# gabeur/mmt

Hardware: AMD Instinct MI355X
Metric: video-text pairs/sec (fwd+bwd+Adam), MSRVTT 7-expert d512 L4 (higher is better)
Workload: dtype bf16; 1 GPU; configs[1]: MSRVTT jsfusion shape, 7 experts x 30 tokens, d512, L4, H4, I3072, batch 32/GPU, dropout 0.1, train mode, Adam; text tower replaced by synthetic (B,768) vectors; global_batch=32, seq_len=218, parallelism=dp1, hip_graphs=True, inputs=resident in HBM, input_slots=8, input_format=dense fp32 dict, text_tower=synthetic, grad_sync=single, grad_wire_dtype=fp32, grad_algo=allreduce, comm_log=False, collectives_captured=False, dense_rows=6976, full=False

## Files before the change

### include/mmt_hip.h

```cpp
#ifndef MMT_HIP_H_
#define MMT_HIP_H_
#include <stdint.h>

#ifdef __cplusplus
extern "C" {
#endif

#define MMT_ABI_VERSION 6
#define MMT_ROW_ALIGN 256

#define MMT_ERR_ARG (-1)
#define MMT_ERR_ALIGN (-2)

int mmt_abi_version(void);
const char* mmt_build_info(void);

enum {
  MMT_EPI_BF16 = 0,
  MMT_EPI_BIAS_BF16 = 1,
  MMT_EPI_BIAS_GELU = 2,
  MMT_EPI_BIAS_DROP_RES = 3,
  MMT_EPI_DGELU = 4,
  MMT_EPI_ADD_F32 = 5,
  MMT_EPI_F32 = 6,
// ... 20 lines not shown
  float* dot_out;
  int32_t live_rows_hint;
} MmtEpilogue;

int mmt_gemm_nt_bf16(const void* A, int64_t lda, const void* B, int64_t ldb, void* C, int64_t ldc,
                     int M, int N, int K, int epilogue, const MmtEpilogue* epi,
                     const int32_t* n_rows_dev, void* stream);

int mmt_gemm_select_tile(int epilogue, int M, int N, int K, int packed, int live_rows_hint, int has_colsum, int has_dot_out,
                         int reserved);

int64_t mmt_gemm_nt_splitk_workspace_floats(int M, int N, int K);
int mmt_gemm_nt_splitk(const void* A, int64_t lda, const void* B, int64_t ldb, void* C, int64_t ldc, int M, int N, int K,
                       int epilogue, const MmtEpilogue* epi, float* ws, void* stream);
int mmt_gemm_nt_splitk_ex(const void* A, int64_t lda, const void* B, int64_t ldb, void* C, int64_t ldc, int M, int N, int K,
                          int epilogue, const MmtEpilogue* epi, float* ws, int splits, int wide, const int32_t* n_rows_dev,
                          int no_epilogue, void* stream);
int mmt_gemm_nn_bf16(const void* A, int64_t lda, const void* B, int64_t ldb, void* C, int64_t ldc, int M, int N, int K,
                     int epilogue, const MmtEpilogue* epi, const int32_t* n_rows_dev, void* stream);
int mmt_gemm_nn_splitk_ex(const void* A, int64_t lda, const void* B, int64_t ldb, void* C, int64_t ldc, int M, int N, int K,
                          int epilogue, const MmtEpilogue* epi, float* ws, int splits, int wide, const int32_t* n_rows_dev,
                          int no_epilogue, void* stream);

#define MMT_GEMM_GROUP_MAX 16
typedef struct MmtGemmItem {
  const void* A; const void* B; void* C; const float* bias;
  int64_t lda, ldb, ldc;
  int32_t M, N, K, tile_begin;
  const int32_t* n_rows_dev;
} MmtGemmItem;
int mmt_gemm_nt_grouped(const MmtGemmItem* items, int n, int epilogue, void* stream);

int mmt_gemm_tn_bf16(const void* A, int64_t lda, const void* B, int64_t ldb, float* ws,
                     int rows, int N, int K2, int splits, const int32_t* n_rows_dev, void* stream);
int mmt_reduce_slabs(const float* ws, int splits, int64_t count, float* out, int accumulate,
                     void* stream);
int mmt_reduce_slabs_pair(const float* ws_a, int64_t count_a, float* out_a, const float* ws_b, int64_t count_b,
                          float* out_b, int splits, void* stream);

#define MMT_WGRAD_MAX 16
typedef struct MmtWgradItem {
  const void* A;
  const void* B;
  float* out;
  float* bias_out;
  int64_t lda, ldb, ldo;
  int32_t N, K2, N_out, K2_out, tile_begin;
  int32_t reserved;
  float* slab;
  float* bias_slab;
  int32_t splits, reserved2;
  const int32_t* n_rows_dev;
} MmtWgradItem;
typedef struct MmtWgradGroup {
  MmtWgradItem item[MMT_WGRAD_MAX];
  const int32_t* n_rows_dev;
  int32_t count, rows;
} MmtWgradGroup;
int mmt_wgrad_grouped(const MmtWgradGroup* g, void* stream);

int mmt_reduce_slabs_2d(const float* ws, int splits, int rows, int cols_ws, int cols_out, float* out,
                        int accumulate, void* stream);

int mmt_ln_fwd(const float* z, const float* gamma, const float* beta, float eps, float* h32, void* h16,
               float* mean, float* rstd, int rows, int d, const int32_t* n_rows_dev, void* stream);
int mmt_embed_ln_fwd(const float* features, const int32_t* type_ids, const int32_t* pos_ids,
                     const float* type_emb, const float* pos_emb, float* z_save, const float* gamma,
                     const float* beta, float eps, float* h32, void* h16, float* mean, float* rstd,
                     int rows, int d, const int32_t* n_rows_dev, const int32_t* row_index,
                     uint32_t drop_key, uint32_t thr16, float drop_scale, const uint32_t* seed_dev,
                     void* stream);
int mmt_embed_ln_fwd_sched(const float* features, const int32_t* type_ids, const int32_t* pos_ids,
                           const float* type_emb, const float* pos_emb, float* z_save, const float* gamma,
                           const float* beta, float eps, float* h32, void* h16, float* mean, float* rstd,
                           int rows, int d, const int32_t* n_rows_dev, const int32_t* row_index,
                           uint32_t drop_key, uint32_t thr16, float drop_scale, const uint32_t* seed_dev,
                           const int32_t* sched_cu, int sched_B, int sched_H, int sched_tiles, int32_t* sched_work,
                           void* stream);
int mmt_ln_fwd_scatter(const float* z, const float* gamma, const float* beta, float eps, float* h32,
                       const int32_t* dst_rows, void* h16, float* mean, float* rstd, int rows, int d, void* stream);
int mmt_rows_gather(const float* src, const int32_t* rows, int n, int d, float* dst, const int32_t* idx_in,
                    int32_t* idx_out, void* stream);
int mmt_rows_scatter(const float* src, const int32_t* rows, int n, int d, float* dst, int accumulate, void* stream);
int mmt_table_grad_direct(const float* g, const int32_t* ids, int rows, int d, int vocab, const int32_t* n_rows_dev,
                          float* dtable, void* stream);
int mmt_embedding_grad(const float* g, const int32_t* ids, int n, int d, int vocab, int padding_idx,
                       const int32_t* n_rows_dev, float* dtable, void* stream);
int mmt_text_plan(const int64_t* input_ids, const int64_t* token_type_ids, const int64_t* position_ids,
                  const int64_t* attention_mask, int B, int W, int32_t* counts, int32_t* cu_seqlens, int32_t* n_rows_dev,
                  int32_t* ids, int32_t* types, int32_t* pos, int32_t* row_index, int32_t* cls_rows, void* stream);
int mmt_gemm_splitk_geometry(int M, int N, int K, int splits_requested, int* splits, int64_t* slab_stride);
int mmt_splitk_ln_fwd(const float* slabs, int splits, int64_t slab_stride, const float* bias, const float* res,
                      const int32_t* res_rows, const int32_t* rowidx, const int32_t* row_index, int32_t* rowidx_out,
                      uint32_t drop_key, uint32_t thr16, float drop_scale, const uint32_t* seed_dev, float* z_out,
                      const float* gamma, const float* beta, float eps, float* h32, void* h16, float* mean, float* rstd,
                      int rows, int d, void* stream);
int mmt_ln_bwd_slabs(const float* slabs, int splits, int64_t slab_stride, const float* res, const float* z,
                     const float* mean, const float* rstd, const float* gamma, float* dz, void* dy, float* partials,
                     int rows, int d, int drop_mode, const int32_t* row_index, uint32_t drop_key, uint32_t thr16,
                     float drop_scale, const uint32_t* seed_dev, void* stream);
int mmt_splitk_ln_fwd_ex(const float* slabs, int splits, int64_t slab_stride, const float* bias, const float* res,
                         const int32_t* res_rows, const int32_t* rowidx, const int32_t* row_index, int32_t* rowidx_out,
                         uint32_t drop_key, uint32_t thr16, float drop_scale, const uint32_t* seed_dev, float* z_out,
                         const float* gamma, const float* beta, float eps, float* h32, void* h16, float* mean, float* rstd,
                         int rows, int d, const int32_t* n_rows_dev, void* stream);
int mmt_ln_bwd_slabs_ex(const float* slabs, int splits, int64_t slab_stride, const float* res, const float* z,
                        const float* mean, const float* rstd, const float* gamma, float* dz, void* dy, float* partials,
                        int rows, int d, int drop_mode, const int32_t* n_rows_dev, const int32_t* row_index,
                        uint32_t drop_key, uint32_t thr16, float drop_scale, const uint32_t* seed_dev, void* stream);

int mmt_ln_bwd_rows_per_block(int rows);
int mmt_ln_bwd(const float* dout, const float* z, const float* mean, const float* rstd, const float* gamma,
               float* dz, void* dy, float* partials, int rows, int d, int drop_mode,
               const int32_t* n_rows_dev, const int32_t* row_index, uint32_t drop_key, uint32_t thr16,
               float drop_scale, const uint32_t* seed_dev, void* stream);
int mmt_col_reduce(const float* partials, int nblocks, int nvec, int d, float* out0, float* out1,
                   float* out2, float* out3, int accumulate, void* stream);
#define MMT_COLRED_MAX 32
typedef struct MmtColReduceJob {
  const float* partials;
  float* out[4];
  int32_t nblocks, nvec, nout, d;
} MmtColReduceJob;
int mmt_col_reduce_multi(const MmtColReduceJob* jobs, int n, void* stream);
int64_t mmt_table_grad_scratch_floats(int vocab, int d);
int mmt_table_grad(const float* g, const int32_t* ids, int rows, int d, int vocab,
                   const int32_t* n_rows_dev, float* scratch, float* dtable, int accumulate, void* stream);
int mmt_table_grad_partials(const float* g, const int32_t* ids, int rows, int d, int vocab,
                            const int32_t* n_rows_dev, float* scratch, void* stream);
int mmt_table_grad_partials_pair(const float* g, const int32_t* ids0, int vocab0, float* scratch0, const int32_t* ids1,
                                 int vocab1, float* scratch1, int rows, int d, const int32_t* n_rows_dev, void* stream);
int mmt_table_grad_chunks(void);
int mmt_colsum_bf16(const void* x, int64_t ld, int rows, int cols, const int32_t* n_rows_dev,
                    float* partials, void* stream);

int mmt_attn_fwd(const void* qkv, const int32_t* cu_seqlens, const float* mask_bias, void* ctx, float* lse,
                 int B, int S, int H, int d, float scale, uint32_t drop_key, uint32_t thr16,
                 float drop_scale, const uint32_t* seed_dev,
                 const int32_t* row_index, void* stream);
int mmt_attn_bwd_ex(const void* qkv, const int32_t* cu_seqlens, const float* mask_bias, const void* ctx,
                    const float* lse, const void* dctx, void* dqkv, float* delta, int delta_ready, int B, int S, int H,
                    int d, float scale, uint32_t drop_key, uint32_t thr16, float drop_scale,
                    const uint32_t* seed_dev, const int32_t* row_index, const int32_t* work, void* stream);
int64_t mmt_attn_schedule_words(int B, int S, int H);
int mmt_attn_schedule(const int32_t* cu_seqlens, int B, int S, int H, int32_t* work, void* stream);
int mmt_attn_bwd(const void* qkv, const int32_t* cu_seqlens, const float* mask_bias, const void* ctx,
                 const float* lse, const void* dctx, void* dqkv, float* delta, int B, int S, int H, int d,
                 float scale, uint32_t drop_key, uint32_t thr16, float drop_scale,
                 const uint32_t* seed_dev,
                 const int32_t* row_index, void* stream);
int mmt_attn_fwd_rows(const void* qkv, const int32_t* cu_seqlens, const float* mask_bias, const int32_t* qsel, int nq,
                      void* ctx, float* lse, int B, int S, int H, int d, float scale, uint32_t drop_key, uint32_t thr16,
                      float drop_scale, const uint32_t* seed_dev,
                 const int32_t* row_index, void* stream);
int mmt_attn_bwd_rows_ex(const void* qkv, const int32_t* cu_seqlens, const float* mask_bias, const int32_t* qsel, int nq,
                         const void* ctx, const float* lse, const void* dctx, void* dqkv, float* delta, int delta_ready,
                         int B, int S, int H, int d, float scale, uint32_t drop_key, uint32_t thr16, float drop_scale,
                         const uint32_t* seed_dev, const int32_t* row_index, void* stream);
int mmt_attn_bwd_rows(const void* qkv, const int32_t* cu_seqlens, const float* mask_bias, const int32_t* qsel, int nq,
                      const void* ctx, const float* lse, const void* dctx, void* dqkv, float* delta, int B, int S, int H,
                      int d, float scale, uint32_t drop_key, uint32_t thr16, float drop_scale,
                      const uint32_t* seed_dev,
                 const int32_t* row_index, void* stream);
int mmt_attn_dropout_mask(uint8_t* out, int B, int H, int S, uint32_t drop_key, uint32_t thr16,
                          const uint32_t* seed_dev, void* stream);

#define MMT_PACK_MAX 24
typedef struct MmtPackItem {
  const float* src;
  void* dst;
  void* dst_t;
  int32_t rows, cols, dst_ld, dst_t_ld, dst_t_rows, reserved;
} MmtPackItem;
int mmt_pack_weights(const MmtPackItem* items, int n, void* stream);
int mmt_adam_step(float* params, const float* grads, float* exp_avg, float* exp_avg_sq, int64_t count,
                  float lr, float beta1, float beta2, float eps, float weight_decay,
                  const int32_t* step_dev, const float* lr_dev, void* stream);

#define MMT_ADAM_SEG_MAX 160
typedef struct MmtAdamSeg {
  int64_t offset, count;
  void* dst;
  void* dst_t;
  int32_t rows, cols, dst_ld, dst_t_ld;
} MmtAdamSeg;
int mmt_adam_fused_blocks(const MmtAdamSeg* seg);
int mmt_adam_step_fused(float* params, const float* grads, float* exp_avg, float* exp_avg_sq,
                        const MmtAdamSeg* segs_host, const MmtAdamSeg* segs_dev, int n_segs, float lr, float beta1,
                        float beta2, float eps, float weight_decay, int32_t* step_dev, const float* lr_dev,
                        int bump_step, void* stream);

#define MMT_MAX_EXPERTS 16
typedef struct MmtExpertIO {
  const float* feat;
  const float* maxpool;
  const float* ind;
  const float* t;
  void* x;
  float* y;
  void* dy;
  int32_t D, Dpad, type_idx, rows_pad;
  const float* y_part[2];
  int32_t n_part, reserved;
} MmtExpertIO;
typedef struct MmtVideoSrc {
  int32_t* src_row;
  int32_t* src_cnt;
  int32_t* xsrc;
} MmtVideoSrc;
int mmt_video_plan(const MmtExpertIO* experts, int M, int B, int T, int pack, int max_pos, int32_t* counts,
                   int32_t* cu_seqlens, int32_t* n_rows_dev, int32_t* slot, int32_t* row_index, int32_t* type_ids,
                   int32_t* pos_ids, float* mask_bias, int32_t* agg_row, uint32_t* seed_bump, const MmtVideoSrc* src,
                   void* stream);
int mmt_video_cast(const MmtExpertIO* experts, int M, int B, int T, const MmtVideoSrc* src, void* stream);
int mmt_video_scatter(const MmtExpertIO* experts, int M, int B, int T, int d, const int32_t* n_rows_dev,
                      const int32_t* row_index, const MmtVideoSrc* src, float* features, void* stream);
int mmt_video_scatter_bwd(const MmtExpertIO* experts, int M, int B, int T, int d, const int32_t* n_rows_dev,
                          const int32_t* row_index, const MmtVideoSrc* src, const float* dfeatures, void* stream);

int mmt_readout_fwd(const float* last_hidden, const int32_t* agg_row, int BM, int d, float* vid_embds,
                    float* inv_norm, void* stream);
int mmt_readout_bwd(const float* vid_embds, const float* inv_norm, const float* dvid_embds,
                    const int32_t* agg_row, int BM, int d, float* dlast_hidden, void* stream);
int mmt_sims_fwd(const float* txt, const float* vid, const float* tw, const float* vw, int NT, int NV, int M,
                 int d, float* sims, float* dots, void* stream);
int mmt_sims_bwd(const float* txt, const float* vid, const float* tw, const float* vw, float* dots,
                 const float* dsims, int NT, int NV, int M, int d, float* dtxt, float* dvid, float* dtw,
                 float* dvw, void* stream);
int mmt_simloss_small_max_n(void);
int mmt_simloss_bwd_small(const float* txt, const float* vid, const float* tw, const float* vw, const float* sims,
                          const float* dots, int n, int M, int d, int kind, float margin, int fix_norm, float* loss,
                          float* dtxt, float* dvid, float* dtw, float* dvw, const float* inv_norm,
                          const int32_t* out_rows, float* dlast, void* stream);

int mmt_maxmargin(const float* sims, int n, float margin, int fix_norm, float* partial, float* loss,
                  float* grad, void* stream);
int mmt_infonce(const float* sims, int n, float* scratch, float* loss, float* grad, void* stream);

int64_t mmt_sims_eval_workspace_floats(int NT, int NV, int M, int d);
int mmt_sims_eval(const float* txt, const float* vid, const float* tw, const float* vw, int NT, int NV, int M, int d,
                  float* ws, float* sims, void* stream);
int mmt_retrieval_ranks(const float* sims, const uint8_t* qmask, int NQ, int NV, float* t2v_rank, float* v2t_rank,
                        float* scratch, void* stream);

int mmt_search_fold(const float* x, const float* w, int N, int M, int d, float* out, void* stream);
int mmt_search_fold_bf16(const float* x, const float* w, int N, int M, int d, uint16_t* out, void* stream);
int mmt_search_fold_split_bf16(const float* x, const float* w, int N, int M, int d, uint16_t* hi, uint16_t* lo,
                               void* stream);
int mmt_search_fold_fp8(const float* x, const float* w, int N, int M, int d, uint8_t* out, float* scale, void* stream);
int mmt_rows_topk(const float* sims, int64_t ld, const int32_t* rows, int NR, int NV, int k, uint64_t* ws, float* scores,
                  int64_t* index, void* stream);

#define MMT_SEARCH_FP32 0
#define MMT_SEARCH_BF16 1
#define MMT_SEARCH_FP8 2
#define MMT_SEARCH_SETS_NONE 0
#define MMT_SEARCH_SETS_QUERY 1
#define MMT_SEARCH_SETS_ITEM 2
typedef struct MmtSearchScan {
  const void* q;
  const void* q_lo;
  const float* qw;
  const void* g;
  const float* gw;
  const float* gscale;
  const uint32_t* subset;
  const int64_t* exclude;
  const uint64_t* after;
  const float* lse;
  const float* set_weights;
  int32_t storage;
  int32_t NQ;
  int32_t NV;
  int32_t M;
  int32_t d;
  int32_t E;
  float beta;
  int32_t sets;
  int32_t set_size;
  int32_t mode;
} MmtSearchScan;
#ifdef __cplusplus
static_assert(sizeof(MmtSearchScan) == 128, "MmtSearchScan: 11 pointers, then 10 four-byte fields");
#else
_Static_assert(sizeof(MmtSearchScan) == 128, "MmtSearchScan: 11 pointers, then 10 four-byte fields");
#endif

int64_t mmt_topk_workspace_keys(int NQ, int NV, int k);
int64_t mmt_rank_workspace_ints(int NQ, int NV, int T);
int64_t mmt_count_workspace_ints(int NQ, int NV, int T);
int64_t mmt_range_workspace_ints(int NQ, int NV);
int64_t mmt_col_lse_workspace_floats(int NB, int NV);
int64_t mmt_rescore_workspace_keys(int NQ, int C);
int64_t mmt_topk_pooled_workspace_keys(int NS, int C, int NV, int k);
int64_t mmt_count_pooled_workspace_ints(int NS, int C, int NV, int T);
int64_t mmt_topk_itemsets_workspace_keys(int NQ, int NT, int C, int k);
int64_t mmt_count_itemsets_workspace_ints(int NQ, int NT, int C, int T);
int mmt_search_topk(const MmtSearchScan* scan, int k, uint64_t* ws, float* scores, int64_t* index, void* stream);
int mmt_search_topk_groups(const MmtSearchScan* scan, int k, const int32_t* group_ids, uint64_t* ws, float* scores,
                           int64_t* groups, int64_t* items, void* stream);
int mmt_search_rank(const MmtSearchScan* scan, const int64_t* targets, int T, int32_t* ws, int32_t* greater,
// ... 93 lines not shown
  float *running_mean[MMT_MAX_EXPERTS], *running_var[MMT_MAX_EXPERTS];
  const float *moe_w[MMT_MAX_EXPERTS], *moe_b[MMT_MAX_EXPERTS];
  float *g_w1[MMT_MAX_EXPERTS], *g_b1[MMT_MAX_EXPERTS], *g_w2[MMT_MAX_EXPERTS], *g_b2[MMT_MAX_EXPERTS];
  float *g_bn_gamma[MMT_MAX_EXPERTS], *g_bn_beta[MMT_MAX_EXPERTS], *g_moe_w[MMT_MAX_EXPERTS], *g_moe_b[MMT_MAX_EXPERTS];
} MmtTextHeads;
int64_t mmt_text_heads_workspace_floats(int N, int M, int d);
typedef struct MmtVideoFront {
  const MmtExpertIO* experts;
  int32_t M, B, T, pack, max_pos, do_cast;
  int32_t *counts, *cu_seqlens, *n_rows_dev, *slot, *row_index, *type_ids, *pos_ids;
  float* mask_bias;
  int32_t* agg_row;
  uint32_t* seed_bump;
  const MmtVideoSrc* src;
} MmtVideoFront;
typedef struct MmtTextHeadsOpts {
  uint32_t moe_drop_key, moe_drop_thr16;
  float moe_drop_scale;
  int32_t reserved;
  const uint32_t* seed_dev;
  uint32_t* key_dev;
  int64_t* num_batches_tracked;
  const MmtVideoFront* video_front;
} MmtTextHeadsOpts;
int mmt_text_heads_fast(int N, int M, int d, int K);
int mmt_text_heads_fwd(const MmtTextHeads* h, const float* text, const float* text_moe, int N, int C, int M, int d,
                       int K, int use_bn, int training, float* ws, float* text_embds, float* text_weights,
                       const MmtTextHeadsOpts* opts, void* stream);
int mmt_text_heads_bwd(const MmtTextHeads* h, const float* text, const float* text_moe, const float* w1_all, int N,
                       int C, int M, int d, int K, int use_bn, int training, float* ws, const float* dtext_embds,
                       const float* text_weights, const float* dtext_weights, float* dtext, float* dtext_moe,
                       const MmtTextHeadsOpts* opts, void* stream);

typedef struct MmtBertLayer {
  const void *wqkv, *wqkv_t, *wo, *wo_t, *w1, *w1_t, *w2, *w2_t;
  const float *bqkv, *bo, *ln1_g, *ln1_b, *b1, *b2, *ln2_g, *ln2_b;
  float *g_wqkv, *g_bqkv, *g_wo, *g_bo, *g_ln1_g, *g_ln1_b, *g_w1, *g_b1, *g_w2, *g_b2, *g_ln2_g, *g_ln2_b;
} MmtBertLayer;

typedef struct MmtBertModel {
  int32_t hidden, layers, heads, inter, max_pos, type_vocab;
  float ln_eps, p_hidden, p_attn;
  int32_t reserved;
  const float *pos_emb, *type_emb, *emb_ln_g, *emb_ln_b;
  float *g_pos_emb, *g_type_emb, *g_emb_ln_g, *g_emb_ln_b;
  const MmtBertLayer* layer;
} MmtBertModel;

typedef struct MmtBertBatch {
  const float* features;
  const int32_t* type_ids;
  const int32_t* pos_ids;
  const float* mask_bias;
  const int32_t* cu_seqlens;
  const int32_t* row_index;
  const int32_t* n_rows_dev;
  const uint32_t* seed_dev;
  int32_t rows, rows_alloc, batch, seq;
  const int32_t* out_rows;
  int32_t n_out_per_sample;
  int32_t fork;
  void* side_stream;
  int32_t live_rows_hint;
} MmtBertBatch;

enum {
  MMT_FORK_WGRAD = 1,
  MMT_FORK_EARLY = 2,
  MMT_FORK_REDUCE = 4,
  MMT_FORK_JOIN = 8,
  MMT_RANGE_LAYERS_ONLY = 16
};

int mmt_stream_fork(void* from, void* to);

int64_t mmt_bert_workspace_bytes(const MmtBertModel* m, int rows_alloc);
int mmt_bert_tail_capacity(int rows_alloc);
int mmt_bert_forward(const MmtBertModel* m, const MmtBertBatch* b, void* ws, float* out_last, int training,
                     void* stream);
int mmt_bert_backward(const MmtBertModel* m, const MmtBertBatch* b, void* ws, float* dlast, float* dfeatures,
                      int training, void* stream);
int mmt_bert_backward_range(const MmtBertModel* m, const MmtBertBatch* b, void* ws, float* dlast, float* dfeatures,
                            int training, int l_hi, int l_lo, void* stream);

int mmt_probe_arm(void** start_events, void** stop_events, int n);
int mmt_probe_arm_site(int site, void** start_events, void** stop_events, int n);
int mmt_probe_count_site(int site);
int mmt_dropout_f32(const float* x, float* y, int64_t n, uint32_t drop_key, uint32_t thr16, float scale,
                    const uint32_t* seed_dev, uint32_t* key_save, const uint32_t* key_load, void* stream);
int mmt_debug_dispatch_probe(int blocks, int threads, int lds_bytes, int spin, float* sink, void* stream);
int mmt_probe_count(void);

#ifdef __cplusplus
}
#endif
#endif
```

### mmt_amd/_lib.py

```python
import ctypes
import os

_HERE = os.path.dirname(os.path.abspath(__file__))
LIB_PATH = os.environ.get('MMT_HIP_LIB') or os.path.join(_HERE, 'lib', 'libmmt_hip.so')

c_int, c_i64, c_u32, c_f32, c_vp = ctypes.c_int, ctypes.c_int64, ctypes.c_uint32, ctypes.c_float, ctypes.c_void_p


class MmtEpilogue(ctypes.Structure):
  _fields_ = [('bias', c_vp), ('res', c_vp), ('ldres', c_i64), ('out2', c_vp), ('ldout2', c_i64),
              ('aux', c_vp), ('ldaux', c_i64), ('colsum', c_vp), ('row_index', c_vp), ('seed_dev', c_vp),
              ('drop_key', c_u32), ('drop_thr16', c_u32), ('drop_scale', c_f32), ('reserved', ctypes.c_int32),
              ('dot_src', c_vp), ('lddot', c_i64), ('dot_out', c_vp), ('live_rows_hint', ctypes.c_int32)]


class MmtPackItem(ctypes.Structure):
  _fields_ = [('src', c_vp), ('dst', c_vp), ('dst_t', c_vp), ('rows', ctypes.c_int32), ('cols', ctypes.c_int32),
              ('dst_ld', ctypes.c_int32), ('dst_t_ld', ctypes.c_int32), ('dst_t_rows', ctypes.c_int32),
              ('reserved', ctypes.c_int32)]


class MmtAdamSeg(ctypes.Structure):
  _fields_ = [('offset', c_i64), ('count', c_i64), ('dst', c_vp), ('dst_t', c_vp), ('rows', ctypes.c_int32),
              ('cols', ctypes.c_int32), ('dst_ld', ctypes.c_int32), ('dst_t_ld', ctypes.c_int32)]


class MmtGemmItem(ctypes.Structure):
  _fields_ = [('A', c_vp), ('B', c_vp), ('C', c_vp), ('bias', c_vp), ('lda', c_i64), ('ldb', c_i64), ('ldc', c_i64),
              ('M', ctypes.c_int32), ('N', ctypes.c_int32), ('K', ctypes.c_int32), ('tile_begin', ctypes.c_int32),
              ('n_rows_dev', c_vp)]


class MmtWgradItem(ctypes.Structure):
  _fields_ = [('A', c_vp), ('B', c_vp), ('out', c_vp), ('bias_out', c_vp), ('lda', c_i64), ('ldb', c_i64), ('ldo', c_i64),
              ('N', ctypes.c_int32), ('K2', ctypes.c_int32), ('N_out', ctypes.c_int32), ('K2_out', ctypes.c_int32),
              ('tile_begin', ctypes.c_int32), ('reserved', ctypes.c_int32), ('slab', c_vp), ('bias_slab', c_vp),
              ('splits', ctypes.c_int32), ('reserved2', ctypes.c_int32), ('n_rows_dev', c_vp)]


class MmtWgradGroup(ctypes.Structure):
  _fields_ = [('item', MmtWgradItem * 16), ('n_rows_dev', c_vp), ('count', ctypes.c_int32), ('rows', ctypes.c_int32)]


class MmtColReduceJob(ctypes.Structure):
  _fields_ = [('partials', c_vp), ('out', c_vp * 4), ('nblocks', ctypes.c_int32), ('nvec', ctypes.c_int32),
              ('nout', ctypes.c_int32), ('d', ctypes.c_int32)]


class MmtVideoSrc(ctypes.Structure):
  _fields_ = [('src_row', c_vp), ('src_cnt', c_vp), ('xsrc', c_vp)]


class MmtExpertIO(ctypes.Structure):
  _fields_ = [('feat', c_vp), ('maxpool', c_vp), ('ind', c_vp), ('t', c_vp), ('x', c_vp), ('y', c_vp), ('dy', c_vp),
              ('D', ctypes.c_int32), ('Dpad', ctypes.c_int32), ('type_idx', ctypes.c_int32),
              ('rows_pad', ctypes.c_int32), ('y_part', c_vp * 2), ('n_part', ctypes.c_int32),
              ('reserved', ctypes.c_int32)]


_LAYER_PTRS = ['wqkv', 'wqkv_t', 'wo', 'wo_t', 'w1', 'w1_t', 'w2', 'w2_t',
               'bqkv', 'bo', 'ln1_g', 'ln1_b', 'b1', 'b2', 'ln2_g', 'ln2_b',
               'g_wqkv', 'g_bqkv', 'g_wo', 'g_bo', 'g_ln1_g', 'g_ln1_b', 'g_w1', 'g_b1', 'g_w2', 'g_b2',
               'g_ln2_g', 'g_ln2_b']


class MmtBertLayer(ctypes.Structure):
  _fields_ = [(n, c_vp) for n in _LAYER_PTRS]


class MmtBertModel(ctypes.Structure):
  _fields_ = ([(n, ctypes.c_int32) for n in ('hidden', 'layers', 'heads', 'inter', 'max_pos', 'type_vocab')] +
              [(n, c_f32) for n in ('ln_eps', 'p_hidden', 'p_attn')] + [('reserved', ctypes.c_int32)] +
              [(n, c_vp) for n in ('pos_emb', 'type_emb', 'emb_ln_g', 'emb_ln_b', 'g_pos_emb', 'g_type_emb',
                                   'g_emb_ln_g', 'g_emb_ln_b')] +
              [('layer', ctypes.POINTER(MmtBertLayer))])


class MmtBertBatch(ctypes.Structure):
  _fields_ = ([(n, c_vp) for n in ('features', 'type_ids', 'pos_ids', 'mask_bias', 'cu_seqlens', 'row_index',
                                   'n_rows_dev', 'seed_dev')] +
              [(n, ctypes.c_int32) for n in ('rows', 'rows_alloc', 'batch', 'seq')] +
              [('out_rows', c_vp), ('n_out_per_sample', ctypes.c_int32), ('fork', ctypes.c_int32),
               ('side_stream', c_vp), ('live_rows_hint', ctypes.c_int32)])


FORK_WGRAD, FORK_EARLY, FORK_REDUCE, FORK_JOIN, RANGE_LAYERS_ONLY = 1, 2, 4, 8, 16


_PTR16 = c_vp * 16


class MmtSgemm(ctypes.Structure):
  _fields_ = [('A', _PTR16), ('B', _PTR16), ('C', _PTR16), ('bias', _PTR16),
              ('sai', c_i64), ('sak', c_i64), ('sbj', c_i64), ('sbk', c_i64), ('ldc', c_i64),
              ('batch', ctypes.c_int32), ('M', ctypes.c_int32), ('N', ctypes.c_int32), ('K', ctypes.c_int32),
              ('beta', c_f32), ('reserved', ctypes.c_int32)]


_TEXT_HEAD_FIELDS = ['w1', 'b1', 'w2', 'b2', 'bn_gamma', 'bn_beta', 'running_mean', 'running_var', 'moe_w', 'moe_b',
                     'g_w1', 'g_b1', 'g_w2', 'g_b2', 'g_bn_gamma', 'g_bn_beta', 'g_moe_w', 'g_moe_b']


class MmtTextHeads(ctypes.Structure):
  _fields_ = [(n, _PTR16) for n in _TEXT_HEAD_FIELDS]


class MmtVideoFront(ctypes.Structure):
  _fields_ = [('experts', c_vp), ('M', ctypes.c_int32), ('B', ctypes.c_int32), ('T', ctypes.c_int32), ('pack', ctypes.c_int32),
              ('max_pos', ctypes.c_int32), ('do_cast', ctypes.c_int32), ('counts', c_vp), ('cu_seqlens', c_vp),
              ('n_rows_dev', c_vp), ('slot', c_vp), ('row_index', c_vp), ('type_ids', c_vp), ('pos_ids', c_vp),
              ('mask_bias', c_vp), ('agg_row', c_vp), ('seed_bump', c_vp), ('src', c_vp)]


class MmtTextHeadsOpts(ctypes.Structure):
  _fields_ = [('moe_drop_key', c_u32), ('moe_drop_thr16', c_u32), ('moe_drop_scale', c_f32), ('reserved', ctypes.c_int32),
              ('seed_dev', c_vp), ('key_dev', c_vp), ('num_batches_tracked', c_vp), ('video_front', c_vp)]


class MmtSearchScan(ctypes.Structure):
  _fields_ = ([(n, c_vp) for n in ('q', 'q_lo', 'qw', 'g', 'gw', 'gscale', 'subset', 'exclude', 'after', 'lse',
                                   'set_weights')] +
              [(n, ctypes.c_int32) for n in ('storage', 'NQ', 'NV', 'M', 'd', 'E')] + [('beta', c_f32)] +
              [(n, ctypes.c_int32) for n in ('sets', 'set_size', 'mode')])


SEARCH_FP32, SEARCH_BF16, SEARCH_FP8 = 0, 1, 2
SEARCH_SETS_NONE, SEARCH_SETS_QUERY, SEARCH_SETS_ITEM = 0, 1, 2
_SCAN = ctypes.POINTER(MmtSearchScan)

EPI = dict(BF16=0, BIAS_BF16=1, BIAS_GELU=2, BIAS_DROP_RES=3, DGELU=4, ADD_F32=5, F32=6, BIAS_F32=7)

SIGNATURES = {
    'mmt_abi_version': (c_int, []),
    'mmt_build_info': (ctypes.c_char_p, []),
    'mmt_gemm_nt_bf16': (c_int, [c_vp, c_i64, c_vp, c_i64, c_vp, c_i64, c_int, c_int, c_int, c_int,
                                 ctypes.POINTER(MmtEpilogue), c_vp, c_vp]),
    'mmt_gemm_select_tile': (c_int, [c_int] * 9),
    'mmt_gemm_tn_bf16': (c_int, [c_vp, c_i64, c_vp, c_i64, c_vp, c_int, c_int, c_int, c_int, c_vp, c_vp]),
    'mmt_gemm_nt_splitk_workspace_floats': (c_i64, [c_int, c_int, c_int]),
    'mmt_gemm_nt_splitk': (c_int, [c_vp, c_i64, c_vp, c_i64, c_vp, c_i64, c_int, c_int, c_int, c_int,
                                   ctypes.POINTER(MmtEpilogue), c_vp, c_vp]),
    'mmt_gemm_nn_bf16': (c_int, [c_vp, c_i64, c_vp, c_i64, c_vp, c_i64, c_int, c_int, c_int, c_int,
                                 ctypes.POINTER(MmtEpilogue), c_vp, c_vp]),
    'mmt_gemm_nn_splitk_ex': (c_int, [c_vp, c_i64, c_vp, c_i64, c_vp, c_i64, c_int, c_int, c_int, c_int,
                                      ctypes.POINTER(MmtEpilogue), c_vp, c_int, c_int, c_vp, c_int, c_vp]),
    'mmt_gemm_nt_splitk_ex': (c_int, [c_vp, c_i64, c_vp, c_i64, c_vp, c_i64, c_int, c_int, c_int, c_int,
                                      ctypes.POINTER(MmtEpilogue), c_vp, c_int, c_int, c_vp, c_int, c_vp]),
    'mmt_gemm_nt_grouped': (c_int, [ctypes.POINTER(MmtGemmItem), c_int, c_int, c_vp]),
    'mmt_wgrad_grouped': (c_int, [ctypes.POINTER(MmtWgradGroup), c_vp]),
    'mmt_reduce_slabs': (c_int, [c_vp, c_int, c_i64, c_vp, c_int, c_vp]),
    'mmt_reduce_slabs_pair': (c_int, [c_vp, c_i64, c_vp, c_vp, c_i64, c_vp, c_int, c_vp]),
    'mmt_ln_fwd': (c_int, [c_vp, c_vp, c_vp, c_f32, c_vp, c_vp, c_vp, c_vp, c_int, c_int, c_vp, c_vp]),
    'mmt_embed_ln_fwd': (c_int, [c_vp, c_vp, c_vp, c_vp, c_vp, c_vp, c_vp, c_vp, c_f32, c_vp, c_vp, c_vp, c_vp,
                                 c_int, c_int, c_vp, c_vp, c_u32, c_u32, c_f32, c_vp, c_vp]),
    'mmt_embed_ln_fwd_sched': (c_int, [c_vp, c_vp, c_vp, c_vp, c_vp, c_vp, c_vp, c_vp, c_f32, c_vp, c_vp, c_vp, c_vp,
                                 c_int, c_int, c_vp, c_vp, c_u32, c_u32, c_f32, c_vp, c_vp, c_int, c_int, c_int, c_vp, c_vp]),
    'mmt_ln_bwd_rows_per_block': (c_int, [c_int]),
    'mmt_gemm_splitk_geometry': (c_int, [c_int, c_int, c_int, c_int, c_vp, c_vp]),
    'mmt_splitk_ln_fwd': (c_int, [c_vp, c_int, c_i64, c_vp, c_vp, c_vp, c_vp, c_vp, c_vp, c_u32, c_u32, c_f32, c_vp, c_vp, c_vp,
                                  c_vp, c_f32, c_vp, c_vp, c_vp, c_vp, c_int, c_int, c_vp]),
    'mmt_ln_bwd_slabs': (c_int, [c_vp, c_int, c_i64, c_vp, c_vp, c_vp, c_vp, c_vp, c_vp, c_vp, c_vp, c_int, c_int, c_int, c_vp,
                                 c_u32, c_u32, c_f32, c_vp, c_vp]),
    'mmt_splitk_ln_fwd_ex': (c_int, [c_vp, c_int, c_i64, c_vp, c_vp, c_vp, c_vp, c_vp, c_vp, c_u32, c_u32, c_f32, c_vp, c_vp, c_vp,
                                     c_vp, c_f32, c_vp, c_vp, c_vp, c_vp, c_int, c_int, c_vp, c_vp]),
    'mmt_ln_bwd_slabs_ex': (c_int, [c_vp, c_int, c_i64, c_vp, c_vp, c_vp, c_vp, c_vp, c_vp, c_vp, c_vp, c_int, c_int, c_int, c_vp,
                                    c_vp, c_u32, c_u32, c_f32, c_vp, c_vp]),
    'mmt_ln_bwd': (c_int, [c_vp, c_vp, c_vp, c_vp, c_vp, c_vp, c_vp, c_vp, c_int, c_int, c_int, c_vp, c_vp,
                           c_u32, c_u32, c_f32, c_vp, c_vp]),
    'mmt_col_reduce': (c_int, [c_vp, c_int, c_int, c_int, c_vp, c_vp, c_vp, c_vp, c_int, c_vp]),
    'mmt_col_reduce_multi': (c_int, [ctypes.POINTER(MmtColReduceJob), c_int, c_vp]),
    'mmt_table_grad_partials': (c_int, [c_vp, c_vp, c_int, c_int, c_int, c_vp, c_vp, c_vp]),
    'mmt_table_grad_chunks': (c_int, []),
    'mmt_table_grad_partials_pair': (c_int, [c_vp, c_vp, c_int, c_vp, c_vp, c_int, c_vp, c_int, c_int, c_vp, c_vp]),
    'mmt_table_grad_scratch_floats': (c_i64, [c_int, c_int]),
    'mmt_table_grad': (c_int, [c_vp, c_vp, c_int, c_int, c_int, c_vp, c_vp, c_vp, c_int, c_vp]),
    'mmt_attn_fwd': (c_int, [c_vp, c_vp, c_vp, c_vp, c_vp, c_int, c_int, c_int, c_int, c_f32, c_u32, c_u32,
                             c_f32, c_vp, c_vp, c_vp]),
    'mmt_attn_bwd': (c_int, [c_vp, c_vp, c_vp, c_vp, c_vp, c_vp, c_vp, c_vp, c_int, c_int, c_int, c_int, c_f32,
                             c_u32, c_u32, c_f32, c_vp, c_vp, c_vp]),
    'mmt_attn_bwd_ex': (c_int, [c_vp, c_vp, c_vp, c_vp, c_vp, c_vp, c_vp, c_vp, c_int, c_int, c_int, c_int, c_int, c_f32,
                                c_u32, c_u32, c_f32, c_vp, c_vp, c_vp, c_vp]),
    'mmt_attn_schedule_words': (c_i64, [c_int, c_int, c_int]),
    'mmt_attn_schedule': (c_int, [c_vp, c_int, c_int, c_int, c_vp, c_vp]),
    'mmt_attn_bwd_rows_ex': (c_int, [c_vp, c_vp, c_vp, c_vp, c_int, c_vp, c_vp, c_vp, c_vp, c_vp, c_int, c_int, c_int, c_int,
                                     c_int, c_f32, c_u32, c_u32, c_f32, c_vp, c_vp, c_vp]),
    'mmt_attn_fwd_rows': (c_int, [c_vp, c_vp, c_vp, c_vp, c_int, c_vp, c_vp, c_int, c_int, c_int, c_int, c_f32, c_u32, c_u32,
                                  c_f32, c_vp, c_vp, c_vp]),
    'mmt_attn_bwd_rows': (c_int, [c_vp, c_vp, c_vp, c_vp, c_int, c_vp, c_vp, c_vp, c_vp, c_vp, c_int, c_int, c_int, c_int,
                                  c_f32, c_u32, c_u32, c_f32, c_vp, c_vp, c_vp]),
    'mmt_ln_fwd_scatter': (c_int, [c_vp, c_vp, c_vp, c_f32, c_vp, c_vp, c_vp, c_vp, c_vp, c_int, c_int, c_vp]),
    'mmt_rows_gather': (c_int, [c_vp, c_vp, c_int, c_int, c_vp, c_vp, c_vp, c_vp]),
    'mmt_rows_scatter': (c_int, [c_vp, c_vp, c_int, c_int, c_vp, c_int, c_vp]),
    'mmt_embedding_grad': (c_int, [c_vp, c_vp, c_int, c_int, c_int, c_int, c_vp, c_vp, c_vp]),
    'mmt_text_plan': (c_int, [c_vp, c_vp, c_vp, c_vp, c_int, c_int, c_vp, c_vp, c_vp, c_vp, c_vp, c_vp, c_vp, c_vp, c_vp]),
    'mmt_table_grad_direct': (c_int, [c_vp, c_vp, c_int, c_int, c_int, c_vp, c_vp, c_vp]),
    'mmt_attn_dropout_mask': (c_int, [c_vp, c_int, c_int, c_int, c_u32, c_u32, c_vp, c_vp]),
    'mmt_reduce_slabs_2d': (c_int, [c_vp, c_int, c_int, c_int, c_int, c_vp, c_int, c_vp]),
    'mmt_colsum_bf16': (c_int, [c_vp, c_i64, c_int, c_int, c_vp, c_vp, c_vp]),
    'mmt_pack_weights': (c_int, [ctypes.POINTER(MmtPackItem), c_int, c_vp]),
    'mmt_dropout_f32': (c_int, [c_vp, c_vp, c_i64, c_u32, c_u32, c_f32, c_vp, c_vp, c_vp, c_vp]),
    'mmt_debug_dispatch_probe': (c_int, [c_int, c_int, c_int, c_int, c_vp, c_vp]),
    'mmt_adam_step': (c_int, [c_vp, c_vp, c_vp, c_vp, c_i64, c_f32, c_f32, c_f32, c_f32, c_f32, c_vp, c_vp, c_vp]),
    'mmt_adam_fused_blocks': (c_int, [ctypes.POINTER(MmtAdamSeg)]),
    'mmt_adam_step_fused': (c_int, [c_vp, c_vp, c_vp, c_vp, ctypes.POINTER(MmtAdamSeg), c_vp, c_int, c_f32, c_f32, c_f32,
                                    c_f32, c_f32, c_vp, c_vp, c_int, c_vp]),
    'mmt_video_plan': (c_int, [ctypes.POINTER(MmtExpertIO), c_int, c_int, c_int, c_int, c_int, c_vp, c_vp, c_vp, c_vp,
                               c_vp, c_vp, c_vp, c_vp, c_vp, c_vp, ctypes.POINTER(MmtVideoSrc), c_vp]),
    'mmt_video_cast': (c_int, [ctypes.POINTER(MmtExpertIO), c_int, c_int, c_int, ctypes.POINTER(MmtVideoSrc), c_vp]),
    'mmt_video_scatter': (c_int, [ctypes.POINTER(MmtExpertIO), c_int, c_int, c_int, c_int, c_vp, c_vp,
                                  ctypes.POINTER(MmtVideoSrc), c_vp, c_vp]),
    'mmt_video_scatter_bwd': (c_int, [ctypes.POINTER(MmtExpertIO), c_int, c_int, c_int, c_int, c_vp, c_vp,
                                      ctypes.POINTER(MmtVideoSrc), c_vp, c_vp]),
    'mmt_readout_fwd': (c_int, [c_vp, c_vp, c_int, c_int, c_vp, c_vp, c_vp]),
    'mmt_readout_bwd': (c_int, [c_vp, c_vp, c_vp, c_vp, c_int, c_int, c_vp, c_vp]),
    'mmt_sims_fwd': (c_int, [c_vp, c_vp, c_vp, c_vp, c_int, c_int, c_int, c_int, c_vp, c_vp, c_vp]),
    'mmt_sims_bwd': (c_int, [c_vp, c_vp, c_vp, c_vp, c_vp, c_vp, c_int, c_int, c_int, c_int, c_vp, c_vp, c_vp, c_vp,
                             c_vp]),
    'mmt_sims_eval_workspace_floats': (c_i64, [c_int, c_int, c_int, c_int]),
    'mmt_sims_eval': (c_int, [c_vp, c_vp, c_vp, c_vp, c_int, c_int, c_int, c_int, c_vp, c_vp, c_vp]),
    'mmt_retrieval_ranks': (c_int, [c_vp, c_vp, c_int, c_int, c_vp, c_vp, c_vp, c_vp]),
    'mmt_search_fold': (c_int, [c_vp, c_vp, c_int, c_int, c_int, c_vp, c_vp]),
    'mmt_topk_workspace_keys': (c_i64, [c_int, c_int, c_int]),
    'mmt_rows_topk': (c_int, [c_vp, c_i64, c_vp, c_int, c_int, c_int, c_vp, c_vp, c_vp, c_vp]),
    'mmt_search_fold_bf16': (c_int, [c_vp, c_vp, c_int, c_int, c_int, c_vp, c_vp]),
    'mmt_search_fold_split_bf16': (c_int, [c_vp, c_vp, c_int, c_int, c_int, c_vp, c_vp, c_vp]),
    'mmt_rank_workspace_ints': (c_i64, [c_int, c_int, c_int]),
    'mmt_search_subset_pack': (c_int, [c_vp, c_int, c_vp, c_vp]),
    'mmt_count_workspace_ints': (c_i64, [c_int, c_int, c_int]),
    'mmt_search_merge_lists': (c_int, [c_vp, c_vp, c_vp, c_int, c_int, c_int, c_int, c_vp, c_vp, c_vp]),
    'mmt_col_lse_workspace_floats': (c_i64, [c_int, c_int]),
    'mmt_range_workspace_ints': (c_i64, [c_int, c_int]),
    'mmt_search_fold_fp8': (c_int, [c_vp, c_vp, c_int, c_int, c_int, c_vp, c_vp, c_vp]),
    'mmt_search_merge_group_lists': (c_int, [c_vp, c_vp, c_vp, c_vp, c_int, c_int, c_int, c_int, c_vp, c_vp, c_vp, c_vp]),
    'mmt_topk_pooled_workspace_keys': (c_i64, [c_int, c_int, c_int, c_int]),
    'mmt_count_pooled_workspace_ints': (c_i64, [c_int, c_int, c_int, c_int]),
    'mmt_topk_itemsets_workspace_keys': (c_i64, [c_int, c_int, c_int, c_int]),
    'mmt_count_itemsets_workspace_ints': (c_i64, [c_int, c_int, c_int, c_int]),
    'mmt_rescore_workspace_keys': (c_i64, [c_int, c_int]),
    'mmt_search_after_keys': (c_int, [c_vp, c_vp, c_int, c_vp, c_vp]),
    'mmt_search_topk': (c_int, [_SCAN, c_int, c_vp, c_vp, c_vp, c_vp]),
    'mmt_search_topk_groups': (c_int, [_SCAN, c_int, c_vp, c_vp, c_vp, c_vp, c_vp, c_vp]),
    'mmt_search_rank': (c_int, [_SCAN, c_vp, c_int, c_vp, c_vp, c_vp, c_vp]),
    'mmt_search_thresholds': (c_int, [_SCAN, c_vp, c_int, c_vp, c_vp]),
    'mmt_search_count': (c_int, [_SCAN, c_vp, c_int, c_vp, c_vp, c_vp, c_vp]),
    'mmt_search_range_count': (c_int, [_SCAN, c_vp, c_vp, c_vp, c_vp]),
    'mmt_search_range_fill': (c_int, [_SCAN, c_vp, c_vp, c_vp, c_vp, c_vp, c_vp]),
    'mmt_search_rescore': (c_int, [_SCAN, c_vp, c_int, c_int, c_vp, c_vp, c_vp, c_vp]),
    'mmt_search_col_lse': (c_int, [_SCAN, c_f32, c_vp, c_vp, c_int, c_vp, c_vp]),
    'mmt_col_topk_workspace_keys': (c_i64, [c_int, c_int, c_int]),
    'mmt_search_col_topk': (c_int, [_SCAN, c_int, c_int, c_vp, c_vp, c_int, c_vp, c_vp, c_vp, c_f32, c_vp]),
    'mmt_search_pair_scores': (c_int, [c_vp, c_vp, c_vp, c_int, c_int, c_int, c_int, c_vp, c_int, c_int, c_vp, c_vp]),
    'mmt_search_mmr': (c_int, [c_vp, c_vp, c_vp, c_int, c_int, c_int, c_f32, c_f32, c_vp, c_vp, c_vp, c_vp]),
    'mmt_self_topk_workspace_keys': (c_i64, [c_int, c_int, c_int]),
    'mmt_self_range_workspace_ints': (c_i64, [c_int, c_int]),
    'mmt_search_self_topk': (c_int, [c_vp, c_vp, c_vp, c_int, c_vp, c_vp, c_int, c_vp, c_vp, c_vp, c_int, c_vp, c_int, c_int,
                                     c_int, c_int, c_vp, c_vp, c_vp, c_vp]),
    'mmt_search_self_range_count': (c_int, [c_vp, c_vp, c_vp, c_int, c_vp, c_vp, c_int, c_vp, c_vp, c_vp, c_int, c_vp, c_int,
                                            c_int, c_int, c_vp, c_vp, c_vp, c_vp]),
    'mmt_search_self_range_fill': (c_int, [c_vp, c_vp, c_vp, c_int, c_vp, c_vp, c_int, c_vp, c_vp, c_vp, c_int, c_vp, c_int,
                                           c_int, c_int, c_vp, c_vp, c_vp, c_vp, c_vp, c_vp]),
    'mmt_row_expsum_workspace_ints64': (c_i64, [c_int, c_int]),
    'mmt_search_row_expsum': (c_int, [_SCAN, c_f32, c_vp, c_int, c_vp, c_vp]),
    'mmt_ls_fold_bf16': (c_int, [c_vp, c_vp, c_int, c_int, c_int, c_int, c_vp, c_vp]),
    'mmt_transpose_bf16': (c_int, [c_vp, c_i64, c_int, c_int, c_vp, c_i64, c_vp]),
    'mmt_ls_finish': (c_int, [c_vp, c_i64, c_vp, c_vp, c_int, c_int, c_int, c_vp]),
    'mmt_ls_col_blocks': (c_int, [c_int]),
    'mmt_ls_diag': (c_int, [c_vp, c_i64, c_vp, c_vp, c_int, c_int, c_int, c_int, c_vp, c_vp]),
    'mmt_ls_counts_ex': (c_int, [c_vp, c_i64, c_vp, c_vp, c_vp, c_vp, c_int, c_int, c_int, c_int, c_int, c_f32, c_vp, c_vp, c_vp, c_vp]),
    'mmt_ls_counts': (c_int, [c_vp, c_i64, c_vp, c_int, c_int, c_int, c_f32, c_vp, c_vp, c_vp, c_vp]),
    'mmt_ls_grad': (c_int, [c_vp, c_i64, c_vp, c_vp, c_vp, c_vp, c_vp, c_int, c_int, c_int, c_int, c_f32, c_f32, c_vp, c_i64,
                            c_vp, c_vp]),
    'mmt_ls_grad_ex': (c_int, [c_vp, c_i64, c_vp, c_vp, c_vp, c_vp, c_vp, c_vp, c_int, c_int, c_int, c_int, c_f32, c_f32, c_vp, c_i64,
                            c_vp, c_int, c_vp]),
    'mmt_ls_unfold': (c_int, [c_vp, c_i64, c_vp, c_vp, c_vp, c_int, c_int, c_int, c_vp, c_vp, c_vp]),
    'mmt_ls_nce_col_blocks': (c_int, [c_int]),
    'mmt_ls_nce_row_groups': (c_int, [c_int]),
    'mmt_ls_nce_stats': (c_int, [c_vp, c_i64, c_vp, c_vp, c_vp, c_int, c_int, c_int, c_int, c_f32, c_vp, c_vp, c_vp]),
    'mmt_ls_nce_grad': (c_int, [c_vp, c_i64, c_vp, c_vp, c_vp, c_vp, c_vp, c_int, c_int, c_int, c_int, c_f32, c_f32, c_vp, c_i64,
                                c_vp, c_vp]),
    'mmt_simloss_small_max_n': (c_int, []),
    'mmt_simloss_bwd_small': (c_int, [c_vp, c_vp, c_vp, c_vp, c_vp, c_vp, c_int, c_int, c_int, c_int, c_f32, c_int, c_vp, c_vp,
                                      c_vp, c_vp, c_vp, c_vp, c_vp, c_vp, c_vp]),
    'mmt_maxmargin': (c_int, [c_vp, c_int, c_f32, c_int, c_vp, c_vp, c_vp, c_vp]),
    'mmt_infonce': (c_int, [c_vp, c_int, c_vp, c_vp, c_vp, c_vp]),
    'mmt_bert_tail_capacity': (c_int, [c_int]),
    'mmt_bert_workspace_bytes': (c_i64, [ctypes.POINTER(MmtBertModel), c_int]),
    'mmt_bert_forward': (c_int, [ctypes.POINTER(MmtBertModel), ctypes.POINTER(MmtBertBatch), c_vp, c_vp, c_int, c_vp]),
    'mmt_bert_backward': (c_int, [ctypes.POINTER(MmtBertModel), ctypes.POINTER(MmtBertBatch), c_vp, c_vp, c_vp, c_int,
                                  c_vp]),
    'mmt_bert_backward_range': (c_int, [ctypes.POINTER(MmtBertModel), ctypes.POINTER(MmtBertBatch), c_vp, c_vp, c_vp,
                                        c_int, c_int, c_int, c_vp]),
    'mmt_stream_fork': (c_int, [c_vp, c_vp]),
    'mmt_sgemm_batched': (c_int, [ctypes.POINTER(MmtSgemm), c_vp]),
    'mmt_text_heads_workspace_floats': (c_i64, [c_int, c_int, c_int]),
    'mmt_text_heads_fast': (c_int, [c_int, c_int, c_int, c_int]),
    'mmt_text_heads_fwd': (c_int, [ctypes.POINTER(MmtTextHeads), c_vp, c_vp, c_int, c_int, c_int, c_int, c_int, c_int,
                                   c_int, c_vp, c_vp, c_vp, ctypes.POINTER(MmtTextHeadsOpts), c_vp]),
    'mmt_text_heads_bwd': (c_int, [ctypes.POINTER(MmtTextHeads), c_vp, c_vp, c_vp, c_int, c_int, c_int, c_int, c_int,
                                   c_int, c_int, c_vp, c_vp, c_vp, c_vp, c_vp, c_vp, ctypes.POINTER(MmtTextHeadsOpts),
                                   c_vp]),
    'mmt_probe_arm': (c_int, [c_vp, c_vp, c_int]),
    'mmt_probe_count': (c_int, []),
    'mmt_probe_arm_site': (c_int, [c_int, c_vp, c_vp, c_int]),
    'mmt_probe_count_site': (c_int, [c_int]),
}

_lib = None


def lib():
  global _lib
  if _lib is None:
    if not os.path.exists(LIB_PATH):
      raise RuntimeError(
          'libmmt_hip.so is missing (%s): run `python -m mmt_amd.build` (hipcc, gfx950). '
          'There is no CPU fallback for the MMT hot path.' % LIB_PATH)
    handle = ctypes.CDLL(LIB_PATH)
    for name, (res, args) in SIGNATURES.items():
      fn = getattr(handle, name)
      fn.restype = res
      fn.argtypes = args
    if handle.mmt_abi_version() != 6:
      raise RuntimeError('libmmt_hip.so ABI mismatch')
    _lib = handle
  return _lib


def check(rc, what):
  if rc != 0:
    raise RuntimeError('%s failed with code %d' % (what, rc))
```

### mmt_amd/bert.py

```python
import ctypes
import math

import torch
from torch import nn

from . import _lib, ops
from ._lib import MmtBertBatch, MmtBertLayer, MmtBertModel, check
from .flat import FlatParams


class BertEmbeddings(nn.Module):

  def __init__(self, config):
    super().__init__()
    self.position_embeddings = nn.Embedding(config.max_position_embeddings, config.hidden_size)
    self.token_type_embeddings = nn.Embedding(config.type_vocab_size, config.hidden_size)
    self.layer_norm = nn.LayerNorm(config.hidden_size, eps=config.layer_norm_eps)
    self.dropout = nn.Dropout(config.hidden_dropout_prob)


class BertSelfAttention(nn.Module):

  def __init__(self, config):
    super().__init__()
    if config.hidden_size % config.num_attention_heads != 0:
      raise ValueError('The hidden size (%d) is not a multiple of the number of attention heads (%d)' %
                       (config.hidden_size, config.num_attention_heads))
    self.num_attention_heads = config.num_attention_heads
    self.attention_head_size = config.hidden_size // config.num_attention_heads
    self.query = nn.Linear(config.hidden_size, config.hidden_size)
    self.key = nn.Linear(config.hidden_size, config.hidden_size)
    self.value = nn.Linear(config.hidden_size, config.hidden_size)
    self.dropout = nn.Dropout(config.attention_probs_dropout_prob)


class BertSelfOutput(nn.Module):

  def __init__(self, config):
    super().__init__()
    self.dense = nn.Linear(config.hidden_size, config.hidden_size)
    self.layer_norm = nn.LayerNorm(config.hidden_size, eps=config.layer_norm_eps)
    self.dropout = nn.Dropout(config.hidden_dropout_prob)


class BertAttention(nn.Module):

  def __init__(self, config):
    super().__init__()
    self.self = BertSelfAttention(config)
    self.output = BertSelfOutput(config)


class BertIntermediate(nn.Module):

  def __init__(self, config):
    super().__init__()
    if config.hidden_act != 'gelu':
      raise NotImplementedError('native video-BERT implements hidden_act="gelu" (erf form) only')
    self.dense = nn.Linear(config.hidden_size, config.intermediate_size)


class BertOutput(nn.Module):

  def __init__(self, config):
    super().__init__()
    self.dense = nn.Linear(config.intermediate_size, config.hidden_size)
    self.layer_norm = nn.LayerNorm(config.hidden_size, eps=config.layer_norm_eps)
    self.dropout = nn.Dropout(config.hidden_dropout_prob)


class BertLayer(nn.Module):

  def __init__(self, config):
    super().__init__()
    self.attention = BertAttention(config)
    self.intermediate = BertIntermediate(config)
    self.output = BertOutput(config)


class BertEncoder(nn.Module):

  def __init__(self, config):
    super().__init__()
    self.layer = nn.ModuleList([BertLayer(config) for _ in range(config.num_hidden_layers)])


class BertPooler(nn.Module):

  def __init__(self, config):
    super().__init__()
    self.dense = nn.Linear(config.hidden_size, config.hidden_size)
    self.activation = nn.Tanh()

  def forward(self, hidden_states):
    return self.activation(self.dense(hidden_states[:, 0]))


class EngineBatch:

  def __init__(self, features, type_ids, pos_ids, mask_bias, rows, batch, seq, cu_seqlens=None,
               row_index=None, n_rows_dev=None, out_rows=None, n_out_per_sample=0):
    self.features, self.type_ids, self.pos_ids, self.mask_bias = features, type_ids, pos_ids, mask_bias
    self.rows, self.batch, self.seq = rows, batch, seq
    self.cu_seqlens, self.row_index, self.n_rows_dev = cu_seqlens, row_index, n_rows_dev
    self.out_rows, self.n_out_per_sample = out_rows, n_out_per_sample
    self.save = False
    self.side_stream, self.fork = None, 0


class _BertFn(torch.autograd.Function):

  @staticmethod
  def forward(ctx, model, batch, features, *params):
    out = model._engine_forward(batch, features, save=batch.save)
    ctx.model, ctx.batch, ctx.generation = model, batch, model._generation
    ctx.training = model.training
    return out

  @staticmethod
  def backward(ctx, dout):
    model = ctx.model
    if model._generation != ctx.generation:
      raise RuntimeError('mmt_amd.BertModel: saved activations were overwritten by a later forward '
                         '(one pending backward per module)')
    dfeat, grads = model._engine_backward(ctx.batch, dout, ctx.training)
    return (None, None, dfeat) + tuple(grads)


class BertModel(nn.Module):

  def __init__(self, config):
    super().__init__()
    self.config = config
    self.embeddings = BertEmbeddings(config)
    self.encoder = BertEncoder(config)
    self.pooler = BertPooler(config)
    self.apply(self._init_weights)
    self.compute_pooler = True
    self._flat = None
    self._owns_flat = True
    self._ws = {}
    self._generation = 0
    self._seed_dev = None
    self._structs = {}

  def _init_weights(self, module):
    if isinstance(module, (nn.Linear, nn.Embedding)):
      module.weight.data.normal_(mean=0.0, std=self.config.initializer_range)
    elif isinstance(module, nn.LayerNorm):
      module.bias.data.zero_()
      module.weight.data.fill_(1.0)
    if isinstance(module, nn.Linear) and module.bias is not None:
      module.bias.data.zero_()

  def engine_named_params(self, prefix=''):
    e = self.embeddings
    out = [('embeddings.position_embeddings.weight', e.position_embeddings.weight),
           ('embeddings.token_type_embeddings.weight', e.token_type_embeddings.weight),
           ('embeddings.layer_norm.weight', e.layer_norm.weight), ('embeddings.layer_norm.bias', e.layer_norm.bias)]
    for i, L in enumerate(self.encoder.layer):
      a, p = L.attention, 'encoder.layer.%d.' % i
      out += [(p + 'attention.self.query.weight', a.self.query.weight),
              (p + 'attention.self.key.weight', a.self.key.weight),
              (p + 'attention.self.value.weight', a.self.value.weight),
              (p + 'attention.self.query.bias', a.self.query.bias),
              (p + 'attention.self.key.bias', a.self.key.bias),
              (p + 'attention.self.value.bias', a.self.value.bias),
              (p + 'attention.output.dense.weight', a.output.dense.weight),
              (p + 'attention.output.dense.bias', a.output.dense.bias),
              (p + 'attention.output.layer_norm.weight', a.output.layer_norm.weight),
              (p + 'attention.output.layer_norm.bias', a.output.layer_norm.bias),
              (p + 'intermediate.dense.weight', L.intermediate.dense.weight),
              (p + 'intermediate.dense.bias', L.intermediate.dense.bias),
              (p + 'output.dense.weight', L.output.dense.weight), (p + 'output.dense.bias', L.output.dense.bias),
              (p + 'output.layer_norm.weight', L.output.layer_norm.weight),
              (p + 'output.layer_norm.bias', L.output.layer_norm.bias)]
    return [(prefix + n, q) for n, q in out]

  def trainable_engine_params(self):
    return [p for _, p in self.engine_named_params()]

  def flat_named_params(self):
    return self.engine_named_params()

  def register_shadows(self, flat):
    d, i = self.config.hidden_size, self.config.intermediate_size
    for l, L in enumerate(self.encoder.layer):
      a = L.attention
      flat.add_shadow(('bert', id(self), l, 'wqkv'), [a.self.query.weight, a.self.key.weight, a.self.value.weight],
                      3 * d, d, transpose=True)
# ... 58 lines not shown
                        emb_ln_g=e.layer_norm.weight, emb_ln_b=e.layer_norm.bias).items():
      setattr(m, name, f.ptr(p))
      setattr(m, 'g_' + name, f.ptr(p, grad_buf))
    m.layer = layers
    self._structs[key] = (m, layers)
    return m, layers

  def _batch_struct(self, batch, rows_alloc):
    b = MmtBertBatch()
    b.features = batch.features.data_ptr()
    b.type_ids = batch.type_ids.data_ptr()
    b.pos_ids = batch.pos_ids.data_ptr() if batch.pos_ids is not None else None
    b.mask_bias = batch.mask_bias.data_ptr()
    b.cu_seqlens = batch.cu_seqlens.data_ptr() if batch.cu_seqlens is not None else None
    b.row_index = batch.row_index.data_ptr() if batch.row_index is not None else None
    b.n_rows_dev = batch.n_rows_dev.data_ptr() if batch.n_rows_dev is not None else None
    b.seed_dev = self._seed_dev.data_ptr()
    b.rows, b.rows_alloc, b.batch, b.seq = batch.rows, rows_alloc, batch.batch, batch.seq
    if batch.out_rows is not None and batch.n_out_per_sample > 0:
      b.out_rows, b.n_out_per_sample = batch.out_rows.data_ptr(), batch.n_out_per_sample
    if batch.side_stream is not None and batch.fork:
      b.side_stream, b.fork = batch.side_stream.cuda_stream, int(batch.fork)
    b.live_rows_hint = int(getattr(batch, 'live_rows_hint', 0) or 0)
    return b

  def _workspace(self, rows_alloc, save, model_struct):
    key = (rows_alloc, bool(save))
    ws = self._ws.get(key)
    if ws is None:
      nbytes = _lib.lib().mmt_bert_workspace_bytes(ctypes.byref(model_struct), rows_alloc)
      if nbytes <= 0:
        raise RuntimeError('mmt_bert_workspace_bytes failed (%d)' % nbytes)
      ws = torch.zeros(nbytes, dtype=torch.uint8, device=self._flat.master.device)
      self._ws[key] = ws
    return ws

  def compact_output(self, batch, rows_alloc):
    if batch.out_rows is None or batch.n_out_per_sample <= 0:
      return False
    return batch.batch * batch.n_out_per_sample <= _lib.lib().mmt_bert_tail_capacity(rows_alloc)

  def _engine_forward(self, batch, features, save):
    rows_alloc = features.shape[0]
    if features.dtype != torch.float32 or not features.is_contiguous() or rows_alloc % ops.ROW_ALIGN:
      raise RuntimeError('engine features must be contiguous fp32 [rows padded to %d, hidden]' % ops.ROW_ALIGN)
    batch.features = features
    grad_buf = self._flat.current_grad()
    m, _ = self._struct(grad_buf)
    if save:
      self._generation += 1
      if self.training and not getattr(self, '_seed_bumped', False):
        self._seed_dev.add_(1)
    self._seed_bumped = False
    ws = self._workspace(rows_alloc, save, m)
    out = torch.empty(rows_alloc, self.config.hidden_size, device=features.device, dtype=torch.float32)
    b = self._batch_struct(batch, rows_alloc)
    check(_lib.lib().mmt_bert_forward(ctypes.byref(m), ctypes.byref(b), ws.data_ptr(), out.data_ptr(),
                                      int(self.training), ops._stream()), 'mmt_bert_forward')
    return out

  def _engine_backward(self, batch, dout, training):
    run = self.backward_ranges(batch, dout, training)
    run(self.config.num_hidden_layers - 1, 0)
    grad_buf = self._flat.current_grad()
    grads = [self._flat.view(p, grad_buf) if p.requires_grad else None for p in self.trainable_engine_params()]
    return run.dfeat, grads

  def backward_ranges(self, batch, dout, training):
    rows_alloc = batch.features.shape[0]
    grad_buf = self._flat.current_grad()
    m, _ = self._struct(grad_buf)
    ws = self._workspace(rows_alloc, True, m)
    if self.compact_output(batch, rows_alloc):
      dlast = dout.contiguous()
    else:
      dlast = dout.contiguous().clone()
    dfeat = torch.empty_like(dlast)
    L = _lib.lib()

    def run(l_hi, l_lo, embed=True):
      b = self._batch_struct(batch, rows_alloc)
      if not embed:
        b.fork |= _lib.RANGE_LAYERS_ONLY
      check(L.mmt_bert_backward_range(ctypes.byref(m), ctypes.byref(b), ws.data_ptr(), dlast.data_ptr(),
                                      dfeat.data_ptr(), int(training), int(l_hi), int(l_lo), ops._stream()),
            'mmt_bert_backward_range')

    run.dfeat, run.keep = dfeat, (dlast, ws, m)
    return run

  def run_engine(self, batch, features):
    self._ensure_ready(features.device)
    params = self.trainable_engine_params()
    batch.save = torch.is_grad_enabled() and (features.requires_grad or any(p.requires_grad for p in params))
    return _BertFn.apply(self, batch, features, *params)

  def forward(self, input_ids, attention_mask=None, token_type_ids=None, position_ids=None, features=None):
    if features is None:
      raise ValueError('features are required (the video BERT has no word embeddings)')
    if not features.is_cuda:
      raise RuntimeError('mmt_amd.BertModel runs on the GPU only (no CPU fallback)')
    bsz, seq, d = features.shape
    dev = features.device
    rows = bsz * seq
    R = ops.pad_rows(rows)
    if attention_mask is None:
      attention_mask = torch.ones(bsz, seq, device=dev)
    if token_type_ids is None:
      token_type_ids = torch.zeros(bsz, seq, dtype=torch.long, device=dev)

    for name, ids, size in (('token_type_ids', token_type_ids, self.config.type_vocab_size),
                            ('position_ids', position_ids, self.config.max_position_embeddings)):
      if ids is not None and ids.numel() and not (0 <= int(ids.min()) and int(ids.max()) < size):
        raise IndexError('%s out of range [0, %d)' % (name, size))

    def rows_i32(x):
      buf = torch.zeros(R, dtype=torch.int32, device=dev)
      buf[:rows] = x.reshape(-1).to(device=dev, dtype=torch.int32)
      return buf

    feat = torch.zeros(R, d, device=dev, dtype=torch.float32)
    feat[:rows] = features.reshape(rows, d).float()
    if features.requires_grad:
      feat = _PadRows.apply(features.reshape(rows, d).float(), R)
    mask_bias = torch.zeros(R, device=dev, dtype=torch.float32)
    mask_bias[:rows] = (1.0 - attention_mask.reshape(-1).to(device=dev, dtype=torch.float32)) * -10000.0
    batch = EngineBatch(None, rows_i32(token_type_ids), rows_i32(position_ids) if position_ids is not None else None,
                        mask_bias, rows, bsz, seq)
    seq_out = self.run_engine(batch, feat)[:rows].view(bsz, seq, d)
    if not self.compute_pooler:
      return (seq_out, None)
    return (seq_out, self.pooler(seq_out))


class _PadRows(torch.autograd.Function):

  @staticmethod
  def forward(ctx, x, R):
    ctx.rows = x.shape[0]
    out = torch.zeros(R, x.shape[1], device=x.device, dtype=x.dtype)
    out[:ctx.rows] = x
    return out

  @staticmethod
  def backward(ctx, g):
    return g[:ctx.rows], None
```

### mmt_amd/csrc/assemble.hip

```cpp
#include "mmt_common.h"
#include "../../include/mmt_hip.h"
#include "video_front.h"

__global__ __launch_bounds__(256) void video_plan_kernel(VideoPlanArgs p) {
  extern __shared__ float plan_ind_s[];
  video_plan_block(p, (int)blockIdx.x, (int)threadIdx.x, plan_ind_s);
}

__global__ void scan_counts_kernel(const int32_t* __restrict__ counts, int B, int32_t* __restrict__ cu,
                                   int32_t* __restrict__ n_rows) {
  if (threadIdx.x == 0 && blockIdx.x == 0) {
    int acc = 0;
    for (int b = 0; b < B; ++b) { cu[b] = acc; acc += counts[b]; }
    cu[B] = acc;
    *n_rows = acc;
  }
}

__global__ __launch_bounds__(256) void cast_kernel(VideoCastArgs c) {
  video_cast_block(c, (int)blockIdx.y, (int)blockIdx.x, (int)gridDim.x, (int)threadIdx.x, 256);
}

template <bool BWD>
__global__ __launch_bounds__(256) void scatter_kernel(ExpertTable tab, int M, int T, int S, int d, int rows,
                                                      const int32_t* __restrict__ n_rows_dev,
                                                      const int32_t* __restrict__ row_index, MmtVideoSrc src,
                                                      float* __restrict__ feat, const float* __restrict__ dfeat) {
  const int lane = threadIdx.x & 63, wave = threadIdx.x >> 6;
  const int nrows = n_rows_dev ? min(*n_rows_dev, rows) : rows;
  const int nch = d >> 8;
  for (int row = blockIdx.x * 4 + wave; row < nrows; row += gridDim.x * 4) {
    const int s = row_index[row] % S;
    if (s == 0) {
      if constexpr (!BWD)
        for (int c = lane * 4; c < d; c += 256) *(f32x4*)(feat + (int64_t)row * d + c) = (f32x4){0.f, 0.f, 0.f, 0.f};
      continue;
    }
    const MmtExpertIO e = tab.e[(s - 1) / (T + 1)];
    const int64_t r = src.src_row[row];
    f32x4 y[4];
    float ss = 0.f;
#pragma unroll
    for (int c = 0; c < 4; ++c)
      if (c < nch) {
        y[c] = *(const f32x4*)(e.y + r * d + c * 256 + lane * 4);
        if (e.n_part > 0) y[c] += *(const f32x4*)(e.y_part[0] + r * d + c * 256 + lane * 4);
        if (e.n_part > 1) y[c] += *(const f32x4*)(e.y_part[1] + r * d + c * 256 + lane * 4);
        ss += y[c][0] * y[c][0] + y[c][1] * y[c][1] + y[c][2] * y[c][2] + y[c][3] * y[c][3];
      }
    const float nrm = sqrtf(wave_sum(ss));
    const float inv = 1.0f / fmaxf(nrm, 1e-12f);
    if constexpr (!BWD) {
#pragma unroll
      for (int c = 0; c < 4; ++c)
        if (c < nch) *(f32x4*)(feat + (int64_t)row * d + c * 256 + lane * 4) = y[c] * inv;
    } else {
      f32x4 g[4];
      float dot = 0.f;
#pragma unroll
      for (int c = 0; c < 4; ++c)
        if (c < nch) {
          g[c] = *(const f32x4*)(dfeat + (int64_t)row * d + c * 256 + lane * 4);
          dot += g[c][0] * y[c][0] + g[c][1] * y[c][1] + g[c][2] * y[c][2] + g[c][3] * y[c][3];
        }
      const float proj = nrm > 1e-12f ? wave_sum(dot) * inv * inv : 0.f;
#pragma unroll
      for (int c = 0; c < 4; ++c)
        if (c < nch) {
          f32x4 dyv = (g[c] - y[c] * proj) * inv;
          u32x2 o = {pack_bf2(dyv[0], dyv[1]), pack_bf2(dyv[2], dyv[3])};
          *(u32x2*)((bf16_t*)e.dy + r * d + c * 256 + lane * 4) = o;
        }
    }
  }
}

__global__ __launch_bounds__(256) void text_count_kernel(const int64_t* __restrict__ mask, int W, int32_t* __restrict__ counts) {
  __shared__ int red[4];
  const int b = blockIdx.x;
  int c = 0;
  for (int t = threadIdx.x; t < W; t += 256) c += (mask[(int64_t)b * W + t] != 0) || t == 0;
#pragma unroll
  for (int o = 32; o > 0; o >>= 1) c += __shfl_xor(c, o, 64);
  if ((threadIdx.x & 63) == 0) red[threadIdx.x >> 6] = c;
  __syncthreads();
  if (threadIdx.x == 0) counts[b] = red[0] + red[1] + red[2] + red[3];
}

__global__ __launch_bounds__(256) void text_pack_kernel(const int64_t* __restrict__ ids_in, const int64_t* __restrict__ types_in,
                                                        const int64_t* __restrict__ pos_in, const int64_t* __restrict__ mask,
                                                        int W, const int32_t* __restrict__ cu, int32_t* __restrict__ ids,
                                                        int32_t* __restrict__ types, int32_t* __restrict__ pos,
                                                        int32_t* __restrict__ row_index, int32_t* __restrict__ cls_rows) {
  __shared__ int wave_cnt[4];
  const int b = blockIdx.x, lane = threadIdx.x & 63, wave = threadIdx.x >> 6;
  const int base = cu[b];
  int carry = 0;
  for (int t0 = 0; t0 < W; t0 += 256) {
    const int t = t0 + threadIdx.x;
    const int64_t src = (int64_t)b * W + t;
    const bool keep = t < W && (mask[src] != 0 || t == 0);
    const unsigned long long bal = __ballot(keep);
    const int before = __popcll(bal & ((1ull << lane) - 1ull));
    if (lane == 0) wave_cnt[wave] = __popcll(bal);
    __syncthreads();
    int woff = 0, total = 0;
#pragma unroll
    for (int i = 0; i < 4; ++i) { if (i < wave) woff += wave_cnt[i]; total += wave_cnt[i]; }
    if (keep) {
      const int r = base + carry + woff + before;
      ids[r] = (int32_t)ids_in[src];
      types[r] = types_in ? (int32_t)types_in[src] : 0;
      pos[r] = pos_in ? (int32_t)pos_in[src] : t;
      row_index[r] = (int32_t)src;
    }
    carry += total;
    __syncthreads();
  }
  if (threadIdx.x == 0) cls_rows[b] = base;
}

extern "C" int mmt_text_plan(const int64_t* input_ids, const int64_t* token_type_ids, const int64_t* position_ids,
                             const int64_t* attention_mask, int B, int W, int32_t* counts, int32_t* cu_seqlens,
                             int32_t* n_rows_dev, int32_t* ids, int32_t* types, int32_t* pos, int32_t* row_index,
                             int32_t* cls_rows, void* stream) {
  if (!input_ids || !attention_mask || !counts || !cu_seqlens || !n_rows_dev || !ids || !types || !pos || !row_index ||
      !cls_rows || B <= 0 || W <= 0)
    return MMT_ERR_ARG;
  hipStream_t s = (hipStream_t)stream;
  hipLaunchKernelGGL(text_count_kernel, dim3(B), dim3(256), 0, s, attention_mask, W, counts);
  hipLaunchKernelGGL(scan_counts_kernel, dim3(1), dim3(64), 0, s, counts, B, cu_seqlens, n_rows_dev);
  hipLaunchKernelGGL(text_pack_kernel, dim3(B), dim3(256), 0, s, input_ids, token_type_ids, position_ids, attention_mask, W,
                     cu_seqlens, ids, types, pos, row_index, cls_rows);
  return (int)hipGetLastError();
}

extern "C" int mmt_video_plan(const MmtExpertIO* experts, int M, int B, int T, int pack, int max_pos,
                              int32_t* counts, int32_t* cu_seqlens, int32_t* n_rows_dev, int32_t* slot,
                              int32_t* row_index, int32_t* type_ids, int32_t* pos_ids, float* mask_bias,
                              int32_t* agg_row, uint32_t* seed_bump, const MmtVideoSrc* src, void* stream) {
  VideoPlanArgs p;
  if (int e = video_plan_args(p, experts, M, B, T, pack, max_pos, counts, cu_seqlens, n_rows_dev, slot, row_index, type_ids,
                              pos_ids, mask_bias, agg_row, seed_bump, src))
    return e;
  hipLaunchKernelGGL(video_plan_kernel, dim3(B), dim3(256), (size_t)M * T * sizeof(float), (hipStream_t)stream, p);
  return (int)hipGetLastError();
}

extern "C" int mmt_video_cast(const MmtExpertIO* experts, int M, int B, int T, const MmtVideoSrc* src, void* stream) {
  VideoCastArgs c;
  if (int e = video_cast_args(c, experts, M, B, T, src)) return e;
  hipLaunchKernelGGL(cast_kernel, dim3(256, M), dim3(256), 0, (hipStream_t)stream, c);
  return (int)hipGetLastError();
}

extern "C" int mmt_video_scatter(const MmtExpertIO* experts, int M, int B, int T, int d, const int32_t* n_rows_dev,
                                 const int32_t* row_index, const MmtVideoSrc* src, float* features, void* stream) {
  ExpertTable tab;
  if (int e = make_table(experts, M, tab)) return e;
  if (int e = check_src(src)) return e;
  if (!row_index || !features || d % 256 || d > 1024) return MMT_ERR_ARG;
  const int S = 1 + M * (T + 1), rows = B * S;
  hipLaunchKernelGGL(scatter_kernel<false>, dim3((rows + 3) / 4), dim3(256), 0, (hipStream_t)stream, tab, M, T, S, d, rows,
                     n_rows_dev, row_index, *src, features, nullptr);
  return (int)hipGetLastError();
}

extern "C" int mmt_video_scatter_bwd(const MmtExpertIO* experts, int M, int B, int T, int d, const int32_t* n_rows_dev,
                                     const int32_t* row_index, const MmtVideoSrc* src, const float* dfeatures,
                                     void* stream) {
  ExpertTable tab;
  if (int e = make_table(experts, M, tab)) return e;
  if (int e = check_src(src)) return e;
  if (!row_index || !dfeatures || d % 256 || d > 1024) return MMT_ERR_ARG;
  for (int i = 0; i < M; ++i)
    if (!experts[i].dy) return MMT_ERR_ARG;
  const int S = 1 + M * (T + 1), rows = B * S;
  hipLaunchKernelGGL(scatter_kernel<true>, dim3((rows + 3) / 4), dim3(256), 0, (hipStream_t)stream, tab, M, T, S, d, rows,
                     n_rows_dev, row_index, *src, nullptr, dfeatures);
  return (int)hipGetLastError();
}
```

### mmt_amd/csrc/bert_engine.hip

```cpp
#include <hip/hip_runtime.h>
#include <stdint.h>
#include <mutex>
#include "../../include/mmt_hip.h"

namespace {

enum { SITE_EMB = 0, SITE_PROBS = 1, SITE_ATTN_OUT = 2, SITE_FFN_OUT = 3 };
inline uint32_t site_key(int layer, int site) { return 0x5eed0000u + (uint32_t)layer * 16u + (uint32_t)site; }
inline uint32_t thr16_of(float p) { int t = (int)(p * 65536.0f + 0.5f); return t < 0 ? 0u : (uint32_t)t; }
inline float scale_of(uint32_t thr) { return thr ? 1.0f / (1.0f - (float)thr / 65536.0f) : 1.0f; }

struct LayerWs {
  char *qkv, *ctx, *a16, *hpre, *g, *h16;
  float *lse, *z1, *mean1, *rstd1, *a32, *z2, *mean2, *rstd2, *h32;
};
constexpr int TAIL_WSPLIT = 4;
struct TailWs {
  char *ctx, *a16, *hpre, *g, *dy2, *dy, *dhpre, *dctx;
  float *lse, *res32, *z1, *mean1, *rstd1, *a32, *z2, *mean2, *rstd2, *dcur, *dz, *dA, *delta;
  int32_t* rowidx;
  float* slabs;
  float *wslab, *bslab;
  int cap;
};
// ... 177 lines not shown
  const float qk_scale = m->hidden == m->heads * 128 ? 0.08838834764831845f : 0.125f;

  TRY(mmt_embed_ln_fwd_sched(b->features, b->type_ids, b->pos_ids, m->type_emb, m->pos_emb, w.z0, m->emb_ln_g,
                       m->emb_ln_b, m->ln_eps, w.h32_in, w.h16_in, w.mean0, w.rstd0, rows, d, b->n_rows_dev,
                       b->row_index, site_key(0, SITE_EMB), th, sh, b->seed_dev, b->cu_seqlens, b->batch, m->heads, (b->seq + 63) / 64,
                             const_cast<int32_t*>(attn_work_of(m, b, w)), stream));
  const float* hin32 = w.h32_in;
  const char* hin16 = w.h16_in;
  const int nc = tail_rows(b, w);
  for (int l = 0; l < m->layers; ++l) {
    const MmtBertLayer& P = m->layer[l];
    LayerWs& L = w.layer[l];
    MmtEpilogue e = {}; e.live_rows_hint = lh;
    e.bias = P.bqkv;
    TRY(mmt_gemm_nt_bf16(hin16, d, P.wqkv, d, L.qkv, 3 * d, rows, 3 * d, d, MMT_EPI_BIAS_BF16, &e, b->n_rows_dev, stream));
    if (nc && l == m->layers - 1) {
      TailWs& t = w.t;
      TRY(mmt_attn_fwd_rows(L.qkv, b->cu_seqlens, b->mask_bias, b->out_rows, b->n_out_per_sample, t.ctx, t.lse, b->batch,
                            b->seq, m->heads, d, qk_scale, site_key(l, SITE_PROBS), ta, sa, b->seed_dev, b->row_index, stream));
      int sp = 0;
      int64_t sstride = 0;
      TRY(mmt_gemm_splitk_geometry(nc, d, d, 0, &sp, &sstride));
      TRY(mmt_gemm_nt_splitk_ex(t.ctx, d, P.wo, d, nullptr, d, nc, d, d, MMT_EPI_F32, nullptr, t.slabs, 0, 0, nullptr, 1, stream));
      TRY(mmt_splitk_ln_fwd(t.slabs, sp, sstride, P.bo, hin32, b->out_rows, nullptr, b->row_index, t.rowidx,
                            site_key(l, SITE_ATTN_OUT), th, sh, b->seed_dev, t.z1, P.ln1_g, P.ln1_b, m->ln_eps, t.a32, t.a16,
                            t.mean1, t.rstd1, nc, d, stream));
      e = {}; e.live_rows_hint = lh;
      e.bias = P.b1; e.out2 = t.g; e.ldout2 = I;
      TRY(mmt_gemm_nt_bf16(t.a16, d, P.w1, d, t.hpre, I, nc, I, d, MMT_EPI_BIAS_GELU, &e, nullptr, stream));
      TRY(mmt_gemm_splitk_geometry(nc, d, I, 0, &sp, &sstride));
      TRY(mmt_gemm_nt_splitk_ex(t.g, I, P.w2, I, nullptr, d, nc, d, I, MMT_EPI_F32, nullptr, t.slabs, 0, 0, nullptr, 1, stream));
      TRY(mmt_splitk_ln_fwd(t.slabs, sp, sstride, P.b2, t.a32, nullptr, t.rowidx, nullptr, nullptr, site_key(l, SITE_FFN_OUT), th,
                            sh, b->seed_dev, t.z2, P.ln2_g, P.ln2_b, m->ln_eps, out_last, nullptr, t.mean2, t.rstd2, nc, d,
                            stream));
      break;
    }
    {
      ProbeScope probe(3, l == 0, stream);
      TRY(mmt_attn_fwd(L.qkv, b->cu_seqlens, b->mask_bias, L.ctx, L.lse, b->batch, b->seq, m->heads, d, qk_scale,
                       site_key(l, SITE_PROBS), ta, sa, b->seed_dev, b->row_index, stream));
    }
    e = {}; e.live_rows_hint = lh;
    e.bias = P.bo; e.res = hin32; e.ldres = d; e.row_index = b->row_index; e.seed_dev = b->seed_dev;
    e.drop_key = site_key(l, SITE_ATTN_OUT); e.drop_thr16 = th; e.drop_scale = sh;
    TRY(mmt_gemm_nt_bf16(L.ctx, d, P.wo, d, L.z1, d, rows, d, d, MMT_EPI_BIAS_DROP_RES, &e, b->n_rows_dev, stream));
    TRY(mmt_ln_fwd(L.z1, P.ln1_g, P.ln1_b, m->ln_eps, L.a32, L.a16, L.mean1, L.rstd1, rows, d, b->n_rows_dev, stream));
    e = {}; e.live_rows_hint = lh;
    e.bias = P.b1; e.out2 = L.g; e.ldout2 = I;
    {
      ProbeScope probe(0, l == 0, stream);
      TRY(mmt_gemm_nt_bf16(L.a16, d, P.w1, d, L.hpre, I, rows, I, d, MMT_EPI_BIAS_GELU, &e, b->n_rows_dev, stream));
    }
    float* hout32 = (l == m->layers - 1) ? out_last : L.h32;
    if (const int splits = short_batch_splits(w, rows, d, I)) {
      int sp = 0;
      int64_t sstride = 0;
      TRY(mmt_gemm_splitk_geometry(rows, d, I, splits, &sp, &sstride));
      {
        ProbeScope probe(1, l == 0, stream);
        TRY(mmt_gemm_nt_splitk_ex(L.g, I, P.w2, I, nullptr, d, rows, d, I, MMT_EPI_F32, nullptr, w.t.slabs, splits, 0,
                                  b->n_rows_dev, 1, stream));
      }
      TRY(mmt_splitk_ln_fwd_ex(w.t.slabs, sp, sstride, P.b2, L.a32, nullptr, nullptr, b->row_index, nullptr,
                               site_key(l, SITE_FFN_OUT), th, sh, b->seed_dev, L.z2, P.ln2_g, P.ln2_b, m->ln_eps, hout32, L.h16,
                               L.mean2, L.rstd2, rows, d, b->n_rows_dev, stream));
    } else {
      e = {}; e.live_rows_hint = lh;
      e.bias = P.b2; e.res = L.a32; e.ldres = d; e.row_index = b->row_index; e.seed_dev = b->seed_dev;
      e.drop_key = site_key(l, SITE_FFN_OUT); e.drop_thr16 = th; e.drop_scale = sh;
      {
        ProbeScope probe(1, l == 0, stream);
        TRY(gemm_hidden(w, rows, d, L.g, I, P.w2, I, L.z2, d, I, MMT_EPI_BIAS_DROP_RES, &e, b->n_rows_dev, stream));
      }
      TRY(mmt_ln_fwd(L.z2, P.ln2_g, P.ln2_b, m->ln_eps, hout32, L.h16, L.mean2, L.rstd2, rows, d, b->n_rows_dev, stream));
    }
    hin32 = hout32;
    hin16 = L.h16;
  }
  return 0;
}

extern "C" int mmt_bert_backward_range(const MmtBertModel* m, const MmtBertBatch* b, void* ws, float* dlast,
                                       float* dfeatures, int training, int l_hi, int l_lo, void* stream) {
  TRY(check_model(m, b));
  const bool embed_only = l_hi == -1 && l_lo == -1;
  if (!ws || !dlast || !dfeatures || l_hi >= m->layers || (!embed_only && (l_lo < 0 || l_lo > l_hi))) return MMT_ERR_ARG;
  Ws w;
  layout(m, b->rows_alloc, (char*)ws, &w);
  const int d = m->hidden, I = m->inter, rows = b->rows;
  const uint32_t th = training ? thr16_of(m->p_hidden) : 0u, ta = training ? thr16_of(m->p_attn) : 0u;
  const float sh = scale_of(th), sa = scale_of(ta);
  const int lh = b->n_rows_dev ? b->live_rows_hint : 0;
  const float qk_scale = m->hidden == m->heads * 128 ? 0.08838834764831845f : 0.125f;
  const int rpb = mmt_ln_bwd_rows_per_block(rows);
  const int ln_blocks = (rows + rpb - 1) / rpb;
  const int32_t* nr = b->n_rows_dev;

  void* side = (b->side_stream && b->side_stream != stream) ? b->side_stream : nullptr;
  const int fork = side ? b->fork : 0;
  const bool fork_w = fork & MMT_FORK_WGRAD, fork_early = fork_w && (fork & MMT_FORK_EARLY);
  const bool fork_r = fork & MMT_FORK_REDUCE, join = fork & MMT_FORK_JOIN;
  void* wstream = fork_w ? side : stream;
  void* rstream = fork_r ? side : stream;
  DoneEvents* done_e = fork_w ? done_entry(ws) : nullptr;
  if (fork_w && !done_e) return MMT_ERR_ARG;
  hipEvent_t* done = done_e ? done_e->ev : nullptr;
  unsigned long long* done_cap = done_e ? done_e->cap : nullptr;

  MmtColReduceJob jobs[2 * 64 + 5];
  int njobs = 0;
  auto add_job = [&](const float* partials, int nblocks, int nvec, int nout, int dd, float* o0, float* o1) {
    MmtColReduceJob& j = jobs[njobs++];
    j = {};
    j.partials = partials; j.nblocks = nblocks; j.nvec = nvec; j.nout = nout; j.d = dd; j.out[0] = o0; j.out[1] = o1;
  };
  auto finish = [&]() -> int {
    if (njobs) {
      if (fork_r) TRY(mmt_stream_fork(stream, side));
      TRY(mmt_col_reduce_multi(jobs, njobs, rstream));
    }
    if (join) TRY(mmt_stream_fork(side, stream));
    return 0;
  };
  const int nc = tail_rows(b, w);
  float* dcur = ((m->layers - 1 - l_hi) & 1) ? w.dA : dlast;
  const float* dc_slabs = nullptr;
  int dc_sp = 0;
  int64_t dc_stride = 0;
  for (int l = l_hi; l >= l_lo && !embed_only; --l) {
    const MmtBertLayer& P = m->layer[l];
    LayerWs& L = w.layer[l];
    const char* hin16 = l ? w.layer[l - 1].h16 : w.h16_in;
    const int par = fork_w ? (l & 1) : 0;
    char *dy = w.dy_[par], *dy2 = w.dy2_[par], *dhpre = w.dhpre_[par], *dqkv = w.dqkv_[par];
    if (fork_w && !join && l + 2 <= m->layers - 1) {
      if (capture_id((hipStream_t)stream) != done_cap[par]) return MMT_ERR_ARG;
      if (hipStreamWaitEvent((hipStream_t)stream, done[par], 0) != hipSuccess) return MMT_ERR_ARG;
    }
    if (nc && l == m->layers - 1) {
      TailWs& t = w.t;
      const int crpb = mmt_ln_bwd_rows_per_block(nc);
      const int cblocks = (nc + crpb - 1) / crpb;
      TRY(mmt_ln_bwd(dlast, t.z2, t.mean2, t.rstd2, P.ln2_g, t.dz, t.dy2, w.ln_partials[2 * l + 2], nc, d, 1, nullptr,
                     t.rowidx, site_key(l, SITE_FFN_OUT), th, sh, b->seed_dev, stream));
      add_job(w.ln_partials[2 * l + 2], cblocks, 3, 2, d, P.g_ln2_g, P.g_ln2_b);
      MmtEpilogue e = {}; e.live_rows_hint = lh;
      e.aux = t.hpre; e.ldaux = I;
      TRY(mmt_gemm_nt_bf16(t.dy2, d, P.w2_t, d, t.dhpre, I, nc, I, d, MMT_EPI_DGELU, &e, nullptr, stream));
      {
        int sp = 0;
        int64_t sstride = 0;
        TRY(mmt_gemm_splitk_geometry(nc, d, I, 0, &sp, &sstride));
        MmtEpilogue er = {}; er.live_rows_hint = lh;
        TRY(mmt_gemm_nt_splitk_ex(t.dhpre, I, P.w1_t, I, nullptr, d, nc, d, I, MMT_EPI_F32, &er, t.slabs, 0, 0, nullptr, 1,
                                  stream));
        TRY(mmt_ln_bwd_slabs(t.slabs, sp, sstride, t.dz, t.z1, t.mean1, t.rstd1, P.ln1_g, t.dz, t.dy, w.ln_partials[2 * l + 1],
                             nc, d, 1, t.rowidx, site_key(l, SITE_ATTN_OUT), th, sh, b->seed_dev, stream));
      }
      add_job(w.ln_partials[2 * l + 1], cblocks, 3, 2, d, P.g_ln1_g, P.g_ln1_b);
      e = {}; e.live_rows_hint = lh;
      e.dot_src = t.ctx; e.lddot = d; e.dot_out = t.delta;
      if (d <= 512) TRY(mmt_gemm_nt_bf16(t.dy, d, P.wo_t, d, t.dctx, d, nc, d, d, MMT_EPI_BF16, &e, nullptr, stream));
      else TRY(mmt_gemm_nt_splitk(t.dy, d, P.wo_t, d, t.dctx, d, nc, d, d, MMT_EPI_BF16, &e, t.slabs, stream));
      TRY(mmt_attn_bwd_rows_ex(L.qkv, b->cu_seqlens, b->mask_bias, b->out_rows, b->n_out_per_sample, t.ctx, t.lse, t.dctx,
                               dqkv, t.delta, 1, b->batch, b->seq, m->heads, d, qk_scale, site_key(l, SITE_PROBS), ta, sa,
                               b->seed_dev, b->row_index, stream));
      if (fork_w) TRY(mmt_stream_fork(stream, side));
      {
        MmtWgradGroup g = {};
        g.count = 4; g.rows = rows; g.n_rows_dev = nr;
        g.item[0].A = dqkv;    g.item[0].lda = 3 * d; g.item[0].B = hin16; g.item[0].ldb = d; g.item[0].N = 3 * d; g.item[0].K2 = d;
        g.item[0].out = P.g_wqkv; g.item[0].bias_out = P.g_bqkv;
        g.item[0].splits = TAIL_WSPLIT; g.item[0].slab = t.wslab; g.item[0].bias_slab = t.bslab;
        g.item[1].A = t.dhpre; g.item[1].lda = I;     g.item[1].B = t.a16; g.item[1].ldb = d; g.item[1].N = I;     g.item[1].K2 = d;
        g.item[1].out = P.g_w1;   g.item[1].bias_out = P.g_b1; g.item[1].reserved = nc;
        g.item[2].A = t.dy2;   g.item[2].lda = d;     g.item[2].B = t.g;   g.item[2].ldb = I; g.item[2].N = d;     g.item[2].K2 = I;
        g.item[2].out = P.g_w2;   g.item[2].bias_out = P.g_b2; g.item[2].reserved = nc;
        g.item[3].A = t.dy;    g.item[3].lda = d;     g.item[3].B = t.ctx; g.item[3].ldb = d; g.item[3].N = d;     g.item[3].K2 = d;
        g.item[3].out = P.g_wo;   g.item[3].bias_out = P.g_bo; g.item[3].reserved = nc;
        TRY(mmt_wgrad_grouped(&g, wstream));
        TRY(mmt_reduce_slabs_pair(t.wslab, (int64_t)3 * d * d, P.g_wqkv, t.bslab, (int64_t)3 * d, P.g_bqkv, TAIL_WSPLIT, wstream));
        if (fork_w) { if (hipEventRecord(done[par], (hipStream_t)side) != hipSuccess) return MMT_ERR_ARG; done_cap[par] = capture_id((hipStream_t)side); }
      }
      e = {}; e.live_rows_hint = lh;
      float* dnext = w.dA;
      TRY(gemm_hidden(w, rows, d, dqkv, 3 * d, P.wqkv_t, 3 * d, dnext, d, 3 * d, MMT_EPI_F32, &e, nr, stream));
      TRY(mmt_rows_scatter(t.dz, b->out_rows, nc, d, dnext, 1, stream));
      dcur = dnext;
      continue;
    }
    MmtWgradGroup gffn = {}, gatt = {};
    gffn.count = 2; gffn.rows = rows; gffn.n_rows_dev = nr;
    gffn.item[0].A = dhpre; gffn.item[0].lda = I;     gffn.item[0].B = L.a16; gffn.item[0].ldb = d; gffn.item[0].N = I;     gffn.item[0].K2 = d;
    gffn.item[0].out = P.g_w1;   gffn.item[0].bias_out = P.g_b1;
    gffn.item[1].A = dy2;   gffn.item[1].lda = d;     gffn.item[1].B = L.g;   gffn.item[1].ldb = I; gffn.item[1].N = d;     gffn.item[1].K2 = I;
    gffn.item[1].out = P.g_w2;   gffn.item[1].bias_out = P.g_b2;
    gatt.count = 2; gatt.rows = rows; gatt.n_rows_dev = nr;
    gatt.item[0].A = dqkv;  gatt.item[0].lda = 3 * d; gatt.item[0].B = hin16; gatt.item[0].ldb = d; gatt.item[0].N = 3 * d; gatt.item[0].K2 = d;
    gatt.item[0].out = P.g_wqkv; gatt.item[0].bias_out = P.g_bqkv;
    gatt.item[1].A = dy;    gatt.item[1].lda = d;     gatt.item[1].B = L.ctx; gatt.item[1].ldb = d; gatt.item[1].N = d;     gatt.item[1].K2 = d;
    gatt.item[1].out = P.g_wo;   gatt.item[1].bias_out = P.g_bo;
    if (dc_slabs) {
      TRY(mmt_ln_bwd_slabs_ex(dc_slabs, dc_sp, dc_stride, w.dz, L.z2, L.mean2, L.rstd2, P.ln2_g, w.dz, dy2, w.ln_partials[2 * l + 2],
                              rows, d, 1, nr, b->row_index, site_key(l, SITE_FFN_OUT), th, sh, b->seed_dev, stream));
      dc_slabs = nullptr;
    } else {
      TRY(mmt_ln_bwd(dcur, L.z2, L.mean2, L.rstd2, P.ln2_g, w.dz, dy2, w.ln_partials[2 * l + 2], rows, d, 1, nr, b->row_index,
                     site_key(l, SITE_FFN_OUT), th, sh, b->seed_dev, stream));
    }
    add_job(w.ln_partials[2 * l + 2], ln_blocks, 3, 2, d, P.g_ln2_g, P.g_ln2_b);
    MmtEpilogue e = {}; e.live_rows_hint = lh;
    e.aux = L.hpre; e.ldaux = I;
    TRY(mmt_gemm_nt_bf16(dy2, d, P.w2_t, d, dhpre, I, rows, I, d, MMT_EPI_DGELU, &e, nr, stream));
    if (fork_early) {
      TRY(mmt_stream_fork(stream, side));
      TRY(mmt_wgrad_grouped(&gffn, side));
    }
    if (const int splits = short_batch_splits(w, rows, d, I)) {
      int sp = 0;
      int64_t sstride = 0;
      TRY(mmt_gemm_splitk_geometry(rows, d, I, splits, &sp, &sstride));
      MmtEpilogue er = {}; er.live_rows_hint = lh;
      TRY(mmt_gemm_nt_splitk_ex(dhpre, I, P.w1_t, I, nullptr, d, rows, d, I, MMT_EPI_F32, &er, w.t.slabs, splits, 0, nr, 1,
                                stream));
      TRY(mmt_ln_bwd_slabs_ex(w.t.slabs, sp, sstride, w.dz, L.z1, L.mean1, L.rstd1, P.ln1_g, w.dz, dy, w.ln_partials[2 * l + 1],
                              rows, d, 1, nr, b->row_index, site_key(l, SITE_ATTN_OUT), th, sh, b->seed_dev, stream));
    } else {
      e = {}; e.live_rows_hint = lh;
      e.res = w.dz; e.ldres = d;
      TRY(gemm_hidden(w, rows, d, dhpre, I, P.w1_t, I, w.dA, d, I, MMT_EPI_ADD_F32, &e, nr, stream));
      TRY(mmt_ln_bwd(w.dA, L.z1, L.mean1, L.rstd1, P.ln1_g, w.dz, dy, w.ln_partials[2 * l + 1], rows, d, 1, nr, b->row_index,
                     site_key(l, SITE_ATTN_OUT), th, sh, b->seed_dev, stream));
    }
    add_job(w.ln_partials[2 * l + 1], ln_blocks, 3, 2, d, P.g_ln1_g, P.g_ln1_b);
    e = {}; e.live_rows_hint = lh;
    e.dot_src = L.ctx; e.lddot = d; e.dot_out = w.delta;
    TRY(mmt_gemm_nt_bf16(dy, d, P.wo_t, d, w.dctx, d, rows, d, d, MMT_EPI_BF16, &e, nr, stream));
    {
      ProbeScope probe(4, l == 0, stream);
      TRY(mmt_attn_bwd_ex(L.qkv, b->cu_seqlens, b->mask_bias, L.ctx, L.lse, w.dctx, dqkv, w.delta, 1, b->batch, b->seq,
                          m->heads, d, qk_scale, site_key(l, SITE_PROBS), ta, sa, b->seed_dev, b->row_index, attn_work_of(m, b, w),
                          stream));
    }
    if (fork_w) {
      TRY(mmt_stream_fork(stream, side));
      if (fork_early) {
        TRY(mmt_wgrad_grouped(&gatt, side));
      } else {
        MmtWgradGroup g = gffn;
        g.count = 4; g.item[2] = gatt.item[0]; g.item[3] = gatt.item[1];
        ProbeScope probe(2, l == 0, side);
        TRY(mmt_wgrad_grouped(&g, side));
      }
      if (hipEventRecord(done[par], (hipStream_t)side) != hipSuccess) return MMT_ERR_ARG;
      done_cap[par] = capture_id((hipStream_t)side);
    }
    e = {}; e.live_rows_hint = lh;
    e.res = w.dz; e.ldres = d;
    float* dnext = (dcur == dlast) ? w.dA : dlast;
    const int qkv_sp = (l > l_lo && !fork_w) ? short_batch_splits(w, rows, d, 3 * d) : 0;
    if (qkv_sp) {
      TRY(mmt_gemm_splitk_geometry(rows, d, 3 * d, qkv_sp, &dc_sp, &dc_stride));
      TRY(mmt_gemm_nt_splitk_ex(dqkv, 3 * d, P.wqkv_t, 3 * d, nullptr, d, rows, d, 3 * d, MMT_EPI_F32, &e, w.t.slabs, qkv_sp, 0, nr, 1,
                                stream));
      dc_slabs = w.t.slabs;
    } else {
      TRY(gemm_hidden(w, rows, d, dqkv, 3 * d, P.wqkv_t, 3 * d, dnext, d, 3 * d, MMT_EPI_ADD_F32, &e, nr, stream));
    }
    if (!fork_w) {
      MmtWgradGroup g = gffn;
      g.count = 4; g.item[2] = gatt.item[0]; g.item[3] = gatt.item[1];
      ProbeScope probe(2, l == 0, stream);
      TRY(mmt_wgrad_grouped(&g, stream));
    }
    dcur = dnext;
  }
  if (!embed_only && (l_lo > 0 || (b->fork & MMT_RANGE_LAYERS_ONLY))) return finish();
  TRY(mmt_ln_bwd(dcur, w.z0, w.mean0, w.rstd0, m->emb_ln_g, dfeatures, nullptr, w.ln_partials[0], rows, d, 2, nr,
                 b->row_index, site_key(0, SITE_EMB), th, sh, b->seed_dev, stream));
  add_job(w.ln_partials[0], ln_blocks, 3, 2, d, m->g_emb_ln_g, m->g_emb_ln_b);
  if (fork_r) TRY(mmt_stream_fork(stream, side));
  const int chunks = mmt_table_grad_chunks();
  const bool pos_partials = b->pos_ids && m->max_pos <= 128;
  if (m->type_vocab <= 128) {
    TRY(mmt_table_grad_partials_pair(dfeatures, b->type_ids, m->type_vocab, w.table_scratch[0],
                                     pos_partials ? b->pos_ids : nullptr, m->max_pos, w.table_scratch[1], rows, d, nr, rstream));
  } else {
    TRY(mmt_table_grad_partials(dfeatures, b->type_ids, rows, d, m->type_vocab, nr, w.table_scratch[0], rstream));
    if (pos_partials) TRY(mmt_table_grad_partials(dfeatures, b->pos_ids, rows, d, m->max_pos, nr, w.table_scratch[1], rstream));
  }
  add_job(w.table_scratch[0], chunks, 1, 1, m->type_vocab * d, m->g_type_emb, nullptr);
  if (pos_partials) add_job(w.table_scratch[1], chunks, 1, 1, m->max_pos * d, m->g_pos_emb, nullptr);
  else if (b->pos_ids)
    TRY(mmt_table_grad_direct(dfeatures, b->pos_ids, rows, d, m->max_pos, nr, m->g_pos_emb, rstream));
  TRY(mmt_col_reduce_multi(jobs, njobs, rstream));
  if (join) TRY(mmt_stream_fork(side, stream));
  return 0;
}

extern "C" int mmt_bert_backward(const MmtBertModel* m, const MmtBertBatch* b, void* ws, float* dlast,
                                 float* dfeatures, int training, void* stream) {
  if (!m) return MMT_ERR_ARG;
  return mmt_bert_backward_range(m, b, ws, dlast, dfeatures, training, m->layers - 1, 0, stream);
}
```

### mmt_amd/csrc/gemm.hip

```cpp
#include "mmt_common.h"
#include "../../include/mmt_hip.h"

#define BK 64

template <int R>
__device__ __forceinline__ void stage_nt(const bf16_t* __restrict__ G, int64_t ld, int row0, int k0,
                                         bf16_t* lds_tile, int wave, int lane) {
#pragma unroll
  for (int i = 0; i < R / 32; ++i) {
    const int rbase = (wave * (R / 32) + i) * 8;
    const int r = rbase + (lane >> 3);
    const int c = (lane & 7) ^ (r & 7);
    const bf16_t* src = G + (int64_t)(row0 + r) * ld + k0 + c * 8;
    __builtin_amdgcn_global_load_lds(GLB_PTR(src), LDS_PTR(lds_tile + rbase * BK), 16, 0, 0);
  }
}

template <int BM, int BN, int EPI>
__global__ __launch_bounds__(256, 2) void gemm_nt_kernel(
    const bf16_t* __restrict__ A, int64_t lda, const bf16_t* __restrict__ B, int64_t ldb,
    void* __restrict__ Cout, int64_t ldc, int M, int N, int K, MmtEpilogue epi,
    const int32_t* __restrict__ n_rows_dev) {
  constexpr int MI = BM / 32, NI = BN / 32;
  __shared__ __attribute__((aligned(16))) bf16_t smem[2 * (BM + BN) * BK];
  const int tiles_n = N / BN;
  const int nrows = n_rows_dev ? *n_rows_dev : M;
  const int live_tiles = min((int)gridDim.x, ((min(nrows, M) + BM - 1) / BM) * tiles_n);
  if ((int)blockIdx.x >= live_tiles) {
    if constexpr (EPI == MMT_EPI_DGELU) {
      const int dtm = (int)blockIdx.x / tiles_n, dn0 = ((int)blockIdx.x % tiles_n) * BN;
      if (epi.colsum && threadIdx.x < BN) epi.colsum[(int64_t)dtm * N + dn0 + threadIdx.x] = 0.f;
    }
    return;
  }
  const int id = xcd_remap(blockIdx.x, live_tiles);
  const int tm = id / tiles_n, tn = id % tiles_n;
  const int m0 = tm * BM, n0 = tn * BN;

  const int tid = threadIdx.x, lane = tid & 63, wave = tid >> 6;
  const int wm = wave >> 1, wn = wave & 1;
  const int li = lane & 15, lg = lane >> 4;

  f32x4 acc[MI][NI];
#pragma unroll
  for (int i = 0; i < MI; ++i)
#pragma unroll
    for (int j = 0; j < NI; ++j) acc[i][j] = (f32x4){0.f, 0.f, 0.f, 0.f};

  constexpr int STAGE = (BM + BN) * BK;

  const int KT = K / BK;
  stage_nt<BM>(A, lda, m0, 0, smem, wave, lane);
  stage_nt<BN>(B, ldb, n0, 0, smem + BM * BK, wave, lane);
  for (int kt = 0; kt < KT; ++kt) {
    const int cur = kt & 1;
    asm volatile("s_waitcnt vmcnt(0)" ::: "memory");
    __syncthreads();
    if (kt + 1 < KT) {
      stage_nt<BM>(A, lda, m0, (kt + 1) * BK, smem + (cur ^ 1) * STAGE, wave, lane);
      stage_nt<BN>(B, ldb, n0, (kt + 1) * BK, smem + (cur ^ 1) * STAGE + BM * BK, wave, lane);
    }
    const bf16_t* as = smem + cur * STAGE;
    const bf16_t* bs = as + BM * BK;
#pragma unroll
    for (int ks = 0; ks < 2; ++ks) {
      bf16x8_t af[MI], bfr[NI];
      const int c = ks * 4 + lg;
#pragma unroll
      for (int i = 0; i < MI; ++i) {
        const int r = wm * (BM / 2) + i * 16 + li;
        af[i] = *(const bf16x8_t*)(as + r * BK + ((c ^ (r & 7)) << 3));
      }
#pragma unroll
      for (int j = 0; j < NI; ++j) {
        const int r = wn * (BN / 2) + j * 16 + li;
        bfr[j] = *(const bf16x8_t*)(bs + r * BK + ((c ^ (r & 7)) << 3));
      }
#pragma unroll
      for (int i = 0; i < MI; ++i)
#pragma unroll
        for (int j = 0; j < NI; ++j)
          acc[i][j] = __builtin_amdgcn_mfma_f32_16x16x32_bf16(bfr[j], af[i], acc[i][j], 0, 0, 0);
    }
  }
// ... 597 lines not shown
    const long t128 = rt128 * (N / 128);
    const bool plain_epi = EPI != MMT_EPI_BIAS_GELU && EPI != MMT_EPI_DGELU && !dot_out;
    if (N < 1024 && N % 128 == 0 && K >= kNarrowLongK && plain_epi && t128 >= kNarrowLongKTiles) return 24;
    if (N < 1024 && packed && rt128 * (N / 64) <= kRoundBlocks) return 18;
    if (N >= 1024 && N % 128 == 0 && K >= 128 && K <= 1024 && t128 >= kWideLiveTiles) return 24;
  }
  if (reserved == 0 && M <= 1024 && !dgelu_sums) return 13;
  if (reserved == 0 && M >= 512) {
    if (N >= 1024 && N % 128 == 0 && !dgelu_sums) return 14;
    if (packed && N % 64 == 0) return 13;
  }
  if (reserved == 0 && M < 512 && N >= 1024 && !dgelu_sums) return 13;
  if (EPI == MMT_EPI_BF16 && dot_out) return 13;
  return (N % 128 == 0 && reserved == 1) ? 1 : 2;
}

extern "C" int mmt_gemm_select_tile(int epilogue, int M, int N, int K, int packed, int live_rows_hint, int has_colsum,
                                    int has_dot_out, int reserved) {
  if (M <= 0 || N <= 0 || K <= 0 || epilogue < 0 || epilogue > MMT_EPI_BIAS_F32) return MMT_ERR_ARG;
  return select_tile(epilogue, M, N, K, packed != 0, live_rows_hint, has_colsum != 0, has_dot_out != 0, reserved);
}

template <int EPI>
static int dispatch_tile(const void* A, int64_t lda, const void* B, int64_t ldb, void* C, int64_t ldc,
                         int M, int N, int K, const MmtEpilogue& e, const int32_t* nr, hipStream_t s) {
  const int t = select_tile(EPI, M, N, K, nr != nullptr, e.live_rows_hint, e.colsum != nullptr, e.dot_out != nullptr, e.reserved);
  if (t >= 3) return mmt_gemm2_dispatch(t, EPI, A, lda, B, ldb, C, ldc, M, N, K, e, nr, s);
  if (t == 1) return launch_nt<128, 128, EPI>(A, lda, B, ldb, C, ldc, M, N, K, e, nr, s);
  return launch_nt<128, 64, EPI>(A, lda, B, ldb, C, ldc, M, N, K, e, nr, s);
}

extern "C" int mmt_gemm_nt_bf16(const void* A, int64_t lda, const void* B, int64_t ldb, void* C,
                                int64_t ldc, int M, int N, int K, int epilogue, const MmtEpilogue* epi,
                                const int32_t* n_rows_dev, void* stream) {
  if (!A || !B || !C || M <= 0 || N <= 0 || K <= 0) return MMT_ERR_ARG;
  if (K % BK || N % 64) return MMT_ERR_ARG;
  if ((lda % 8) || (ldb % 8) || (ldc % 4) || ((uintptr_t)A & 15) || ((uintptr_t)B & 15) || ((uintptr_t)C & 15))
    return MMT_ERR_ALIGN;
  MmtEpilogue e = {};
  if (epi) e = *epi;
  hipStream_t s = (hipStream_t)stream;
  switch (epilogue) {
    case MMT_EPI_BF16:
      if (e.dot_out && !e.dot_src) return MMT_ERR_ARG;
      return dispatch_tile<MMT_EPI_BF16>(A, lda, B, ldb, C, ldc, M, N, K, e, n_rows_dev, s);
    case MMT_EPI_BIAS_BF16:
      if (!e.bias) return MMT_ERR_ARG;
      return dispatch_tile<MMT_EPI_BIAS_BF16>(A, lda, B, ldb, C, ldc, M, N, K, e, n_rows_dev, s);
    case MMT_EPI_BIAS_GELU:
      if (!e.bias || !e.out2) return MMT_ERR_ARG;
      return dispatch_tile<MMT_EPI_BIAS_GELU>(A, lda, B, ldb, C, ldc, M, N, K, e, n_rows_dev, s);
    case MMT_EPI_BIAS_DROP_RES:
      if (!e.bias || !e.res) return MMT_ERR_ARG;
      return dispatch_tile<MMT_EPI_BIAS_DROP_RES>(A, lda, B, ldb, C, ldc, M, N, K, e, n_rows_dev, s);
    case MMT_EPI_DGELU:
      if (!e.aux) return MMT_ERR_ARG;
      return dispatch_tile<MMT_EPI_DGELU>(A, lda, B, ldb, C, ldc, M, N, K, e, n_rows_dev, s);
    case MMT_EPI_ADD_F32:
      if (!e.res) return MMT_ERR_ARG;
      return dispatch_tile<MMT_EPI_ADD_F32>(A, lda, B, ldb, C, ldc, M, N, K, e, n_rows_dev, s);
    case MMT_EPI_F32: return dispatch_tile<MMT_EPI_F32>(A, lda, B, ldb, C, ldc, M, N, K, e, n_rows_dev, s);
    case MMT_EPI_BIAS_F32:
      if (!e.bias) return MMT_ERR_ARG;
      return dispatch_tile<MMT_EPI_BIAS_F32>(A, lda, B, ldb, C, ldc, M, N, K, e, n_rows_dev, s);
  }
  return MMT_ERR_ARG;
}

extern "C" int mmt_gemm_tn_bf16(const void* A, int64_t lda, const void* B, int64_t ldb, float* ws,
                                int rows, int N, int K2, int splits, const int32_t* n_rows_dev,
                                void* stream) {
  if (!A || !B || !ws || rows <= 0 || N <= 0 || K2 <= 0 || splits <= 0) return MMT_ERR_ARG;
  if (N % 128 || K2 % 128) return MMT_ERR_ARG;
  if ((lda % 8) || (ldb % 8) || ((uintptr_t)A & 15) || ((uintptr_t)B & 15) || ((uintptr_t)ws & 15))
    return MMT_ERR_ALIGN;
  const int grid = (N / 128) * (K2 / 128) * splits;
  hipLaunchKernelGGL(gemm_tn_kernel, dim3(grid), dim3(256), 0, (hipStream_t)stream, (const bf16_t*)A, lda,
                     (const bf16_t*)B, ldb, ws, rows, N, K2, splits, n_rows_dev);
  return (int)hipGetLastError();
}

__global__ void reduce_slabs_pair_kernel(const float* __restrict__ wa, int64_t ca4, float* __restrict__ oa,
                                         const float* __restrict__ wb, int64_t cb4, float* __restrict__ ob, int splits) {
  for (int64_t i = blockIdx.x * (int64_t)blockDim.x + threadIdx.x; i < ca4 + cb4; i += (int64_t)gridDim.x * blockDim.x) {
    const bool first = i < ca4;
    const f32x4* ws = (const f32x4*)(first ? wa : wb);
    const int64_t j = first ? i : i - ca4, c4 = first ? ca4 : cb4;
    f32x4 s = ws[j];
    for (int k = 1; k < splits; ++k) s += ws[k * c4 + j];
    ((f32x4*)(first ? oa : ob))[j] = s;
  }
}

extern "C" int mmt_reduce_slabs_pair(const float* ws_a, int64_t count_a, float* out_a, const float* ws_b, int64_t count_b,
                                     float* out_b, int splits, void* stream) {
  if (!ws_a || !out_a || !ws_b || !out_b || splits <= 0 || count_a <= 0 || count_b <= 0 || ((count_a | count_b) & 3))
    return MMT_ERR_ARG;
  const int64_t c4 = (count_a + count_b) / 4;
  const int grid = (int)((c4 + 255) / 256 < 2048 ? (c4 + 255) / 256 : 2048);
  hipLaunchKernelGGL(reduce_slabs_pair_kernel, dim3(grid), dim3(256), 0, (hipStream_t)stream, ws_a, count_a / 4, out_a, ws_b,
                     count_b / 4, out_b, splits);
  return (int)hipGetLastError();
}

extern "C" int mmt_reduce_slabs(const float* ws, int splits, int64_t count, float* out, int accumulate,
                                void* stream) {
  if (!ws || !out || splits <= 0 || count <= 0 || (count & 3)) return MMT_ERR_ARG;
  const int64_t c4 = count / 4;
  const int grid = (int)((c4 + 255) / 256 < 2048 ? (c4 + 255) / 256 : 2048);
  hipLaunchKernelGGL(reduce_slabs_kernel, dim3(grid), dim3(256), 0, (hipStream_t)stream, ws, splits, c4,
                     out, accumulate);
  return (int)hipGetLastError();
}
```

### mmt_amd/csrc/norm.hip

```cpp
#include "mmt_common.h"
#include "attn_sched.h"
#include "../../include/mmt_hip.h"

#define MAXC 4

template <bool EMBED>
__global__ __launch_bounds__(256) void ln_fwd_kernel(
    const float* __restrict__ z_in, const int32_t* __restrict__ type_ids, const int32_t* __restrict__ pos_ids,
    const float* __restrict__ type_emb, const float* __restrict__ pos_emb, float* __restrict__ z_save,
    const float* __restrict__ gamma, const float* __restrict__ beta, float eps, float* __restrict__ h32,
    bf16_t* __restrict__ h16, float* __restrict__ mean_out, float* __restrict__ rstd_out, int rows, int d,
    const int32_t* __restrict__ n_rows_dev, const int32_t* __restrict__ row_index, uint32_t drop_key_in,
    uint32_t thr16, float drop_scale, const uint32_t* __restrict__ seed_dev, const int32_t* __restrict__ dst_rows,
    int ln_blocks, AttnSched sched) {
  if (EMBED && (int)blockIdx.x >= ln_blocks) {
    if (sched.work) attn_schedule_block(sched);
    return;
  }
  const int lane = threadIdx.x & 63, wave = threadIdx.x >> 6;
  const int nrows = n_rows_dev ? min(*n_rows_dev, rows) : rows;
  const int nch = d >> 8;
  const unsigned drop_key = eff_key(drop_key_in, seed_dev);
  for (int row = blockIdx.x * 4 + wave; row < nrows; row += ln_blocks * 4) {
    const int64_t hrow = dst_rows ? dst_rows[row] : row;
    f32x4 x[MAXC];
    float s = 0.f;
#pragma unroll
    for (int c = 0; c < MAXC; ++c) {
      if (c < nch) {
        const int col = c * 256 + lane * 4;
        x[c] = *(const f32x4*)(z_in + (int64_t)row * d + col);
        if constexpr (EMBED) {
          x[c] += *(const f32x4*)(type_emb + (int64_t)type_ids[row] * d + col);
          if (pos_ids) x[c] += *(const f32x4*)(pos_emb + (int64_t)pos_ids[row] * d + col);
          if (z_save) *(f32x4*)(z_save + (int64_t)row * d + col) = x[c];
        }
        s += x[c][0] + x[c][1] + x[c][2] + x[c][3];
      }
    }
    const float mean = wave_sum(s) / (float)d;
    float v = 0.f;
#pragma unroll
    for (int c = 0; c < MAXC; ++c)
      if (c < nch) {
#pragma unroll
        for (int k = 0; k < 4; ++k) { const float t = x[c][k] - mean; v += t * t; }
      }
    const float rstd = 1.0f / sqrtf(wave_sum(v) / (float)d + eps);
    if (lane == 0) { mean_out[row] = mean; rstd_out[row] = rstd; }
    const int orow = row_index ? row_index[row] : row;
#pragma unroll
    for (int c = 0; c < MAXC; ++c)
      if (c < nch) {
        const int col = c * 256 + lane * 4;
        const f32x4 g = *(const f32x4*)(gamma + col), b = *(const f32x4*)(beta + col);
        f32x4 y;
#pragma unroll
        for (int k = 0; k < 4; ++k) y[k] = (x[c][k] - mean) * rstd * g[k] + b[k];
        if constexpr (EMBED) {
          if (thr16) {
            bool kp[4];
            keep4(drop_key, (unsigned long long)orow * (unsigned)d + (unsigned)col, thr16, kp);
#pragma unroll
            for (int k = 0; k < 4; ++k) y[k] = kp[k] ? y[k] * drop_scale : 0.f;
          }
        }
        if (h32) *(f32x4*)(h32 + hrow * d + col) = y;
        u32x2 o = {pack_bf2(y[0], y[1]), pack_bf2(y[2], y[3])};
        if (h16) *(u32x2*)(h16 + (int64_t)row * d + col) = o;
      }
  }
}

struct SplitkLnArgs {
  const float* slabs; int splits; int64_t slab_stride;
  const float *bias, *res; const int32_t *res_rows, *rowidx, *row_index; int32_t* rowidx_out;
  uint32_t drop_key, thr16; float drop_scale; const uint32_t* seed_dev;
  float* z_out; const float *gamma, *beta; float eps;
  float* h32; bf16_t* h16; float *mean, *rstd;
  int rows, d;
  const int32_t* n_rows_dev;
};
__global__ __launch_bounds__(256) void splitk_ln_fwd_kernel(SplitkLnArgs a) {
  const int lane = threadIdx.x & 63, wave = threadIdx.x >> 6;
  const int row = blockIdx.x * 4 + wave;
// ... 201 lines not shown
          dbias[c][2] += bf2f((bf16_t)(o[1] & 0xffff)); dbias[c][3] += bf2f((bf16_t)(o[1] >> 16));
        }
      }
  }
#pragma unroll
  for (int c = 0; c < NCH; ++c)
    {
      const int col = c * 256 + lane * 4;
      *(f32x4*)(red_raw + (wave * 3 + 0) * d + col) = dg[c];
      *(f32x4*)(red_raw + (wave * 3 + 1) * d + col) = db[c];
      *(f32x4*)(red_raw + (wave * 3 + 2) * d + col) = dbias[c];
    }
  __syncthreads();
  for (int e = threadIdx.x; e < 3 * d / 4; e += 64 * LNB_WAVES) {
    f32x4 acc = *(const f32x4*)(red_raw + e * 4);
#pragma unroll
    for (int w = 1; w < LNB_WAVES; ++w) acc += *(const f32x4*)(red_raw + w * 3 * d + e * 4);
    *(f32x4*)(partials + (int64_t)blockIdx.x * 3 * d + e * 4) = acc;
  }
}

struct ColOuts { float* p[4]; };
#define CR_RG 16
__global__ __launch_bounds__(64 * CR_RG) void col_reduce_kernel(const float* __restrict__ partials, int nblocks, int nvec,
                                                                int d, ColOuts outs, int accumulate) {
  __shared__ float red[CR_RG][64];
  const int chunks = (d + 63) / 64;
  const int j = blockIdx.x / chunks, c = (blockIdx.x % chunks) * 64 + (threadIdx.x & 63);
  const int rg = threadIdx.x >> 6;
  float* out = outs.p[j];
  float s = 0.f;
  if (out && c < d)
    for (int b = rg; b < nblocks; b += CR_RG) s += partials[((int64_t)b * nvec + j) * d + c];
  red[rg][threadIdx.x & 63] = s;
  __syncthreads();
  if (rg == 0 && out && c < d) {
    const int t = threadIdx.x;
    float v = 0.f;
#pragma unroll
    for (int g = 0; g < CR_RG; ++g) v += red[g][t];
    out[c] = accumulate ? out[c] + v : v;
  }
}

struct ColJobs { MmtColReduceJob job[MMT_COLRED_MAX]; int begin[MMT_COLRED_MAX]; int count; };
__global__ __launch_bounds__(64 * CR_RG) void col_reduce_multi_kernel(ColJobs jobs) {
  __shared__ float red[CR_RG][64];
  int p = 0;
#pragma unroll 1
  for (int q = 1; q < jobs.count; ++q)
    if ((int)blockIdx.x >= jobs.begin[q]) p = q;
  const MmtColReduceJob& jb = jobs.job[p];
  const int bid = (int)blockIdx.x - jobs.begin[p];
  const int d = jb.d, nvec = jb.nvec, nblocks = jb.nblocks;
  const int chunks = (d + 63) / 64;
  const int j = bid / chunks, c = (bid % chunks) * 64 + (threadIdx.x & 63);
  const int rg = threadIdx.x >> 6;
  float* out = jb.out[j];
  const float* __restrict__ partials = jb.partials;
  float s = 0.f;
  if (out && c < d) {
    float s1 = 0.f, s2 = 0.f, s3 = 0.f;
    int b = rg;
    for (; b + 3 * CR_RG < nblocks; b += 4 * CR_RG) {
      s += partials[((int64_t)b * nvec + j) * d + c];
      s1 += partials[((int64_t)(b + CR_RG) * nvec + j) * d + c];
      s2 += partials[((int64_t)(b + 2 * CR_RG) * nvec + j) * d + c];
      s3 += partials[((int64_t)(b + 3 * CR_RG) * nvec + j) * d + c];
    }
    for (; b < nblocks; b += CR_RG) s += partials[((int64_t)b * nvec + j) * d + c];
    s = (s + s1) + (s2 + s3);
  }
  red[rg][threadIdx.x & 63] = s;
  __syncthreads();
  if (rg == 0 && out && c < d) {
    const int t = threadIdx.x;
    float v = 0.f;
#pragma unroll
    for (int g = 0; g < CR_RG; ++g) v += red[g][t];
    out[c] = v;
  }
}

#define TABLE_CHUNKS 64
__global__ __launch_bounds__(256) void table_grad_kernel(
    const float* __restrict__ g, const int32_t* __restrict__ ids, int rows, int d, int vocab,
    const int32_t* __restrict__ n_rows_dev, float* __restrict__ partial) {
  const int v = blockIdx.x, col = blockIdx.y * 256 + threadIdx.x, chunk = blockIdx.z;
  const int nrows = n_rows_dev ? min(*n_rows_dev, rows) : rows;
  const int per = (nrows + TABLE_CHUNKS - 1) / TABLE_CHUNKS;
  const int r_begin = chunk * per, r_end = min(nrows, r_begin + per);
  __shared__ int32_t sid[256];
  float s = 0.f;
  for (int r0 = r_begin; r0 < r_end; r0 += 256) {
    const int r = r0 + threadIdx.x;
    sid[threadIdx.x] = r < r_end ? ids[r] : -1;
    __syncthreads();
    const int lim = min(256, r_end - r0);
    for (int k = 0; k < lim; ++k)
      if (sid[k] == v) s += g[(int64_t)(r0 + k) * d + col];
    __syncthreads();
  }
  partial[((int64_t)chunk * vocab + v) * d + col] = s;
}

typedef __attribute__((ext_vector_type(16))) float f32x16_t;
struct TablePair { const int32_t* ids[2]; float* partial[2]; int vocab[2]; };
#define TG_ROWS 64
template <int NU>
__global__ __launch_bounds__(256) void table_grad_mfma_kernel(const float* __restrict__ g, TablePair tp, int rows, int d,
                                                              const int32_t* __restrict__ n_rows_dev) {
  __shared__ __attribute__((aligned(16))) float gt[TG_ROWS][128 + 4];
  __shared__ int32_t idt[2][TG_ROWS];
  const int tid = threadIdx.x, lane = tid & 63, wave = tid >> 6, l31 = lane & 31, h = lane >> 5;
  const int cb = blockIdx.x * 128, chunk = blockIdx.y;
  const int nrows = n_rows_dev ? min(*n_rows_dev, rows) : rows;
  const int per = (nrows + TABLE_CHUNKS - 1) / TABLE_CHUNKS;
  const int r_begin = chunk * per, r_end = min(nrows, r_begin + per);
  const int ntab = tp.ids[1] ? 2 : 1;
  f32x16_t acc[2][NU];
#pragma unroll
  for (int t = 0; t < 2; ++t)
#pragma unroll
    for (int u = 0; u < NU; ++u)
#pragma unroll
      for (int r = 0; r < 16; ++r) acc[t][u][r] = 0.f;
  for (int r0 = r_begin; r0 < r_end; r0 += TG_ROWS) {
#pragma unroll
    for (int i = 0; i < TG_ROWS * 32 / 256; ++i) {
      const int e = i * 256 + tid, rr = e >> 5, c4 = (e & 31) * 4;
      f32x4 v = {0.f, 0.f, 0.f, 0.f};
      if (r0 + rr < r_end) v = *(const f32x4*)(g + (int64_t)(r0 + rr) * d + cb + c4);
      *(f32x4*)(&gt[rr][c4]) = v;
    }
    if (tid < 2 * TG_ROWS) {
      const int t = tid / TG_ROWS, rr = tid % TG_ROWS;
      idt[t][rr] = (t < ntab && r0 + rr < r_end) ? tp.ids[t][r0 + rr] : -1;
    }
    __syncthreads();
#pragma unroll
    for (int t = 0; t < 2; ++t) {
      if (t >= ntab) continue;
#pragma unroll
      for (int u = 0; u < NU; ++u) {
        if (u * 32 >= tp.vocab[t]) continue;
        const int myv = u * 32 + l31;
#pragma unroll 8
        for (int kk = 0; kk < TG_ROWS / 2; ++kk) {
          const int k = 2 * kk + h;
          acc[t][u] = __builtin_amdgcn_mfma_f32_32x32x2f32(idt[t][k] == myv ? 1.0f : 0.0f, gt[k][wave * 32 + l31], acc[t][u], 0, 0, 0);
        }
      }
    }
    __syncthreads();
  }
#pragma unroll
  for (int t = 0; t < 2; ++t) {
    if (t >= ntab) continue;
#pragma unroll
    for (int u = 0; u < NU; ++u)
#pragma unroll
      for (int r = 0; r < 16; ++r) {
        const int v = u * 32 + (r & 3) + 8 * (r >> 2) + 4 * h;
        if (v < tp.vocab[t]) tp.partial[t][((int64_t)chunk * tp.vocab[t] + v) * d + cb + wave * 32 + l31] = acc[t][u][r];
      }
  }
}

static inline int ln_grid(int rows) {
  int g = (rows + 3) / 4;
  return g < 1 ? 1 : (g > 4096 ? 4096 : g);
}

extern "C" int mmt_ln_fwd(const float* z, const float* gamma, const float* beta, float eps, float* h32,
                          void* h16, float* mean, float* rstd, int rows, int d, const int32_t* n_rows_dev,
                          void* stream) {
  if (!z || !gamma || !beta || !h16 || !mean || !rstd || rows <= 0) return MMT_ERR_ARG;
  if (d % 256 || d > MAXC * 256) return MMT_ERR_ARG;
  hipLaunchKernelGGL(ln_fwd_kernel<false>, dim3(ln_grid(rows)), dim3(256), 0, (hipStream_t)stream, z,
                     nullptr, nullptr, nullptr, nullptr, nullptr, gamma, beta, eps, h32, (bf16_t*)h16, mean,
                     rstd, rows, d, n_rows_dev, nullptr, 0u, 0u, 1.0f, nullptr, nullptr, ln_grid(rows), AttnSched{});
  return (int)hipGetLastError();
}

extern "C" int mmt_ln_fwd_scatter(const float* z, const float* gamma, const float* beta, float eps, float* h32,
                                  const int32_t* dst_rows, void* h16, float* mean, float* rstd, int rows, int d,
                                  void* stream) {
  if (!z || !gamma || !beta || !h32 || !dst_rows || !mean || !rstd || rows <= 0) return MMT_ERR_ARG;
  if (d % 256 || d > MAXC * 256) return MMT_ERR_ARG;
  hipLaunchKernelGGL(ln_fwd_kernel<false>, dim3(ln_grid(rows)), dim3(256), 0, (hipStream_t)stream, z,
                     nullptr, nullptr, nullptr, nullptr, nullptr, gamma, beta, eps, h32, (bf16_t*)h16, mean,
                     rstd, rows, d, nullptr, nullptr, 0u, 0u, 1.0f, nullptr, dst_rows, ln_grid(rows), AttnSched{});
  return (int)hipGetLastError();
}

__global__ __launch_bounds__(256) void row_move_kernel(const float* __restrict__ src, float* __restrict__ dst,
                                                       const int32_t* __restrict__ rows, int n, int d, int scatter,
                                                       const int32_t* __restrict__ idx_in, int32_t* __restrict__ idx_out) {
  const int lane = threadIdx.x & 63, wave = threadIdx.x >> 6;
  for (int i = blockIdx.x * 4 + wave; i < n; i += gridDim.x * 4) {
    const int64_t r = rows[i];
    const float* s = scatter ? src + (int64_t)i * d : src + r * d;
    float* t = scatter ? dst + r * d : dst + (int64_t)i * d;
    if (scatter == 2) {
      for (int c = lane * 4; c < d; c += 256) *(f32x4*)(t + c) += *(const f32x4*)(s + c);
    } else {
      for (int c = lane * 4; c < d; c += 256) *(f32x4*)(t + c) = *(const f32x4*)(s + c);
    }
    if (!scatter && idx_out && lane == 0) idx_out[i] = idx_in ? idx_in[r] : (int32_t)r;
  }
}

extern "C" int mmt_rows_gather(const float* src, const int32_t* rows, int n, int d, float* dst, const int32_t* idx_in,
                               int32_t* idx_out, void* stream) {
  if (!src || !rows || !dst || n <= 0 || d <= 0 || (d & 3)) return MMT_ERR_ARG;
  hipLaunchKernelGGL(row_move_kernel, dim3((n + 3) / 4), dim3(256), 0, (hipStream_t)stream, src, dst, rows, n, d, 0, idx_in,
                     idx_out);
  return (int)hipGetLastError();
}
extern "C" int mmt_rows_scatter(const float* src, const int32_t* rows, int n, int d, float* dst, int accumulate,
                                void* stream) {
  if (!src || !rows || !dst || n <= 0 || d <= 0 || (d & 3)) return MMT_ERR_ARG;
  hipLaunchKernelGGL(row_move_kernel, dim3((n + 3) / 4), dim3(256), 0, (hipStream_t)stream, src, dst, rows, n, d,
                     accumulate ? 2 : 1, nullptr, nullptr);
  return (int)hipGetLastError();
}

__global__ __launch_bounds__(256) void table_grad_direct_kernel(const float* __restrict__ g, const int32_t* __restrict__ ids,
                                                                int rows, int d, const int32_t* __restrict__ n_rows_dev,
                                                                float* __restrict__ out) {
  const int v = blockIdx.x, c = threadIdx.x * 4;
  const int n = n_rows_dev ? min(rows, *n_rows_dev) : rows;
  if (c >= d) return;
  f32x4 acc = {0.f, 0.f, 0.f, 0.f};
  for (int r = 0; r < n; ++r)
    if (ids[r] == v) acc += *(const f32x4*)(g + (int64_t)r * d + c);
  *(f32x4*)(out + (int64_t)v * d + c) = acc;
}

extern "C" int mmt_table_grad_direct(const float* g, const int32_t* ids, int rows, int d, int vocab,
                                     const int32_t* n_rows_dev, float* dtable, void* stream) {
  if (!g || !ids || !dtable || rows <= 0 || vocab <= 0 || d <= 0 || (d & 3) || d > 1024) return MMT_ERR_ARG;
  hipLaunchKernelGGL(table_grad_direct_kernel, dim3(vocab), dim3(256), 0, (hipStream_t)stream, g, ids, rows, d, n_rows_dev,
                     dtable);
  return (int)hipGetLastError();
}

__global__ __launch_bounds__(256) void embedding_grad_kernel(const float* __restrict__ g, const int32_t* __restrict__ ids,
                                                             int n, int d, int vocab, int padding_idx,
                                                             const int32_t* __restrict__ n_rows_dev,
                                                             float* __restrict__ dtable) {
  const int i = blockIdx.x;
  if (n_rows_dev) n = min(n, *n_rows_dev);
  if (i >= n) return;
  const int id = ids[i];
  if (id < 0 || id >= vocab || id == padding_idx) return;
  int seen = 0;
  for (int j = threadIdx.x; j < i; j += 256) seen |= (ids[j] == id);
  if (__syncthreads_or(seen)) return;
  for (int c = threadIdx.x * 4; c < d; c += 1024) {
    f32x4 acc = *(const f32x4*)(g + (int64_t)i * d + c);
    for (int j = i + 1; j < n; ++j)
      if (ids[j] == id) acc += *(const f32x4*)(g + (int64_t)j * d + c);
    *(f32x4*)(dtable + (int64_t)id * d + c) = acc;
  }
}

extern "C" int mmt_embedding_grad(const float* g, const int32_t* ids, int n, int d, int vocab, int padding_idx,
                                  const int32_t* n_rows_dev, float* dtable, void* stream) {
  if (!g || !ids || !dtable || n <= 0 || d <= 0 || (d & 3) || vocab <= 0) return MMT_ERR_ARG;
  hipLaunchKernelGGL(embedding_grad_kernel, dim3(n), dim3(256), 0, (hipStream_t)stream, g, ids, n, d, vocab, padding_idx,
                     n_rows_dev, dtable);
  return (int)hipGetLastError();
}

extern "C" int mmt_embed_ln_fwd_sched(const float* features, const int32_t* type_ids, const int32_t* pos_ids,
                                const float* type_emb, const float* pos_emb, float* z_save,
                                const float* gamma, const float* beta, float eps, float* h32, void* h16,
                                float* mean, float* rstd, int rows, int d, const int32_t* n_rows_dev,
                                const int32_t* row_index, uint32_t drop_key, uint32_t thr16, float drop_scale,
                                const uint32_t* seed_dev, const int32_t* sched_cu, int sched_B, int sched_H, int sched_tiles,
                                      int32_t* sched_work, void* stream) {
  if (!features || !type_ids || !type_emb || !gamma || !beta || !h16 || !mean || !rstd || rows <= 0)
    return MMT_ERR_ARG;
  if (pos_ids && !pos_emb) return MMT_ERR_ARG;
  if (d % 256 || d > MAXC * 256) return MMT_ERR_ARG;
  const AttnSched sc = {sched_cu, sched_work, sched_B, sched_H, sched_tiles};
  hipLaunchKernelGGL(ln_fwd_kernel<true>, dim3(ln_grid(rows) + (sched_work ? 1 : 0)), dim3(256), 0, (hipStream_t)stream, features,
                     type_ids, pos_ids, type_emb, pos_emb, z_save, gamma, beta, eps, h32, (bf16_t*)h16, mean,
                     rstd, rows, d, n_rows_dev, row_index, drop_key, thr16, drop_scale, seed_dev, nullptr, ln_grid(rows), sc);
  return (int)hipGetLastError();
}
extern "C" int mmt_embed_ln_fwd(const float* features, const int32_t* type_ids, const int32_t* pos_ids,
// ... 146 lines not shown
```

### mmt_amd/model.py

```python
import collections
import ctypes
import re
import types

import torch
import torch.nn.functional as F
from torch import nn

from . import _lib, ops
from ._lib import MmtExpertIO, MmtTextHeads, MmtTextHeadsOpts, MmtVideoFront, MmtVideoSrc, check
from .bert import BertModel, EngineBatch
from .feature_store import RaggedFeatures
from .flat import FlatParams


def _round_up(x, m):
  return (x + m - 1) // m * m


class ReduceDim(nn.Module):

  def __init__(self, input_dimension, output_dimension):
    super().__init__()
    self.fc = nn.Linear(input_dimension, output_dimension)

  def forward(self, x):
    return F.normalize(self.fc(x), dim=-1)


class ContextGating(nn.Module):

  def __init__(self, dimension, add_batch_norm=True):
    super().__init__()
    self.fc = nn.Linear(dimension, dimension)
    self.add_batch_norm = add_batch_norm
    self.batch_norm = nn.BatchNorm1d(dimension)

  def forward(self, x):
    x1 = self.fc(x)
    if self.add_batch_norm:
      x1 = self.batch_norm(x1)
    return F.glu(torch.cat((x, x1), 1), 1)


class GatedEmbeddingUnit(nn.Module):

  def __init__(self, input_dimension, output_dimension, use_bn, normalize):
    super().__init__()
    self.fc = nn.Linear(input_dimension, output_dimension)
    self.cg = ContextGating(output_dimension, add_batch_norm=use_bn)
    self.normalize = normalize

  def forward(self, x):
    x = self.cg(self.fc(x))
    if self.normalize:
      x = F.normalize(x, dim=-1)
    return x


class _VideoTokensFn(torch.autograd.Function):

  @staticmethod
  def forward(ctx, net, plan, *params):
    ctx.net, ctx.plan, ctx.generation = net, plan, plan.generation
    return net._video_tokens_forward(plan)

  @staticmethod
  def backward(ctx, dfeat):
    if ctx.plan.generation != ctx.generation:
      raise RuntimeError('mmt_amd.CENet: video-token buffers were overwritten by a later forward')
    return (None, None) + tuple(ctx.net._video_tokens_backward(ctx.plan, dfeat.contiguous()))


class _ReadoutFn(torch.autograd.Function):

  @staticmethod
  def forward(ctx, last, agg_row, bm, compact=False, stash=None):
    ctx.compact = compact
    d = last.shape[1]
    out = torch.empty(bm, d, device=last.device, dtype=torch.float32)
    inv = torch.empty(bm, device=last.device, dtype=torch.float32)
    check(_lib.lib().mmt_readout_fwd(ops._p(last), ops._p(agg_row), bm, d, ops._p(out), ops._p(inv), ops._stream()),
          'mmt_readout_fwd')
    ctx.save_for_backward(out, inv, agg_row)
    ctx.shape = last.shape
    if stash is not None:
      stash.update(readout_inv=inv, readout_rows=None if compact else agg_row, readout_compact=compact)
    return out

  @staticmethod
  def backward(ctx, dout):
    out, inv, agg_row = ctx.saved_tensors
    dlast = (torch.empty if ctx.compact else torch.zeros)(ctx.shape, device=out.device, dtype=torch.float32)
# ... 31 lines not shown
class _MoeDropoutFn(torch.autograd.Function):
  SITE_KEY = 0x7e57d0a1

  @staticmethod
  def forward(ctx, x, p, seed_dev):
    x = x.contiguous().float()
    y = torch.empty_like(x)
    ctx.key = torch.empty(1, dtype=torch.int32, device=x.device)
    ctx.thr, ctx.scale = ops.dropout_params(p)
    check(_lib.lib().mmt_dropout_f32(ops._p(x), ops._p(y), x.numel(), _MoeDropoutFn.SITE_KEY, ctx.thr, ctx.scale,
                                     ops._p(seed_dev), ops._p(ctx.key), None, ops._stream()), 'mmt_dropout_f32')
    return y

  @staticmethod
  def backward(ctx, g):
    g = g.contiguous().float()
    gx = torch.empty_like(g)
    check(_lib.lib().mmt_dropout_f32(ops._p(g), ops._p(gx), g.numel(), _MoeDropoutFn.SITE_KEY, ctx.thr, ctx.scale, None,
                                     None, ops._p(ctx.key), ops._stream()), 'mmt_dropout_f32')
    return gx, None, None


class _TextHeadsFn(torch.autograd.Function):

  @staticmethod
  def forward(ctx, net, text, text_moe, caps, moe_drop_p, *params):
    tm = None if text_moe is None else text_moe.detach().contiguous().float()
    out = net._text_heads_forward(text.detach().contiguous().float(), tm, caps, moe_drop_p)
    ctx.net, ctx.caps, ctx.generation, ctx.training = net, caps, net._th_generation, net.training
    ctx.need_dtext = text.requires_grad
    ctx.need_dmoe = text_moe is not None and text_moe.requires_grad
    net._th_needs_input_grad = ctx.need_dtext or ctx.need_dmoe
    return out

  @staticmethod
  def backward(ctx, de, dtw):
    net = ctx.net
    if net._th_generation != ctx.generation:
      raise RuntimeError('mmt_amd.CENet: text-head buffers were overwritten by a later forward')
    dtext, dmoe, grads = net._text_heads_backward(ctx.caps, de, dtw, ctx.need_dtext, ctx.need_dmoe, ctx.training)
    return (None, dtext, dmoe, None, None) + tuple(grads)


def cross_view_similarity(vid_embds, text_embds, vid_weights, text_weights, merge='avg'):
  b, m, d = vid_embds.shape
  c = text_embds.shape[2]
  dev = vid_embds.device
  on_cpu = not vid_embds.is_cuda
  if on_cpu:
    if not torch.cuda.is_available():
      raise RuntimeError('mmt_amd similarity needs a GPU (no CPU fallback)')
    vid_embds, text_embds, vid_weights, text_weights = (x.cuda() for x in (vid_embds, text_embds, vid_weights,
                                                                           text_weights))
  txt = text_embds.permute(0, 2, 1, 3).reshape(b * c, m, d)
  sims = _SimsFn.apply(txt, vid_embds, text_weights.reshape(b * c, m), vid_weights.reshape(b, m))
  if c > 1:
    if merge == 'avg':
      sims = sims.view(b, c, b).mean(1)
    elif merge != 'indep':
      raise ValueError('unrecognised merge mode: {}'.format(merge))
  return sims.to(dev) if on_cpu else sims


def sharded_cross_view_inner_product(vid_embds, text_embds, vid_weights, text_weights, subspaces,
                                     merge_caption_similiarities='avg'):
  vid = torch.stack([vid_embds[mod] for mod in subspaces], 1)
  b = vid.shape[0]
  txt = torch.stack([text_embds[mod].reshape(b, -1, vid.shape[-1]) for mod in subspaces], 1)
  c = txt.shape[2]
  return cross_view_similarity(vid, txt, vid_weights.reshape(b, -1), text_weights.reshape(b, c, -1),
                               merge_caption_similiarities)


class _VideoPlan:
  KSPLIT = 768

  def __init__(self, net, bsz, t, device):
    mods, dims = net.modalities, net.expert_dims
    m = len(mods)
    self.batch, self.tokens, self.seq = bsz, t, 1 + m * (t + 1)
    self.rows = bsz * self.seq
    self.rows_alloc = ops.pad_rows(self.rows)
    self.generation = 0
    self.front_done = -1
    i32 = dict(device=device, dtype=torch.int32)
    self.counts = torch.zeros(bsz, **i32)
    self.cu = torch.zeros(bsz + 1, **i32)
    self.n_rows = torch.zeros(1, **i32)
    self.slot = torch.zeros(self.rows, **i32)
    self.row_index = torch.zeros(self.rows_alloc, **i32)
    self.type_ids = torch.zeros(self.rows_alloc, **i32)
    self.pos_ids = torch.zeros(self.rows_alloc, **i32)
    self.mask_bias = torch.zeros(self.rows_alloc, device=device, dtype=torch.float32)
    self.agg_row = torch.zeros(bsz * m, **i32)
    self.src_row = torch.zeros(self.rows_alloc, **i32)
    self.src_cnt = torch.zeros(m, **i32)
    self.xsrc = torch.zeros(m, bsz * t, **i32)
    self.src = MmtVideoSrc()
    self.src.src_row, self.src.src_cnt, self.src.xsrc = (x.data_ptr() for x in (self.src_row, self.src_cnt, self.xsrc))
    self.compact_rows = None
    self.features = None
    self.src_rows = bsz * (t + 1)
    self.src_rows_pad = _round_up(self.src_rows, 128)
    d = net.same_dim
    self.x, self.y, self.dy, self.y_part = {}, {}, {}, {}
    self.zero_bias = torch.zeros(d, device=device, dtype=torch.float32)
    chunks = {mod: min(3, -(-_round_up(dims[mod]['dim'], 128) // self.KSPLIT)) for mod in mods}
    if sum(chunks.values()) > 16:
      chunks = {mod: 1 for mod in mods}
    self.xin = {}
    self.precast = False
    for mod in mods:
      dpad = _round_up(dims[mod]['dim'], 128)
      self.x[mod] = torch.zeros(self.src_rows_pad, dpad, device=device, dtype=torch.bfloat16)
      self.y[mod] = torch.zeros(self.src_rows_pad, d, device=device, dtype=torch.float32)
      self.dy[mod] = torch.zeros(self.src_rows_pad, d, device=device, dtype=torch.bfloat16)
      self.y_part[mod] = [torch.zeros(self.src_rows_pad, d, device=device, dtype=torch.float32)
                          for _ in range(chunks[mod] - 1)]
    self.io = (MmtExpertIO * m)()
    self.inputs = None


class CENet(nn.Module):

  def __init__(self, l2renorm, expert_dims, tokenizer, keep_missing_modalities, test_caption_mode,
               freeze_weights=False, mimic_ce_dims=False, concat_experts=False, concat_mix_experts=False,
               use_experts='origfeat', txt_inp=None, txt_agg=None, txt_pro=None, txt_wgh=None, vid_inp=None,
               vid_cont=None, vid_wgh=None, pos_enc=None, out_tok=None, use_mask='nomask', same_dim=512,
               vid_bert_params=None, txt_bert_params=None, agg_dims=None, normalize_experts=True,
               txt_bert=None, pack_tokens=True):
    super().__init__()
    self.expert_dims = expert_dims
    self.modalities = list(expert_dims.keys())
    self.test_caption_mode = test_caption_mode
    self.keep_missing_modalities = keep_missing_modalities
    self.l2renorm, self.same_dim = l2renorm, same_dim
    self.txt_inp, self.txt_agg, self.txt_pro, self.txt_wgh = txt_inp, txt_agg, txt_pro, txt_wgh
    self.vid_inp, self.vid_cont, self.vid_wgh = vid_inp, vid_cont, vid_wgh
    self.pos_enc, self.out_tok = pos_enc, out_tok
    self.vid_bert_params = vid_bert_params
    self.normalize_experts = normalize_experts
    self.pack_tokens = pack_tokens
    self.tail_rows_only = True
    self._vid_weights = {}
    self.live_rows_hint = None
    self.text_live_rows_hint = None
    self.overlap_text_heads = False
    self._side_streams = {}
    type_vocab = (vid_bert_params or {}).get('type_vocab_size')
    if type_vocab is not None:
      bad = [m for m, e in expert_dims.items() if not 0 <= e['idx'] < type_vocab]
      if bad:
        raise IndexError('expert type ids of %r do not fit vid_bert_params.type_vocab_size = %d' % (bad, type_vocab))
    unsupported = []
    if vid_cont != 'bert': unsupported.append('vid_cont=%r' % vid_cont)
    if vid_inp != 'both': unsupported.append('vid_inp=%r' % vid_inp)
    if out_tok != 'mxp': unsupported.append('out_tok=%r' % out_tok)
    if pos_enc not in ('tint', 'none'): unsupported.append('pos_enc=%r' % pos_enc)
    if vid_wgh != 'none': unsupported.append('vid_wgh=%r' % vid_wgh)
    if not keep_missing_modalities: unsupported.append('keep_missing_modalities=False')
    if not normalize_experts: unsupported.append('normalize_experts=False')
    if txt_pro not in ('gbn', 'gem', 'lin'): unsupported.append('txt_pro=%r' % txt_pro)
    if txt_wgh not in ('emb', 'none'): unsupported.append('txt_wgh=%r' % txt_wgh)
    if unsupported:
      raise NotImplementedError('mmt_amd.CENet implements the published MMT configuration natively; '
                                'unsupported: ' + ', '.join(unsupported))
# ... 111 lines not shown
    return out

  @staticmethod
  def count_live_rows(features_ind):
    first = next(iter(features_ind.values()))
    total = int(first.shape[0])
    for ind in features_ind.values():
      total += int(ind.shape[0]) + int((torch.as_tensor(ind) != 0).sum())
    return total

  @staticmethod
  def count_live_tokens(token_ids):
    return int((torch.as_tensor(token_ids)[..., 1] != 0).sum())

  def engine_params(self):
    return self._flat.params

  def flats(self):
    out = [self._flat]
    if self._native_text_tower:
      out.append(self.txt_bert.build_flat())
    return out

  def _reduce_params(self):
    out = []
    for mod in self.modalities:
      out += [self.video_dim_reduce[mod].fc.weight, self.video_dim_reduce[mod].fc.bias]
    return out

  def _prepare(self, device):
    if self._flat.ensure(device):
      self.vid_bert._structs = {}
      self._th_ws = {}
    self._flat.pack()
    if torch.is_grad_enabled():
      self._flat.select_grad_buffer()
    self.vid_bert._ensure_ready(device)

  def _video_tokens_forward(self, plan):
    L, m, d = _lib.lib(), len(self.modalities), self.same_dim
    io, stream = plan.io, ops._stream()
    max_pos = self.vid_bert_params['max_position_embeddings'] - 1
    vb = self.vid_bert
    bump = vb._seed_dev if (plan.bump_seed and vb._seed_dev is not None) else None
    vb._seed_bumped = bump is not None
    if plan.front_done != plan.generation:
      check(L.mmt_video_plan(io, m, plan.batch, plan.tokens, int(self.pack_tokens), max_pos, ops._p(plan.counts),
                             ops._p(plan.cu), ops._p(plan.n_rows), ops._p(plan.slot), ops._p(plan.row_index),
                             ops._p(plan.type_ids), ops._p(plan.pos_ids), ops._p(plan.mask_bias), ops._p(plan.agg_row),
                             ops._p(bump), ctypes.byref(plan.src), stream), 'mmt_video_plan')
      if not plan.precast:
        check(L.mmt_video_cast(io, m, plan.batch, plan.tokens, ctypes.byref(plan.src), stream), 'mmt_video_cast')
    items, index = [], []
    for i, mod in enumerate(self.modalities):
      x, w = plan.xin[mod], self._flat.shadow(('reduce', mod))[0]
      outs = [plan.y[mod]] + plan.y_part[mod]
      step = _round_up(-(-x.shape[1] // len(outs)), 64)
      for c, out in enumerate(outs):
        k0 = c * step
        k1 = x.shape[1] if c == len(outs) - 1 else k0 + step
        items.append((x[:, k0:k1], w[:, k0:k1], out, self.video_dim_reduce[mod].fc.bias if c == 0 else plan.zero_bias))
        index.append(i)
    ops.gemm_nt_grouped(items, m=plan.src_rows, n_rows_dev=plan.src_cnt, n_rows_index=index)
    feats = torch.empty(plan.rows_alloc, d, device=plan.slot.device, dtype=torch.float32)
    check(L.mmt_video_scatter(io, m, plan.batch, plan.tokens, d, ops._p(plan.n_rows), ops._p(plan.row_index),
                              ctypes.byref(plan.src), ops._p(feats), stream), 'mmt_video_scatter')
    return feats

  def _video_front(self, plan):
    vb = self.vid_bert
    bump = vb._seed_dev if (plan.bump_seed and vb._seed_dev is not None) else None
    f = MmtVideoFront()
    f.experts = ctypes.addressof(plan.io)
    f.M, f.B, f.T, f.pack = len(self.modalities), plan.batch, plan.tokens, int(self.pack_tokens)
    f.max_pos, f.do_cast = self.vid_bert_params['max_position_embeddings'] - 1, int(not plan.precast)
    for name, t in (('counts', plan.counts), ('cu_seqlens', plan.cu), ('n_rows_dev', plan.n_rows), ('slot', plan.slot),
                    ('row_index', plan.row_index), ('type_ids', plan.type_ids), ('pos_ids', plan.pos_ids),
                    ('mask_bias', plan.mask_bias), ('agg_row', plan.agg_row)):
      setattr(f, name, t.data_ptr())
    f.seed_bump = bump.data_ptr() if bump is not None else None
    f.src = ctypes.addressof(plan.src)
    return f

  def _video_tokens_backward(self, plan, dfeat, side_stream=None):
    L, m, d = _lib.lib(), len(self.modalities), self.same_dim
    stream = ops._stream()
    check(L.mmt_video_scatter_bwd(plan.io, m, plan.batch, plan.tokens, d, ops._p(plan.n_rows), ops._p(plan.row_index),
                                  ctypes.byref(plan.src), ops._p(dfeat), stream), 'mmt_video_scatter_bwd')
    grad_buf = self._flat.current_grad()
    grads, items = [], []
    for mod in self.modalities:
      fc = self.video_dim_reduce[mod].fc
      gw, gb = self._flat.view(fc.weight, grad_buf), self._flat.view(fc.bias, grad_buf)
      items.append((plan.dy[mod], plan.xin[mod], gw, gb))
      grads += [gw if fc.weight.requires_grad else None, gb if fc.bias.requires_grad else None]
    if side_stream is not None:
      side_stream.wait_stream(torch.cuda.current_stream())
      with torch.cuda.stream(side_stream):
        ops.wgrad_grouped(items, plan.src_rows, item_rows_dev=plan.src_cnt)
    else:
      ops.wgrad_grouped(items, plan.src_rows, item_rows_dev=plan.src_cnt)
    return grads

  def video_embeddings(self, features, features_t, features_ind, features_maxpool, plan=None):
    if plan is None:
      plan = self._video_prepare(features, features_t, features_ind, features_maxpool)
    mods, bsz, dev = self.modalities, plan.batch, plan.slot.device
    feats = _VideoTokensFn.apply(self, plan, *self._reduce_params())
    batch = EngineBatch(None, plan.type_ids, plan.pos_ids if self.pos_enc != 'none' else None, plan.mask_bias,
                        plan.rows, bsz, plan.seq, cu_seqlens=plan.cu,
                        row_index=plan.row_index if self.pack_tokens else None,
                        n_rows_dev=plan.n_rows if self.pack_tokens else None,
                        out_rows=plan.agg_row if self.tail_rows_only else None, n_out_per_sample=len(mods))
    hint = self.live_rows_hint
    if hint is None and isinstance(features, RaggedFeatures):
      hint = bsz + sum(int(v) for v in features.live.values())
    batch.live_rows_hint = int(hint or 0) if self.pack_tokens else 0
    last = self.vid_bert.run_engine(batch, feats)
    self._stages = dict(plan=plan, feats=feats, batch=batch, last=last) if last.requires_grad else None
    if self.vid_bert.compact_output(batch, plan.rows_alloc):
      if plan.compact_rows is None:
        plan.compact_rows = torch.arange(bsz * len(mods), device=dev, dtype=torch.int32)
      vid = _ReadoutFn.apply(last, plan.compact_rows, bsz * len(mods), True, self._stages)
    else:
      vid = _ReadoutFn.apply(last, plan.agg_row, bsz * len(mods), False, self._stages)
    vid = vid.view(bsz, len(mods), self.same_dim)
    if self._stages is not None:
      self._stages['vid_embds'] = vid
    return vid

  def _video_prepare(self, features, features_t, features_ind, features_maxpool):
    mods = self.modalities
    ragged = features if isinstance(features, RaggedFeatures) else None
    if ragged is not None:
      if not self.pack_tokens:
        raise NotImplementedError('RaggedFeatures carry no padded rows: they need pack_tokens=True')
      if [n for n, _ in ragged.layout.experts] != mods or any(
          d != self.expert_dims[n]['dim'] for n, d in ragged.layout.experts):
        raise ValueError('RaggedFeatures experts %r do not match the model\'s %r' % (ragged.layout.experts, mods))
      dev, bsz, t = ragged.device, ragged.batch, ragged.tokens
      if dev.type != 'cuda':
        raise RuntimeError('mmt_amd.CENet runs on the GPU only (no CPU fallback)')
      features_ind, features_t = ragged.ind, ragged.t
    else:
      f0 = features[mods[0]]
      if not f0.is_cuda:
        raise RuntimeError('mmt_amd.CENet runs on the GPU only (no CPU fallback)')
      dev = f0.device
      bsz, t = f0.shape[0], f0.shape[1]
      for mod in mods:
        if features[mod].shape[1] != t:
          raise NotImplementedError('all experts must share max_expert_tokens (as in every published config)')
    self._prepare(dev)
    key = (bsz, t, dev)
    plan = self._plans.get(key)
    if plan is None:
      plan = self._plans[key] = _VideoPlan(self, bsz, t, dev)
    plan.generation += 1
    keep = []
    for i, mod in enumerate(mods):
      io = plan.io[i]
      if ragged is not None:
        tensors = [x.detach().to(device=dev, dtype=torch.float32).contiguous() for x in (features_ind[mod], features_t[mod])]
        x = ragged.x[mod]
        if x.shape != plan.x[mod].shape:
          raise ValueError('RaggedFeatures layout does not match the model (rows/K padding)')
        keep.append(tensors + [x])
        io.feat = io.maxpool = None
        io.ind, io.t = (v.data_ptr() for v in tensors)
      else:
        tensors = [features[mod], features_maxpool[mod], features_ind[mod], features_t[mod]]
        tensors = [x.detach().to(device=dev, dtype=torch.float32).contiguous() for x in tensors]
        keep.append(tensors)
        x = plan.x[mod]
        io.feat, io.maxpool, io.ind, io.t = (v.data_ptr() for v in tensors)
      plan.xin[mod] = x
      io.x, io.y, io.dy = x.data_ptr(), plan.y[mod].data_ptr(), plan.dy[mod].data_ptr()
      io.D, io.Dpad = self.expert_dims[mod]['dim'], x.shape[1]
      io.n_part = len(plan.y_part[mod])
      for c, part in enumerate(plan.y_part[mod]):
        io.y_part[c] = part.data_ptr()
      io.type_idx, io.rows_pad = self.expert_dims[mod]['idx'], plan.src_rows_pad
    plan.inputs = keep
    plan.precast = ragged is not None
    plan.bump_seed = self.vid_bert.training and torch.is_grad_enabled()
    return plan

  def _text_head_params(self):
    out = [self.text_GU[mod].fc.weight for mod in self.modalities]
    for mod in self.modalities:
      gu = self.text_GU[mod]
      out += [gu.fc.bias, gu.cg.fc.weight, gu.cg.fc.bias, gu.cg.batch_norm.weight, gu.cg.batch_norm.bias]
    if self.txt_wgh == 'emb':
      for mod in self.modalities:
        out += [self.moe_fc_txt[mod].weight, self.moe_fc_txt[mod].bias]
    return out

  def _text_heads_struct(self, grad_buf):
    f, h = self._flat, MmtTextHeads()
    for i, mod in enumerate(self.modalities):
# ... 194 lines not shown
```

Before: 25410 pairs/s.

## Co-launch independent backward kernels into single grids to cut launch count

Merges independent backward kernels into combined launches that partition blocks by index. The qkv slab reduction now shares a grid with the tail rows scatter when no weight-grad side stream is used. The embedding table-grad MFMA kernel shares a grid with the video scatter backward, which moves from the Python tokens backward into the engine. This removes separate kernel launches and serialization gaps on the stream, but adds argument plumbing and a path where the scatter is skipped in Python and depends on the engine running it.

```diff
diff --git a/include/mmt_hip.h b/include/mmt_hip.h
--- a/include/mmt_hip.h
+++ b/include/mmt_hip.h
@@ -126,6 +126,9 @@
 int mmt_rows_gather(const float* src, const int32_t* rows, int n, int d, float* dst, const int32_t* idx_in,
                     int32_t* idx_out, void* stream);
 int mmt_rows_scatter(const float* src, const int32_t* rows, int n, int d, float* dst, int accumulate, void* stream);
+int mmt_reduce_slabs_pair_rows_scatter(const float* ws_a, int64_t count_a, float* out_a, const float* ws_b, int64_t count_b,
+                                       float* out_b, int splits, const float* src, const int32_t* rows, int n, int d,
+                                       float* dst, int accumulate, void* stream);
 int mmt_table_grad_direct(const float* g, const int32_t* ids, int rows, int d, int vocab, const int32_t* n_rows_dev,
                           float* dtable, void* stream);
 int mmt_embedding_grad(const float* g, const int32_t* ids, int n, int d, int vocab, int padding_idx,
@@ -261,6 +264,17 @@
                       const int32_t* row_index, const MmtVideoSrc* src, float* features, void* stream);
 int mmt_video_scatter_bwd(const MmtExpertIO* experts, int M, int B, int T, int d, const int32_t* n_rows_dev,
                           const int32_t* row_index, const MmtVideoSrc* src, const float* dfeatures, void* stream);
+typedef struct MmtVideoScatterBwd {
+  const MmtExpertIO* experts;
+  int32_t M, B, T, d;
+  const int32_t* n_rows_dev;
+  const int32_t* row_index;
+  const MmtVideoSrc* src;
+} MmtVideoScatterBwd;
+int mmt_video_scatter_bwd_desc_bytes(void);
+int mmt_table_grad_pair_scatter_bwd(const float* g, const int32_t* ids0, int vocab0, float* scratch0, const int32_t* ids1,
+                                    int vocab1, float* scratch1, int rows, int d, const int32_t* n_rows_dev,
+                                    const MmtVideoScatterBwd* sc, void* stream);
 
 int mmt_readout_fwd(const float* last_hidden, const int32_t* agg_row, int BM, int d, float* vid_embds,
                     float* inv_norm, void* stream);
@@ -520,6 +534,8 @@
                       int training, void* stream);
 int mmt_bert_backward_range(const MmtBertModel* m, const MmtBertBatch* b, void* ws, float* dlast, float* dfeatures,
                             int training, int l_hi, int l_lo, void* stream);
+int mmt_bert_backward_range_scatter(const MmtBertModel* m, const MmtBertBatch* b, void* ws, float* dlast, float* dfeatures,
+                                    int training, int l_hi, int l_lo, const MmtVideoScatterBwd* scatter, void* stream);
 
 int mmt_probe_arm(void** start_events, void** stop_events, int n);
 int mmt_probe_arm_site(int site, void** start_events, void** stop_events, int n);
diff --git a/mmt_amd/_lib.py b/mmt_amd/_lib.py
--- a/mmt_amd/_lib.py
+++ b/mmt_amd/_lib.py
@@ -56,6 +56,11 @@
               ('D', ctypes.c_int32), ('Dpad', ctypes.c_int32), ('type_idx', ctypes.c_int32),
               ('rows_pad', ctypes.c_int32), ('y_part', c_vp * 2), ('n_part', ctypes.c_int32),
               ('reserved', ctypes.c_int32)]
+
+
+class MmtVideoScatterBwd(ctypes.Structure):
+  _fields_ = [('experts', c_vp), ('M', ctypes.c_int32), ('B', ctypes.c_int32), ('T', ctypes.c_int32), ('d', ctypes.c_int32),
+              ('n_rows_dev', c_vp), ('row_index', c_vp), ('src', c_vp)]
 
 
 _LAYER_PTRS = ['wqkv', 'wqkv_t', 'wo', 'wo_t', 'w1', 'w1_t', 'w2', 'w2_t',
@@ -191,6 +196,8 @@
     'mmt_ln_fwd_scatter': (c_int, [c_vp, c_vp, c_vp, c_f32, c_vp, c_vp, c_vp, c_vp, c_vp, c_int, c_int, c_vp]),
     'mmt_rows_gather': (c_int, [c_vp, c_vp, c_int, c_int, c_vp, c_vp, c_vp, c_vp]),
     'mmt_rows_scatter': (c_int, [c_vp, c_vp, c_int, c_int, c_vp, c_int, c_vp]),
+    'mmt_reduce_slabs_pair_rows_scatter': (c_int, [c_vp, c_i64, c_vp, c_vp, c_i64, c_vp, c_int, c_vp, c_vp, c_int, c_int, c_vp,
+                                                   c_int, c_vp]),
     'mmt_embedding_grad': (c_int, [c_vp, c_vp, c_int, c_int, c_int, c_int, c_vp, c_vp, c_vp]),
     'mmt_text_plan': (c_int, [c_vp, c_vp, c_vp, c_vp, c_int, c_int, c_vp, c_vp, c_vp, c_vp, c_vp, c_vp, c_vp, c_vp, c_vp]),
     'mmt_table_grad_direct': (c_int, [c_vp, c_vp, c_int, c_int, c_int, c_vp, c_vp, c_vp]),
@@ -211,6 +218,9 @@
                                   ctypes.POINTER(MmtVideoSrc), c_vp, c_vp]),
     'mmt_video_scatter_bwd': (c_int, [ctypes.POINTER(MmtExpertIO), c_int, c_int, c_int, c_int, c_vp, c_vp,
                                       ctypes.POINTER(MmtVideoSrc), c_vp, c_vp]),
+    'mmt_video_scatter_bwd_desc_bytes': (c_int, []),
+    'mmt_table_grad_pair_scatter_bwd': (c_int, [c_vp, c_vp, c_int, c_vp, c_vp, c_int, c_vp, c_int, c_int, c_vp,
+                                                ctypes.POINTER(MmtVideoScatterBwd), c_vp]),
     'mmt_readout_fwd': (c_int, [c_vp, c_vp, c_int, c_int, c_vp, c_vp, c_vp]),
     'mmt_readout_bwd': (c_int, [c_vp, c_vp, c_vp, c_vp, c_int, c_int, c_vp, c_vp]),
     'mmt_sims_fwd': (c_int, [c_vp, c_vp, c_vp, c_vp, c_int, c_int, c_int, c_int, c_vp, c_vp, c_vp]),
@@ -290,6 +300,8 @@
                                   c_vp]),
     'mmt_bert_backward_range': (c_int, [ctypes.POINTER(MmtBertModel), ctypes.POINTER(MmtBertBatch), c_vp, c_vp, c_vp,
                                         c_int, c_int, c_int, c_vp]),
+    'mmt_bert_backward_range_scatter': (c_int, [ctypes.POINTER(MmtBertModel), ctypes.POINTER(MmtBertBatch), c_vp, c_vp,
+                                                c_vp, c_int, c_int, c_int, ctypes.POINTER(MmtVideoScatterBwd), c_vp]),
     'mmt_stream_fork': (c_int, [c_vp, c_vp]),
     'mmt_sgemm_batched': (c_int, [ctypes.POINTER(MmtSgemm), c_vp]),
     'mmt_text_heads_workspace_floats': (c_i64, [c_int, c_int, c_int]),
diff --git a/mmt_amd/bert.py b/mmt_amd/bert.py
--- a/mmt_amd/bert.py
+++ b/mmt_amd/bert.py
@@ -106,6 +106,7 @@
     self.out_rows, self.n_out_per_sample = out_rows, n_out_per_sample
     self.save = False
     self.side_stream, self.fork = None, 0
+    self.scatter_bwd = None
 
 
 class _BertFn(torch.autograd.Function):
@@ -330,9 +331,10 @@
       b = self._batch_struct(batch, rows_alloc)
       if not embed:
         b.fork |= _lib.RANGE_LAYERS_ONLY
-      check(L.mmt_bert_backward_range(ctypes.byref(m), ctypes.byref(b), ws.data_ptr(), dlast.data_ptr(),
-                                      dfeat.data_ptr(), int(training), int(l_hi), int(l_lo), ops._stream()),
-            'mmt_bert_backward_range')
+      sc = ctypes.byref(batch.scatter_bwd) if getattr(batch, 'scatter_bwd', None) is not None else None
+      check(L.mmt_bert_backward_range_scatter(ctypes.byref(m), ctypes.byref(b), ws.data_ptr(), dlast.data_ptr(),
+                                              dfeat.data_ptr(), int(training), int(l_hi), int(l_lo), sc, ops._stream()),
+            'mmt_bert_backward_range_scatter')
 
     run.dfeat, run.keep = dfeat, (dlast, ws, m)
     return run
diff --git a/mmt_amd/csrc/assemble.hip b/mmt_amd/csrc/assemble.hip
--- a/mmt_amd/csrc/assemble.hip
+++ b/mmt_amd/csrc/assemble.hip
@@ -1,6 +1,7 @@
 #include "mmt_common.h"
 #include "../../include/mmt_hip.h"
 #include "video_front.h"
+#include "colaunch.h"
 
 __global__ __launch_bounds__(256) void video_plan_kernel(VideoPlanArgs p) {
   extern __shared__ float plan_ind_s[];
@@ -26,52 +27,22 @@
                                                       const int32_t* __restrict__ n_rows_dev,
                                                       const int32_t* __restrict__ row_index, MmtVideoSrc src,
                                                       float* __restrict__ feat, const float* __restrict__ dfeat) {
-  const int lane = threadIdx.x & 63, wave = threadIdx.x >> 6;
-  const int nrows = n_rows_dev ? min(*n_rows_dev, rows) : rows;
-  const int nch = d >> 8;
-  for (int row = blockIdx.x * 4 + wave; row < nrows; row += gridDim.x * 4) {
-    const int s = row_index[row] % S;
-    if (s == 0) {
-      if constexpr (!BWD)
-        for (int c = lane * 4; c < d; c += 256) *(f32x4*)(feat + (int64_t)row * d + c) = (f32x4){0.f, 0.f, 0.f, 0.f};
-      continue;
-    }
-    const MmtExpertIO e = tab.e[(s - 1) / (T + 1)];
-    const int64_t r = src.src_row[row];
-    f32x4 y[4];
-    float ss = 0.f;
-#pragma unroll
-    for (int c = 0; c < 4; ++c)
-      if (c < nch) {
-        y[c] = *(const f32x4*)(e.y + r * d + c * 256 + lane * 4);
-        if (e.n_part > 0) y[c] += *(const f32x4*)(e.y_part[0] + r * d + c * 256 + lane * 4);
-        if (e.n_part > 1) y[c] += *(const f32x4*)(e.y_part[1] + r * d + c * 256 + lane * 4);
-        ss += y[c][0] * y[c][0] + y[c][1] * y[c][1] + y[c][2] * y[c][2] + y[c][3] * y[c][3];
-      }
-    const float nrm = sqrtf(wave_sum(ss));
-    const float inv = 1.0f / fmaxf(nrm, 1e-12f);
-    if constexpr (!BWD) {
-#pragma unroll
-      for (int c = 0; c < 4; ++c)
-        if (c < nch) *(f32x4*)(feat + (int64_t)row * d + c * 256 + lane * 4) = y[c] * inv;
-    } else {
-      f32x4 g[4];
-      float dot = 0.f;
-#pragma unroll
-      for (int c = 0; c < 4; ++c)
-        if (c < nch) {
-          g[c] = *(const f32x4*)(dfeat + (int64_t)row * d + c * 256 + lane * 4);
-          dot += g[c][0] * y[c][0] + g[c][1] * y[c][1] + g[c][2] * y[c][2] + g[c][3] * y[c][3];
-        }
-      const float proj = nrm > 1e-12f ? wave_sum(dot) * inv * inv : 0.f;
-#pragma unroll
-      for (int c = 0; c < 4; ++c)
-        if (c < nch) {
-          f32x4 dyv = (g[c] - y[c] * proj) * inv;
-          u32x2 o = {pack_bf2(dyv[0], dyv[1]), pack_bf2(dyv[2], dyv[3])};
-          *(u32x2*)((bf16_t*)e.dy + r * d + c * 256 + lane * 4) = o;
-        }
-    }
+  video_scatter_block<BWD>((int)blockIdx.x, (int)gridDim.x, tab, M, T, S, d, rows, n_rows_dev, row_index, src, feat, dfeat);
+}
+
+__global__ __launch_bounds__(256) void table_grad_scatter_bwd_kernel(const float* __restrict__ g, TablePair tp, int rows, int d,
+                                                                     const int32_t* __restrict__ n_rows_dev, int ntg,
+                                                                     ExpertTable tab, int M, int T, int S, int sc_rows,
+                                                                     const int32_t* __restrict__ sc_n_rows_dev,
+                                                                     const int32_t* __restrict__ row_index, MmtVideoSrc src) {
+  __shared__ __attribute__((aligned(16))) float gt[TG_ROWS][128 + 4];
+  __shared__ int32_t idt[2][TG_ROWS];
+  const int bid = (int)blockIdx.x;
+  if (bid < ntg) {
+    const int gx = d / 128;
+    table_grad_mfma_block<2>(bid % gx, bid / gx, gt, idt, g, tp, rows, d, n_rows_dev);
+  } else {
+    video_scatter_block<true>(bid - ntg, (int)gridDim.x - ntg, tab, M, T, S, d, sc_rows, sc_n_rows_dev, row_index, src, nullptr, g);
   }
 }
 
@@ -180,3 +151,32 @@
                      n_rows_dev, row_index, *src, nullptr, dfeatures);
   return (int)hipGetLastError();
 }
+
+static int check_scatter_bwd(const MmtVideoScatterBwd* sc, ExpertTable& tab) {
+  if (!sc) return MMT_ERR_ARG;
+  if (int e = make_table(sc->experts, sc->M, tab)) return e;
+  if (int e = check_src(sc->src)) return e;
+  if (!sc->row_index || sc->B <= 0 || sc->T <= 0 || sc->d % 256 || sc->d <= 0 || sc->d > 1024) return MMT_ERR_ARG;
+  for (int i = 0; i < sc->M; ++i)
+    if (!sc->experts[i].dy) return MMT_ERR_ARG;
+  return 0;
+}
+
+extern "C" int mmt_video_scatter_bwd_desc_bytes(void) { return (int)sizeof(MmtVideoScatterBwd); }
+
+extern "C" int mmt_table_grad_pair_scatter_bwd(const float* g, const int32_t* ids0, int vocab0, float* scratch0,
+                                               const int32_t* ids1, int vocab1, float* scratch1, int rows, int d,
+                                               const int32_t* n_rows_dev, const MmtVideoScatterBwd* sc, void* stream) {
+  if (!g || !ids0 || !scratch0 || rows <= 0 || vocab0 <= 0 || vocab0 > 64 || d <= 0 || d % 128) return MMT_ERR_ARG;
+  if (ids1 && (!scratch1 || vocab1 <= 0 || vocab1 > 64)) return MMT_ERR_ARG;
+  ExpertTable tab;
+  if (int e = check_scatter_bwd(sc, tab)) return e;
+  if (sc->d != d) return MMT_ERR_ARG;
+  TablePair tp = {{ids0, ids1}, {scratch0, scratch1}, {vocab0, vocab1}};
+  const int S = 1 + sc->M * (sc->T + 1), sc_rows = sc->B * S;
+  if (sc_rows > rows) return MMT_ERR_ARG;
+  const int ntg = (d / 128) * TABLE_CHUNKS, grid = ntg + (sc_rows + 3) / 4;
+  hipLaunchKernelGGL(table_grad_scatter_bwd_kernel, dim3(grid), dim3(256), 0, (hipStream_t)stream, g, tp, rows, d, n_rows_dev,
+                     ntg, tab, sc->M, sc->T, S, sc_rows, sc->n_rows_dev, sc->row_index, *sc->src);
+  return (int)hipGetLastError();
+}
diff --git a/mmt_amd/csrc/bert_engine.hip b/mmt_amd/csrc/bert_engine.hip
--- a/mmt_amd/csrc/bert_engine.hip
+++ b/mmt_amd/csrc/bert_engine.hip
@@ -283,9 +283,18 @@
 
 extern "C" int mmt_bert_backward_range(const MmtBertModel* m, const MmtBertBatch* b, void* ws, float* dlast,
                                        float* dfeatures, int training, int l_hi, int l_lo, void* stream) {
+  return mmt_bert_backward_range_scatter(m, b, ws, dlast, dfeatures, training, l_hi, l_lo, nullptr, stream);
+}
+
+extern "C" int mmt_bert_backward_range_scatter(const MmtBertModel* m, const MmtBertBatch* b, void* ws, float* dlast,
+                                               float* dfeatures, int training, int l_hi, int l_lo,
+                                               const MmtVideoScatterBwd* scatter, void* stream) {
   TRY(check_model(m, b));
   const bool embed_only = l_hi == -1 && l_lo == -1;
   if (!ws || !dlast || !dfeatures || l_hi >= m->layers || (!embed_only && (l_lo < 0 || l_lo > l_hi))) return MMT_ERR_ARG;
+  if (scatter && (scatter->d != m->hidden || scatter->M <= 0 || scatter->B <= 0 || scatter->T <= 0 ||
+                  (int64_t)scatter->B * (1 + (int64_t)scatter->M * (scatter->T + 1)) > b->rows))
+    return MMT_ERR_ARG;
   Ws w;
   layout(m, b->rows_alloc, (char*)ws, &w);
   const int d = m->hidden, I = m->inter, rows = b->rows;
@@ -380,13 +389,21 @@
         g.item[3].A = t.dy;    g.item[3].lda = d;     g.item[3].B = t.ctx; g.item[3].ldb = d; g.item[3].N = d;     g.item[3].K2 = d;
         g.item[3].out = P.g_wo;   g.item[3].bias_out = P.g_bo; g.item[3].reserved = nc;
         TRY(mmt_wgrad_grouped(&g, wstream));
-        TRY(mmt_reduce_slabs_pair(t.wslab, (int64_t)3 * d * d, P.g_wqkv, t.bslab, (int64_t)3 * d, P.g_bqkv, TAIL_WSPLIT, wstream));
-        if (fork_w) { if (hipEventRecord(done[par], (hipStream_t)side) != hipSuccess) return MMT_ERR_ARG; done_cap[par] = capture_id((hipStream_t)side); }
+        if (fork_w) {
+          TRY(mmt_reduce_slabs_pair(t.wslab, (int64_t)3 * d * d, P.g_wqkv, t.bslab, (int64_t)3 * d, P.g_bqkv, TAIL_WSPLIT, wstream));
+          if (hipEventRecord(done[par], (hipStream_t)side) != hipSuccess) return MMT_ERR_ARG;
+          done_cap[par] = capture_id((hipStream_t)side);
+        }
       }
       e = {}; e.live_rows_hint = lh;
       float* dnext = w.dA;
       TRY(gemm_hidden(w, rows, d, dqkv, 3 * d, P.wqkv_t, 3 * d, dnext, d, 3 * d, MMT_EPI_F32, &e, nr, stream));
-      TRY(mmt_rows_scatter(t.dz, b->out_rows, nc, d, dnext, 1, stream));
+      if (fork_w) {
+        TRY(mmt_rows_scatter(t.dz, b->out_rows, nc, d, dnext, 1, stream));
+      } else {
+        TRY(mmt_reduce_slabs_pair_rows_scatter(t.wslab, (int64_t)3 * d * d, P.g_wqkv, t.bslab, (int64_t)3 * d, P.g_bqkv,
+                                               TAIL_WSPLIT, t.dz, b->out_rows, nc, d, dnext, 1, stream));
+      }
       dcur = dnext;
       continue;
     }
@@ -483,7 +500,12 @@
   if (fork_r) TRY(mmt_stream_fork(stream, side));
   const int chunks = mmt_table_grad_chunks();
   const bool pos_partials = b->pos_ids && m->max_pos <= 128;
-  if (m->type_vocab <= 128) {
+  const bool scatter_rides = scatter && m->type_vocab <= 64 && (!pos_partials || m->max_pos <= 64) && !fork_r;
+  if (scatter_rides) {
+    TRY(mmt_table_grad_pair_scatter_bwd(dfeatures, b->type_ids, m->type_vocab, w.table_scratch[0],
+                                        pos_partials ? b->pos_ids : nullptr, m->max_pos, w.table_scratch[1], rows, d, nr, scatter,
+                                        stream));
+  } else if (m->type_vocab <= 128) {
     TRY(mmt_table_grad_partials_pair(dfeatures, b->type_ids, m->type_vocab, w.table_scratch[0],
                                      pos_partials ? b->pos_ids : nullptr, m->max_pos, w.table_scratch[1], rows, d, nr, rstream));
   } else {
@@ -496,6 +518,9 @@
     TRY(mmt_table_grad_direct(dfeatures, b->pos_ids, rows, d, m->max_pos, nr, m->g_pos_emb, rstream));
   TRY(mmt_col_reduce_multi(jobs, njobs, rstream));
   if (join) TRY(mmt_stream_fork(side, stream));
+  if (scatter && !scatter_rides)
+    TRY(mmt_video_scatter_bwd(scatter->experts, scatter->M, scatter->B, scatter->T, scatter->d, scatter->n_rows_dev,
+                              scatter->row_index, scatter->src, dfeatures, stream));
   return 0;
 }
 
diff --git a/mmt_amd/csrc/colaunch.h b/mmt_amd/csrc/colaunch.h
--- /dev/null
+++ b/mmt_amd/csrc/colaunch.h
@@ -0,0 +1,155 @@
+#pragma once
+#include "mmt_common.h"
+#include "video_front.h"
+
+__device__ __forceinline__ void reduce_slabs_pair_block(int bid, int nblocks, const float* __restrict__ wa, int64_t ca4,
+                                                        float* __restrict__ oa, const float* __restrict__ wb, int64_t cb4,
+                                                        float* __restrict__ ob, int splits) {
+  for (int64_t i = bid * (int64_t)blockDim.x + threadIdx.x; i < ca4 + cb4; i += (int64_t)nblocks * blockDim.x) {
+    const bool first = i < ca4;
+    const f32x4* ws = (const f32x4*)(first ? wa : wb);
+    const int64_t j = first ? i : i - ca4, c4 = first ? ca4 : cb4;
+    f32x4 s = ws[j];
+    for (int k = 1; k < splits; ++k) s += ws[k * c4 + j];
+    ((f32x4*)(first ? oa : ob))[j] = s;
+  }
+}
+
+static inline int reduce_slabs_pair_grid(int64_t count_a, int64_t count_b) {
+  const int64_t c4 = (count_a + count_b) / 4;
+  return (int)((c4 + 255) / 256 < 2048 ? (c4 + 255) / 256 : 2048);
+}
+
+__device__ __forceinline__ void row_move_block(int bid, int nblocks, const float* __restrict__ src, float* __restrict__ dst,
+                                               const int32_t* __restrict__ rows, int n, int d, int scatter,
+                                               const int32_t* __restrict__ idx_in, int32_t* __restrict__ idx_out) {
+  const int lane = threadIdx.x & 63, wave = threadIdx.x >> 6;
+  for (int i = bid * 4 + wave; i < n; i += nblocks * 4) {
+    const int64_t r = rows[i];
+    const float* s = scatter ? src + (int64_t)i * d : src + r * d;
+    float* t = scatter ? dst + r * d : dst + (int64_t)i * d;
+    if (scatter == 2) {
+      for (int c = lane * 4; c < d; c += 256) *(f32x4*)(t + c) += *(const f32x4*)(s + c);
+    } else {
+      for (int c = lane * 4; c < d; c += 256) *(f32x4*)(t + c) = *(const f32x4*)(s + c);
+    }
+    if (!scatter && idx_out && lane == 0) idx_out[i] = idx_in ? idx_in[r] : (int32_t)r;
+  }
+}
+
+#define TABLE_CHUNKS 64
+typedef __attribute__((ext_vector_type(16))) float f32x16_t;
+struct TablePair { const int32_t* ids[2]; float* partial[2]; int vocab[2]; };
+#define TG_ROWS 64
+template <int NU>
+__device__ __forceinline__ void table_grad_mfma_block(int bx, int chunk, float (*gt)[128 + 4], int32_t (*idt)[TG_ROWS],
+                                                      const float* __restrict__ g, const TablePair& tp, int rows, int d,
+                                                      const int32_t* __restrict__ n_rows_dev) {
+  const int tid = threadIdx.x, lane = tid & 63, wave = tid >> 6, l31 = lane & 31, h = lane >> 5;
+  const int cb = bx * 128;
+  const int nrows = n_rows_dev ? min(*n_rows_dev, rows) : rows;
+  const int per = (nrows + TABLE_CHUNKS - 1) / TABLE_CHUNKS;
+  const int r_begin = chunk * per, r_end = min(nrows, r_begin + per);
+  const int ntab = tp.ids[1] ? 2 : 1;
+  f32x16_t acc[2][NU];
+#pragma unroll
+  for (int t = 0; t < 2; ++t)
+#pragma unroll
+    for (int u = 0; u < NU; ++u)
+#pragma unroll
+      for (int r = 0; r < 16; ++r) acc[t][u][r] = 0.f;
+  for (int r0 = r_begin; r0 < r_end; r0 += TG_ROWS) {
+#pragma unroll
+    for (int i = 0; i < TG_ROWS * 32 / 256; ++i) {
+      const int e = i * 256 + tid, rr = e >> 5, c4 = (e & 31) * 4;
+      f32x4 v = {0.f, 0.f, 0.f, 0.f};
+      if (r0 + rr < r_end) v = *(const f32x4*)(g + (int64_t)(r0 + rr) * d + cb + c4);
+      *(f32x4*)(&gt[rr][c4]) = v;
+    }
+    if (tid < 2 * TG_ROWS) {
+      const int t = tid / TG_ROWS, rr = tid % TG_ROWS;
+      idt[t][rr] = (t < ntab && r0 + rr < r_end) ? tp.ids[t][r0 + rr] : -1;
+    }
+    __syncthreads();
+#pragma unroll
+    for (int t = 0; t < 2; ++t) {
+      if (t >= ntab) continue;
+#pragma unroll
+      for (int u = 0; u < NU; ++u) {
+        if (u * 32 >= tp.vocab[t]) continue;
+        const int myv = u * 32 + l31;
+#pragma unroll 8
+        for (int kk = 0; kk < TG_ROWS / 2; ++kk) {
+          const int k = 2 * kk + h;
+          acc[t][u] = __builtin_amdgcn_mfma_f32_32x32x2f32(idt[t][k] == myv ? 1.0f : 0.0f, gt[k][wave * 32 + l31], acc[t][u], 0, 0, 0);
+        }
+      }
+    }
+    __syncthreads();
+  }
+#pragma unroll
+  for (int t = 0; t < 2; ++t) {
+    if (t >= ntab) continue;
+#pragma unroll
+    for (int u = 0; u < NU; ++u)
+#pragma unroll
+      for (int r = 0; r < 16; ++r) {
+        const int v = u * 32 + (r & 3) + 8 * (r >> 2) + 4 * h;
+        if (v < tp.vocab[t]) tp.partial[t][((int64_t)chunk * tp.vocab[t] + v) * d + cb + wave * 32 + l31] = acc[t][u][r];
+      }
+  }
+}
+
+template <bool BWD>
+__device__ __forceinline__ void video_scatter_block(int bid, int nblocks, const ExpertTable& tab, int M, int T, int S, int d,
+                                                    int rows, const int32_t* __restrict__ n_rows_dev,
+                                                    const int32_t* __restrict__ row_index, const MmtVideoSrc& src,
+                                                    float* __restrict__ feat, const float* __restrict__ dfeat) {
+  const int lane = threadIdx.x & 63, wave = threadIdx.x >> 6;
+  const int nrows = n_rows_dev ? min(*n_rows_dev, rows) : rows;
+  const int nch = d >> 8;
+  for (int row = bid * 4 + wave; row < nrows; row += nblocks * 4) {
+    const int s = row_index[row] % S;
+    if (s == 0) {
+      if constexpr (!BWD)
+        for (int c = lane * 4; c < d; c += 256) *(f32x4*)(feat + (int64_t)row * d + c) = (f32x4){0.f, 0.f, 0.f, 0.f};
+      continue;
+    }
+    const MmtExpertIO e = tab.e[(s - 1) / (T + 1)];
+    const int64_t r = src.src_row[row];
+    f32x4 y[4];
+    float ss = 0.f;
+#pragma unroll
+    for (int c = 0; c < 4; ++c)
+      if (c < nch) {
+        y[c] = *(const f32x4*)(e.y + r * d + c * 256 + lane * 4);
+        if (e.n_part > 0) y[c] += *(const f32x4*)(e.y_part[0] + r * d + c * 256 + lane * 4);
+        if (e.n_part > 1) y[c] += *(const f32x4*)(e.y_part[1] + r * d + c * 256 + lane * 4);
+        ss += y[c][0] * y[c][0] + y[c][1] * y[c][1] + y[c][2] * y[c][2] + y[c][3] * y[c][3];
+      }
+    const float nrm = sqrtf(wave_sum(ss));
+    const float inv = 1.0f / fmaxf(nrm, 1e-12f);
+    if constexpr (!BWD) {
+#pragma unroll
+      for (int c = 0; c < 4; ++c)
+        if (c < nch) *(f32x4*)(feat + (int64_t)row * d + c * 256 + lane * 4) = y[c] * inv;
+    } else {
+      f32x4 g[4];
+      float dot = 0.f;
+#pragma unroll
+      for (int c = 0; c < 4; ++c)
+        if (c < nch) {
+          g[c] = *(const f32x4*)(dfeat + (int64_t)row * d + c * 256 + lane * 4);
+          dot += g[c][0] * y[c][0] + g[c][1] * y[c][1] + g[c][2] * y[c][2] + g[c][3] * y[c][3];
+        }
+      const float proj = nrm > 1e-12f ? wave_sum(dot) * inv * inv : 0.f;
+#pragma unroll
+      for (int c = 0; c < 4; ++c)
+        if (c < nch) {
+          f32x4 dyv = (g[c] - y[c] * proj) * inv;
+          u32x2 o = {pack_bf2(dyv[0], dyv[1]), pack_bf2(dyv[2], dyv[3])};
+          *(u32x2*)((bf16_t*)e.dy + r * d + c * 256 + lane * 4) = o;
+        }
+    }
+  }
+}
diff --git a/mmt_amd/csrc/gemm.hip b/mmt_amd/csrc/gemm.hip
--- a/mmt_amd/csrc/gemm.hip
+++ b/mmt_amd/csrc/gemm.hip
@@ -1,5 +1,6 @@
 #include "mmt_common.h"
 #include "../../include/mmt_hip.h"
+#include "colaunch.h"
 
 #define BK 64
 
@@ -763,24 +764,15 @@
 
 __global__ void reduce_slabs_pair_kernel(const float* __restrict__ wa, int64_t ca4, float* __restrict__ oa,
                                          const float* __restrict__ wb, int64_t cb4, float* __restrict__ ob, int splits) {
-  for (int64_t i = blockIdx.x * (int64_t)blockDim.x + threadIdx.x; i < ca4 + cb4; i += (int64_t)gridDim.x * blockDim.x) {
-    const bool first = i < ca4;
-    const f32x4* ws = (const f32x4*)(first ? wa : wb);
-    const int64_t j = first ? i : i - ca4, c4 = first ? ca4 : cb4;
-    f32x4 s = ws[j];
-    for (int k = 1; k < splits; ++k) s += ws[k * c4 + j];
-    ((f32x4*)(first ? oa : ob))[j] = s;
-  }
+  reduce_slabs_pair_block((int)blockIdx.x, (int)gridDim.x, wa, ca4, oa, wb, cb4, ob, splits);
 }
 
 extern "C" int mmt_reduce_slabs_pair(const float* ws_a, int64_t count_a, float* out_a, const float* ws_b, int64_t count_b,
                                      float* out_b, int splits, void* stream) {
   if (!ws_a || !out_a || !ws_b || !out_b || splits <= 0 || count_a <= 0 || count_b <= 0 || ((count_a | count_b) & 3))
     return MMT_ERR_ARG;
-  const int64_t c4 = (count_a + count_b) / 4;
-  const int grid = (int)((c4 + 255) / 256 < 2048 ? (c4 + 255) / 256 : 2048);
-  hipLaunchKernelGGL(reduce_slabs_pair_kernel, dim3(grid), dim3(256), 0, (hipStream_t)stream, ws_a, count_a / 4, out_a, ws_b,
-                     count_b / 4, out_b, splits);
+  hipLaunchKernelGGL(reduce_slabs_pair_kernel, dim3(reduce_slabs_pair_grid(count_a, count_b)), dim3(256), 0, (hipStream_t)stream,
+                     ws_a, count_a / 4, out_a, ws_b, count_b / 4, out_b, splits);
   return (int)hipGetLastError();
 }
 
diff --git a/mmt_amd/csrc/norm.hip b/mmt_amd/csrc/norm.hip
--- a/mmt_amd/csrc/norm.hip
+++ b/mmt_amd/csrc/norm.hip
@@ -1,6 +1,7 @@
 #include "mmt_common.h"
 #include "attn_sched.h"
 #include "../../include/mmt_hip.h"
+#include "colaunch.h"
 
 #define MAXC 4
 
@@ -368,7 +369,6 @@
   }
 }
 
-#define TABLE_CHUNKS 64
 __global__ __launch_bounds__(256) void table_grad_kernel(
     const float* __restrict__ g, const int32_t* __restrict__ ids, int rows, int d, int vocab,
     const int32_t* __restrict__ n_rows_dev, float* __restrict__ partial) {
@@ -390,67 +390,12 @@
   partial[((int64_t)chunk * vocab + v) * d + col] = s;
 }
 
-typedef __attribute__((ext_vector_type(16))) float f32x16_t;
-struct TablePair { const int32_t* ids[2]; float* partial[2]; int vocab[2]; };
-#define TG_ROWS 64
 template <int NU>
 __global__ __launch_bounds__(256) void table_grad_mfma_kernel(const float* __restrict__ g, TablePair tp, int rows, int d,
                                                               const int32_t* __restrict__ n_rows_dev) {
   __shared__ __attribute__((aligned(16))) float gt[TG_ROWS][128 + 4];
   __shared__ int32_t idt[2][TG_ROWS];
-  const int tid = threadIdx.x, lane = tid & 63, wave = tid >> 6, l31 = lane & 31, h = lane >> 5;
-  const int cb = blockIdx.x * 128, chunk = blockIdx.y;
-  const int nrows = n_rows_dev ? min(*n_rows_dev, rows) : rows;
-  const int per = (nrows + TABLE_CHUNKS - 1) / TABLE_CHUNKS;
-  const int r_begin = chunk * per, r_end = min(nrows, r_begin + per);
-  const int ntab = tp.ids[1] ? 2 : 1;
-  f32x16_t acc[2][NU];
-#pragma unroll
-  for (int t = 0; t < 2; ++t)
-#pragma unroll
-    for (int u = 0; u < NU; ++u)
-#pragma unroll
-      for (int r = 0; r < 16; ++r) acc[t][u][r] = 0.f;
-  for (int r0 = r_begin; r0 < r_end; r0 += TG_ROWS) {
-#pragma unroll
-    for (int i = 0; i < TG_ROWS * 32 / 256; ++i) {
-      const int e = i * 256 + tid, rr = e >> 5, c4 = (e & 31) * 4;
-      f32x4 v = {0.f, 0.f, 0.f, 0.f};
-      if (r0 + rr < r_end) v = *(const f32x4*)(g + (int64_t)(r0 + rr) * d + cb + c4);
-      *(f32x4*)(&gt[rr][c4]) = v;
-    }
-    if (tid < 2 * TG_ROWS) {
-      const int t = tid / TG_ROWS, rr = tid % TG_ROWS;
-      idt[t][rr] = (t < ntab && r0 + rr < r_end) ? tp.ids[t][r0 + rr] : -1;
-    }
-    __syncthreads();
-#pragma unroll
-    for (int t = 0; t < 2; ++t) {
-      if (t >= ntab) continue;
-#pragma unroll
-      for (int u = 0; u < NU; ++u) {
-        if (u * 32 >= tp.vocab[t]) continue;
-        const int myv = u * 32 + l31;
-#pragma unroll 8
-        for (int kk = 0; kk < TG_ROWS / 2; ++kk) {
-          const int k = 2 * kk + h;
-          acc[t][u] = __builtin_amdgcn_mfma_f32_32x32x2f32(idt[t][k] == myv ? 1.0f : 0.0f, gt[k][wave * 32 + l31], acc[t][u], 0, 0, 0);
-        }
-      }
-    }
-    __syncthreads();
-  }
-#pragma unroll
-  for (int t = 0; t < 2; ++t) {
-    if (t >= ntab) continue;
-#pragma unroll
-    for (int u = 0; u < NU; ++u)
-#pragma unroll
-      for (int r = 0; r < 16; ++r) {
-        const int v = u * 32 + (r & 3) + 8 * (r >> 2) + 4 * h;
-        if (v < tp.vocab[t]) tp.partial[t][((int64_t)chunk * tp.vocab[t] + v) * d + cb + wave * 32 + l31] = acc[t][u][r];
-      }
-  }
+  table_grad_mfma_block<NU>((int)blockIdx.x, (int)blockIdx.y, gt, idt, g, tp, rows, d, n_rows_dev);
 }
 
 static inline int ln_grid(int rows) {
@@ -483,18 +428,31 @@
 __global__ __launch_bounds__(256) void row_move_kernel(const float* __restrict__ src, float* __restrict__ dst,
                                                        const int32_t* __restrict__ rows, int n, int d, int scatter,
                                                        const int32_t* __restrict__ idx_in, int32_t* __restrict__ idx_out) {
-  const int lane = threadIdx.x & 63, wave = threadIdx.x >> 6;
-  for (int i = blockIdx.x * 4 + wave; i < n; i += gridDim.x * 4) {
-    const int64_t r = rows[i];
-    const float* s = scatter ? src + (int64_t)i * d : src + r * d;
-    float* t = scatter ? dst + r * d : dst + (int64_t)i * d;
-    if (scatter == 2) {
-      for (int c = lane * 4; c < d; c += 256) *(f32x4*)(t + c) += *(const f32x4*)(s + c);
-    } else {
-      for (int c = lane * 4; c < d; c += 256) *(f32x4*)(t + c) = *(const f32x4*)(s + c);
-    }
-    if (!scatter && idx_out && lane == 0) idx_out[i] = idx_in ? idx_in[r] : (int32_t)r;
-  }
+  row_move_block((int)blockIdx.x, (int)gridDim.x, src, dst, rows, n, d, scatter, idx_in, idx_out);
+}
+
+__global__ __launch_bounds__(256) void reduce_pair_rows_scatter_kernel(
+    int nred, const float* __restrict__ wa, int64_t ca4, float* __restrict__ oa, const float* __restrict__ wb, int64_t cb4,
+    float* __restrict__ ob, int splits, const float* __restrict__ src, float* __restrict__ dst,
+    const int32_t* __restrict__ rows, int n, int d, int scatter) {
+  const int bid = (int)blockIdx.x;
+  if (bid < nred) reduce_slabs_pair_block(bid, nred, wa, ca4, oa, wb, cb4, ob, splits);
+  else row_move_block(bid - nred, (int)gridDim.x - nred, src, dst, rows, n, d, scatter, nullptr, nullptr);
+}
+
+extern "C" int mmt_reduce_slabs_pair_rows_scatter(const float* ws_a, int64_t count_a, float* out_a, const float* ws_b,
+                                                  int64_t count_b, float* out_b, int splits, const float* src,
+                                                  const int32_t* rows, int n, int d, float* dst, int accumulate,
+                                                  void* stream) {
+  const bool red = count_a > 0 || count_b > 0;
+  if (red && (!ws_a || !out_a || !ws_b || !out_b || splits <= 0 || count_a <= 0 || count_b <= 0 || ((count_a | count_b) & 3)))
+    return MMT_ERR_ARG;
+  if (count_a < 0 || count_b < 0 || n < 0 || (!red && n == 0)) return MMT_ERR_ARG;
+  if (n > 0 && (!src || !rows || !dst || d <= 0 || (d & 3))) return MMT_ERR_ARG;
+  const int nred = red ? reduce_slabs_pair_grid(count_a, count_b) : 0;
+  hipLaunchKernelGGL(reduce_pair_rows_scatter_kernel, dim3(nred + (n + 3) / 4), dim3(256), 0, (hipStream_t)stream, nred, ws_a,
+                     count_a / 4, out_a, ws_b, count_b / 4, out_b, splits, src, dst, rows, n, d, accumulate ? 2 : 1);
+  return (int)hipGetLastError();
 }
 
 extern "C" int mmt_rows_gather(const float* src, const int32_t* rows, int n, int d, float* dst, const int32_t* idx_in,
diff --git a/mmt_amd/model.py b/mmt_amd/model.py
--- a/mmt_amd/model.py
+++ b/mmt_amd/model.py
@@ -8,7 +8,7 @@
 from torch import nn
 
 from . import _lib, ops
-from ._lib import MmtExpertIO, MmtTextHeads, MmtTextHeadsOpts, MmtVideoFront, MmtVideoSrc, check
+from ._lib import MmtExpertIO, MmtTextHeads, MmtTextHeadsOpts, MmtVideoFront, MmtVideoScatterBwd, MmtVideoSrc, check
 from .bert import BertModel, EngineBatch
 from .feature_store import RaggedFeatures
 from .flat import FlatParams
@@ -206,6 +206,7 @@
     self.rows = bsz * self.seq
     self.rows_alloc = ops.pad_rows(self.rows)
     self.generation = 0
+    self.scatter_in_engine = False
     self.front_done = -1
     i32 = dict(device=device, dtype=torch.int32)
     self.counts = torch.zeros(bsz, **i32)
@@ -483,11 +484,19 @@
     f.src = ctypes.addressof(plan.src)
     return f
 
+  def _scatter_bwd_desc(self, plan):
+    sc = MmtVideoScatterBwd()
+    sc.experts, sc.src = ctypes.addressof(plan.io), ctypes.addressof(plan.src)
+    sc.M, sc.B, sc.T, sc.d = len(self.modalities), plan.batch, plan.tokens, self.same_dim
+    sc.n_rows_dev, sc.row_index = plan.n_rows.data_ptr(), plan.row_index.data_ptr()
+    return sc
+
   def _video_tokens_backward(self, plan, dfeat, side_stream=None):
     L, m, d = _lib.lib(), len(self.modalities), self.same_dim
     stream = ops._stream()
-    check(L.mmt_video_scatter_bwd(plan.io, m, plan.batch, plan.tokens, d, ops._p(plan.n_rows), ops._p(plan.row_index),
-                                  ctypes.byref(plan.src), ops._p(dfeat), stream), 'mmt_video_scatter_bwd')
+    if not plan.scatter_in_engine:
+      check(L.mmt_video_scatter_bwd(plan.io, m, plan.batch, plan.tokens, d, ops._p(plan.n_rows), ops._p(plan.row_index),
+                                    ctypes.byref(plan.src), ops._p(dfeat), stream), 'mmt_video_scatter_bwd')
     grad_buf = self._flat.current_grad()
     grads, items = [], []
     for mod in self.modalities:
@@ -517,6 +526,8 @@
     if hint is None and isinstance(features, RaggedFeatures):
       hint = bsz + sum(int(v) for v in features.live.values())
     batch.live_rows_hint = int(hint or 0) if self.pack_tokens else 0
+    batch.scatter_bwd, batch.scatter_plan = self._scatter_bwd_desc(plan), plan
+    plan.scatter_in_engine = True
     last = self.vid_bert.run_engine(batch, feats)
     self._stages = dict(plan=plan, feats=feats, batch=batch, last=last) if last.requires_grad else None
     if self.vid_bert.compact_output(batch, plan.rows_alloc):
```

Result: no change. 25550 pairs/s, median of 6 (+0.6%).
